# ruffle-rs/h263-rs

Hardware: NVIDIA B200
Metric: decoded_rgba_megapixels_per_s (higher is better)
Workload: dtype f32+u8

## Files before the change

bindings/h263cu-sys/src/lib.rs:

```rust
#![allow(non_camel_case_types)]
use std::os::raw::{c_char, c_int, c_void};

pub const H263CU_OK: c_int = 0;
pub const H263CU_ERR_INTERNAL_DECODER_ERROR: c_int = -1;
pub const H263CU_ERR_MIDDLE_OF_BITSTREAM: c_int = -2;
pub const H263CU_ERR_INVALID_MACROBLOCK_HEADER: c_int = -3;
pub const H263CU_ERR_INVALID_MACROBLOCK_CODED_BITS: c_int = -4;
pub const H263CU_ERR_INVALID_INTRA_DC: c_int = -5;
pub const H263CU_ERR_INVALID_SHORT_COEFFICIENT: c_int = -6;
pub const H263CU_ERR_INVALID_LONG_COEFFICIENT: c_int = -7;
pub const H263CU_ERR_INVALID_MVD: c_int = -8;
pub const H263CU_ERR_INVALID_PTYPE: c_int = -9;
pub const H263CU_ERR_INVALID_PLUSPTYPE: c_int = -10;
pub const H263CU_ERR_INVALID_GOB_HEADER: c_int = -11;
pub const H263CU_ERR_INVALID_BITSTREAM: c_int = -12;
pub const H263CU_ERR_PICTURE_FORMAT_MISSING: c_int = -13;
pub const H263CU_ERR_PICTURE_FORMAT_INVALID: c_int = -14;
pub const H263CU_ERR_UNCODED_IFRAME_BLOCKS: c_int = -15;
pub const H263CU_ERR_UNHANDLED_IO_ERROR: c_int = -16;
pub const H263CU_ERR_UNIMPLEMENTED_DECODING: c_int = -17;
pub const H263CU_ERR_BAD_ARGUMENT: c_int = -100;
pub const H263CU_ERR_CUDA: c_int = -101;
pub const H263CU_ERR_NO_DEVICE: c_int = -102;
pub const H263CU_ERR_CAPACITY: c_int = -103;
pub const H263CU_ERR_REFERENCE_WOULD_ABORT: c_int = -104;
pub const H263CU_ERR_NO_PICTURE: c_int = -105;
pub const H263CU_ERR_OUT_OF_MEMORY: c_int = -106;

pub const H263CU_OPT_SORENSON_SPARK_BITSTREAM: u32 = 1;
pub const H263CU_OPT_USE_SCALABILITY_MODE: u32 = 2;
pub const H263CU_OPT_DECODE_DISPOSABLE: u32 = 0x100;

pub const H263CU_PIC_I: u8 = 0;
pub const H263CU_PIC_P: u8 = 1;
pub const H263CU_PIC_DISPOSABLE_P: u8 = 2;
pub const H263CU_PIC_OTHER: u8 = 3;
pub const H263CU_PICFLAG_DEBLOCK: u8 = 1;
pub const H263CU_PICFLAG_HAS_INTER: u8 = 2;
pub const H263CU_PICFLAG_MV_IN_RANGE: u8 = 4;
pub const H263CU_PICFLAG_DISPOSABLE: u8 = 8;
pub const H263CU_MB_INTER: u8 = 1;
pub const H263CU_MB_WIDE: u8 = 2;
pub const H263CU_MB_FOURMV: u8 = 4;
pub const H263CU_MB_CODED: u8 = 8;
pub const H263CU_OUT_RGBA: u32 = 1;
pub const H263CU_OUT_DEBLOCK: u32 = 2;
pub const H263CU_YUV_I420: u32 = 0;
pub const H263CU_YUV_NV12: u32 = 1;
pub const H263CU_TENSOR_U8: u32 = 0;
pub const H263CU_TENSOR_F32: u32 = 1;
pub const H263CU_TENSOR_F16: u32 = 2;
pub const H263CU_TENSOR_BF16: u32 = 3;
pub const H263CU_FIT_STRETCH: u32 = 0;
pub const H263CU_FIT_LETTERBOX: u32 = 1;
pub const H263CU_FIT_CENTER_CROP: u32 = 2;
pub const H263CU_FILTER_BILINEAR: u32 = 0;
pub const H263CU_FILTER_BILINEAR_AA: u32 = 1;
pub const H263CU_FILTER_BICUBIC_AA: u32 = 2;

#[repr(C)]
#[derive(Clone, Copy, Debug, Default)]
pub struct h263cu_pic {
    pub stream: u32,
    pub width: u16,
    pub height: u16,
    pub mb_w: u8,
    pub mb_h: u8,
    pub pic_type: u8,
    pub pquant: u8,
    pub flags: u8,
    pub version: u8,
    pub temporal_reference: u16,
    pub first_mb: u32,
    pub n_mbs: u32,
    pub first_event: u32,
    pub n_event_units: u32,
}

#[repr(C)]
#[derive(Clone, Copy, Debug, Default)]
pub struct h263cu_mb {
    pub ev_off: u32,
    pub pic: u16,
    pub mbx: u8,
    pub mby: u8,
    pub flags: u8,
    pub quant: u8,
    pub nev: [u8; 6],
    pub u: [u8; 8],
}

#[repr(C)]
#[derive(Clone, Copy, Debug, Default)]
pub struct h263cu_flv_packet {
    pub offset: u64,
    pub size: u32,
    pub timestamp_ms: u32,
    pub frame_type: u8,
    pub codec_id: u8,
    pub reserved: u16,
    pub reserved2: u32,
}

pub type h263cu_event = u16;

#[repr(C)]
#[derive(Clone, Copy, Debug)]
pub struct h263cu_device_rgba {
    pub base: *mut u8,
    pub row_pitch: u64,
    pub pic_stride: u64,
    pub width: u32,
    pub height: u32,
    pub stream: *mut c_void,
}

#[repr(C)]
#[derive(Clone, Copy, Debug)]
pub struct h263cu_device_plane {
    pub base: *mut u8,
    pub row_pitch: u64,
    pub pic_stride: u64,
}

#[repr(C)]
#[derive(Clone, Copy, Debug)]
pub struct h263cu_device_yuv {
    pub plane: [h263cu_device_plane; 3],
    pub width: u32,
    pub height: u32,
    pub format: u32,
    pub reserved: u32,
    pub stream: *mut c_void,
}

#[repr(C)]
#[derive(Clone, Copy, Debug)]
pub struct h263cu_device_tensor {
    pub base: *mut c_void,
    pub stride: [i64; 4],
    pub width: u32,
    pub height: u32,
    pub dtype: u32,
    pub reserved: u32,
    pub mul: [f32; 3],
    pub add: [f32; 3],
    pub stream: *mut c_void,
}

#[repr(C)]
#[derive(Clone, Copy, Debug)]
pub struct h263cu_tensor_crop {
    pub x: u32,
    pub y: u32,
    pub width: u32,
    pub height: u32,
}

#[repr(C)]
#[derive(Clone, Copy, Debug)]
pub struct h263cu_tensor_fit {
    pub mode: u32,
    pub short_side: u32,
    pub fill: [f32; 3],
    pub reserved: u32,
    pub crops: *const h263cu_tensor_crop,
}

#[repr(C)]
pub struct h263cu_parser {
    _private: [u8; 0],
}
#[repr(C)]
pub struct h263cu_ctx {
    _private: [u8; 0],
}
#[repr(C)]
pub struct h263cu_step {
    _private: [u8; 0],
}
#[repr(C)]
pub struct h263cu_graph {
    _private: [u8; 0],
}
#[repr(C)]
pub struct h263cu_group {
    _private: [u8; 0],
}

extern "C" {
    pub fn h263cu_is_eof_error(err: c_int) -> c_int;
    pub fn h263cu_is_macroblock_error(err: c_int) -> c_int;
    pub fn h263cu_is_gob_error(err: c_int) -> c_int;
    pub fn h263cu_strerror(err: c_int) -> *const c_char;
    pub fn h263cu_version() -> c_int;

    pub fn h263cu_parser_create(decoder_options: u32) -> *mut h263cu_parser;
// ... 167 lines not shown
```

h263_rs_b200/_lib.py:

```python
import ctypes as C
import os

HERE = os.path.dirname(os.path.abspath(__file__))
LIB_PATH = os.environ.get("H263CU_LIB", os.path.join(HERE, "libh263cu.so"))

OK = 0
ERR_INVALID_BITSTREAM = -12
ERR_UNHANDLED_IO_ERROR = -16
ERR_BAD_ARGUMENT = -100
ERR_CUDA = -101
ERR_NO_DEVICE = -102
ERR_CAPACITY = -103
ERR_REFERENCE_WOULD_ABORT = -104
ERR_NO_PICTURE = -105

OPT_SORENSON = 1
OUT_RGBA = 1
OUT_DEBLOCK = 2

PIC_I, PIC_P, PIC_DISPOSABLE_P, PIC_OTHER = 0, 1, 2, 3
MB_INTER, MB_WIDE, MB_FOURMV, MB_CODED = 1, 2, 4, 8


class Pic(C.Structure):
    _fields_ = [
        ("stream", C.c_uint32), ("width", C.c_uint16), ("height", C.c_uint16), ("mb_w", C.c_uint8),
        ("mb_h", C.c_uint8), ("pic_type", C.c_uint8), ("pquant", C.c_uint8), ("flags", C.c_uint8),
        ("version", C.c_uint8), ("temporal_reference", C.c_uint16), ("first_mb", C.c_uint32), ("n_mbs", C.c_uint32),
        ("first_event", C.c_uint32), ("n_event_units", C.c_uint32),
    ]


class MbUnion(C.Union):
    _fields_ = [("mv", (C.c_int8 * 2) * 4), ("intradc", C.c_uint8 * 6)]


class Mb(C.Structure):
    _fields_ = [
        ("ev_off", C.c_uint32), ("pic", C.c_uint16), ("mbx", C.c_uint8), ("mby", C.c_uint8), ("flags", C.c_uint8),
        ("quant", C.c_uint8), ("nev", C.c_uint8 * 6), ("u", MbUnion),
    ]


class DeviceRgba(C.Structure):
    _fields_ = [
        ("base", C.c_void_p), ("row_pitch", C.c_uint64), ("pic_stride", C.c_uint64), ("width", C.c_uint32),
        ("height", C.c_uint32), ("stream", C.c_void_p),
    ]


class DevicePlane(C.Structure):
    _fields_ = [("base", C.c_void_p), ("row_pitch", C.c_uint64), ("pic_stride", C.c_uint64)]


class DeviceYuv(C.Structure):
    _fields_ = [
        ("plane", DevicePlane * 3), ("width", C.c_uint32), ("height", C.c_uint32), ("format", C.c_uint32),
        ("reserved", C.c_uint32), ("stream", C.c_void_p),
    ]


YUV_I420, YUV_NV12 = 0, 1


class DeviceTensor(C.Structure):
    _fields_ = [
        ("base", C.c_void_p), ("stride", C.c_int64 * 4), ("width", C.c_uint32), ("height", C.c_uint32),
        ("dtype", C.c_uint32), ("reserved", C.c_uint32), ("mul", C.c_float * 3), ("add", C.c_float * 3),
        ("stream", C.c_void_p),
    ]


TENSOR_U8, TENSOR_F32, TENSOR_F16, TENSOR_BF16 = 0, 1, 2, 3


class TensorCrop(C.Structure):
    _fields_ = [("x", C.c_uint32), ("y", C.c_uint32), ("width", C.c_uint32), ("height", C.c_uint32)]


class TensorFit(C.Structure):
    _fields_ = [
        ("mode", C.c_uint32), ("short_side", C.c_uint32), ("fill", C.c_float * 3), ("reserved", C.c_uint32),
        ("crops", C.POINTER(TensorCrop)),
    ]


FIT_STRETCH, FIT_LETTERBOX, FIT_CENTER_CROP = 0, 1, 2
FILTER_BILINEAR, FILTER_BILINEAR_AA, FILTER_BICUBIC_AA = 0, 1, 2

assert C.sizeof(Pic) == 32 and C.sizeof(Mb) == 24 and C.sizeof(DeviceRgba) == 40
assert C.sizeof(DevicePlane) == 24 and C.sizeof(DeviceYuv) == 96 and C.sizeof(DeviceTensor) == 88
assert C.sizeof(TensorCrop) == 16 and C.sizeof(TensorFit) == 32

SYMBOLS = [
    "h263cu_is_eof_error", "h263cu_is_macroblock_error", "h263cu_is_gob_error", "h263cu_strerror",
    "h263cu_version", "h263cu_parser_create", "h263cu_parser_destroy", "h263cu_parser_options", "h263cu_parser_reset",
    "h263cu_peek_picture", "h263cu_parse_picture", "h263cu_parse_step", "h263cu_device_count",
    "h263cu_create", "h263cu_destroy", "h263cu_device_of", "h263cu_alloc_pinned", "h263cu_free_pinned",
    "h263cu_step_upload", "h263cu_step_free", "h263cu_step_run", "h263cu_submit_step",
    "h263cu_submit_step_readback", "h263cu_decode_step", "h263cu_sync", "h263cu_stream_info", "h263cu_read_yuv", "h263cu_read_rgba",
    "h263cu_checksums", "h263cu_timer_start", "h263cu_timer_stop", "h263cu_launch_count", "h263cu_tiled_launch_count",
    "h263cu_profile_enable", "h263cu_profile_read", "h263cu_host_times",
    "h263cu_yuv420_to_rgba", "h263cu_deblock", "h263cu_quant_to_strength",
    "h263cu_flv_scan", "h263cu_flv_mux",
    "h263cu_test_read_bits", "h263cu_test_start_code", "h263cu_test_read_vlc", "h263cu_test_decode_block",
    "h263cu_readback_wait", "h263cu_stream_dims", "h263cu_graph_build", "h263cu_graph_launch", "h263cu_graph_free", "h263cu_group_create", "h263cu_group_destroy", "h263cu_group_size", "h263cu_group_ctx",
    "h263cu_group_decode_step", "h263cu_group_sync", "h263cu_decode_step_device", "h263cu_group_decode_step_device",
    "h263cu_decode_step_device_yuv", "h263cu_group_decode_step_device_yuv",
    "h263cu_decode_step_device_tensor", "h263cu_group_decode_step_device_tensor",
    "h263cu_decode_step_device_tensor_fit", "h263cu_group_decode_step_device_tensor_fit", "h263cu_test_fit_geometry",
    "h263cu_decode_step_device_tensor_filter", "h263cu_group_decode_step_device_tensor_filter",
]

_lib = None


def lib():
    global _lib
    if _lib is not None:
        return _lib
    if not os.path.exists(LIB_PATH):
        raise RuntimeError(
            "libh263cu.so is missing (%s): run `python -c 'import __graft_entry__ as g; g.build()'`; "
            "this package has no CPU fallback" % LIB_PATH
        )
    L = C.CDLL(LIB_PATH)
    vp, u32, u64, i32 = C.c_void_p, C.c_uint32, C.c_uint64, C.c_int
    L.h263cu_strerror.restype = C.c_char_p
    L.h263cu_strerror.argtypes = [i32]
    L.h263cu_parser_create.restype = vp
    L.h263cu_parser_create.argtypes = [u32]
    L.h263cu_parser_destroy.argtypes = [vp]
    L.h263cu_parser_options.restype = u32
    L.h263cu_parser_options.argtypes = [vp]
    L.h263cu_parser_destroy.restype = None
    L.h263cu_parser_reset.argtypes = [vp]
    L.h263cu_parser_reset.restype = None
    L.h263cu_peek_picture.argtypes = [u32, C.c_char_p, C.c_size_t, C.POINTER(Pic)]
    L.h263cu_parse_picture.argtypes = [vp, C.c_char_p, C.c_size_t, u32, C.c_uint16, u32, u32, C.POINTER(Pic), vp, u32,
                                       vp, u32]
    L.h263cu_parse_step.argtypes = [vp, vp, vp, vp, u32, i32, vp, vp, u32, vp, u32, C.POINTER(u32), C.POINTER(u32),
                                    C.POINTER(u32), vp, vp]
    if hasattr(L, "h263cu_create"):
        L.h263cu_create.restype = vp
        L.h263cu_create.argtypes = [i32, u32, u32, u32, u32, C.POINTER(i32)]
        L.h263cu_destroy.argtypes = [vp]
        L.h263cu_destroy.restype = None
        L.h263cu_device_of.argtypes = [vp]
        L.h263cu_alloc_pinned.restype = vp
        L.h263cu_alloc_pinned.argtypes = [C.c_size_t]
        L.h263cu_free_pinned.argtypes = [vp]
        L.h263cu_free_pinned.restype = None
        L.h263cu_step_upload.restype = vp
        L.h263cu_step_upload.argtypes = [vp, vp, u32, vp, u32, vp, u32, C.POINTER(i32)]
        L.h263cu_step_free.argtypes = [vp, vp]
        L.h263cu_step_free.restype = None
        L.h263cu_step_run.argtypes = [vp, vp, u32]
        L.h263cu_submit_step.argtypes = [vp, vp, u32, vp, u32, vp, u32, u32]
        L.h263cu_submit_step_readback.argtypes = [vp, vp, u32, vp, u32, vp, u32, u32, vp, vp]
        L.h263cu_decode_step.argtypes = [vp, vp, vp, vp, vp, u32, i32, u32, vp, u64, vp, C.POINTER(u32)]
        L.h263cu_decode_step_device.argtypes = [vp, vp, vp, vp, vp, u32, i32, u32, C.POINTER(DeviceRgba), vp, C.POINTER(u32)]
        L.h263cu_decode_step_device_yuv.argtypes = [vp, vp, vp, vp, vp, u32, i32, u32, C.POINTER(DeviceYuv), vp, C.POINTER(u32)]
        L.h263cu_decode_step_device_tensor.argtypes = [vp, vp, vp, vp, vp, u32, i32, u32, C.POINTER(DeviceTensor), vp, C.POINTER(u32)]
        L.h263cu_decode_step_device_tensor_fit.argtypes = [vp, vp, vp, vp, vp, u32, i32, u32, C.POINTER(DeviceTensor),
                                                           C.POINTER(TensorFit), vp, C.POINTER(u32)]
        L.h263cu_decode_step_device_tensor_filter.argtypes = [vp, vp, vp, vp, vp, u32, i32, u32, C.POINTER(DeviceTensor),
                                                              C.POINTER(TensorFit), u32, vp, C.POINTER(u32)]
        L.h263cu_sync.argtypes = [vp]
        L.h263cu_readback_wait.argtypes = [vp, u32]
        L.h263cu_graph_build.restype = vp
        L.h263cu_graph_build.argtypes = [vp, vp, u32, u32, C.POINTER(i32)]
        L.h263cu_graph_launch.argtypes = [vp, vp]
        L.h263cu_graph_free.argtypes = [vp, vp]
        L.h263cu_graph_free.restype = None
# ... 69 lines not shown
```

h263_rs_b200/csrc/context.cu:

```cuda
#include <cuda_runtime.h>

#include <algorithm>
#include <chrono>
#include <cmath>
#include <cstdio>
#include <cstdlib>
#include <cstring>
#include <mutex>
#include <new>
#include <vector>

#include "device_math.cuh"
#include "kernels.cuh"

using namespace h263dev;

namespace h263fe {
int parse_step_deferred(h263cu_parser* const* parsers, const uint8_t* const* packets, const size_t* lens,
                        const uint32_t* stream_ids, uint32_t n, int threads, h263cu_pic* pics, h263cu_mb* mbs, uint32_t mb_cap,
                        h263cu_event* events, uint32_t ev_cap, uint32_t* n_pics_out, uint32_t* n_mbs_out, uint32_t* n_units_out,
                        int* per_pic_err, int32_t* pic_of_input, uint32_t max_w, uint32_t max_h, const uint32_t* min_size);
void parse_step_finish(h263cu_parser* const* parsers, uint32_t n, bool accept);
}

extern "C" const uint8_t h263cu_quant_to_strength[32] = H263_QUANT_TO_STRENGTH;

namespace {

#define CU_TRY(expr)                      \
    do {                                  \
        cudaError_t _e = (expr);          \
        if (_e != cudaSuccess) return map_cuda_error(_e); \
    } while (0)

int map_cuda_error(cudaError_t e) {
    switch (e) {
        case cudaErrorNoDevice:
        case cudaErrorInsufficientDriver:
        case cudaErrorInvalidDevice: return H263CU_ERR_NO_DEVICE;
        case cudaErrorMemoryAllocation: return H263CU_ERR_OUT_OF_MEMORY;
        default: return H263CU_ERR_CUDA;
    }
}

inline size_t round_up(size_t v, size_t a) { return (v + a - 1) / a * a; }

struct StreamState {
    bool has_pic = false;
    uint8_t cur_slot = 0;
    int8_t rgba_slot = -1;
    uint16_t w = 0, h = 0;
    uint8_t pic_type = 0, pquant = 0;
    uint16_t tr = 0;
    uint32_t stamp = 0;
    uint32_t seen = 0;
    bool has_ref = false;
    uint8_t ref_slot = 0;
    uint16_t ref_w = 0, ref_h = 0;
    bool padded = false;
};

inline int next_slot(const StreamState& st) { return st.has_ref ? (st.ref_slot ^ 1) : (st.has_pic ? (st.cur_slot ^ 1) : 0); }

inline void advance_stream(StreamState& st, const h263cu_pic& p, bool want_rgba, int rgba_ring, bool tiled) {
    const int slot = next_slot(st);
    st.cur_slot = (uint8_t)slot;
    st.has_pic = true;
    st.w = p.width, st.h = p.height;
    st.pic_type = p.pic_type, st.pquant = p.pquant, st.tr = p.temporal_reference;
    st.rgba_slot = want_rgba ? (int8_t)rgba_ring : (int8_t)-1;
    if (!(p.flags & H263CU_PICFLAG_DISPOSABLE)) {
        st.has_ref = true;
        st.ref_slot = (uint8_t)slot;
        st.ref_w = p.width, st.ref_h = p.height;
        st.padded = tiled;
    }
}

}

struct h263cu_step {
    std::vector<h263cu_pic> pics;
    h263cu_mb* d_mbs = nullptr;
    h263cu_event* d_events = nullptr;
    uint32_t n_mbs = 0, n_units = 0;
    size_t mb_cap = 0, ev_cap = 0;
    uint32_t max_w = 0, max_h = 0;
};

struct h263cu_ctx {
    int device = 0;
    uint32_t max_streams = 0, max_w = 0, max_h = 0;
    uint32_t mbw = 0, mbh = 0;
    uint32_t pitch_y = 0, pitch_c = 0, rgba_pitch = 0;
    size_t y_slot = 0, c_slot = 0, rgba_slot = 0;
    uint8_t *y_pool = nullptr, *c_pool = nullptr, *rgba_pool = nullptr;
    CUtensorMap rgba_map;
    std::vector<StreamState> streams;
    uint32_t stamp = 0, decode_epoch = 0;
    uint32_t rgba_parity = 0;

    cudaStream_t s_main = nullptr, s_h2d = nullptr, s_d2h = nullptr;
    cudaStream_t s_pics = nullptr;
    static constexpr int PIC_RING = 4;
    PicDev* h_pics[PIC_RING] = {};
    PicDev* d_pics[PIC_RING] = {};
    cudaEvent_t pics_done[PIC_RING] = {};
    cudaEvent_t pics_up[PIC_RING] = {};
    FitGeom* h_geo[PIC_RING] = {};
    FitGeom* d_geo[PIC_RING] = {};
    size_t pics_cap = 0;
    int pic_ring_pos = 0;
    h263cu_step ring[2];
    cudaEvent_t ring_h2d_done[2] = {}, ring_run_done[2] = {};
    int ring_pos = 0;
    struct Staging {
        h263cu_pic* pics = nullptr;
        h263cu_mb* mbs = nullptr;
        h263cu_event* events = nullptr;
        size_t pic_cap = 0, mb_cap = 0, ev_cap = 0;
    } staging[2];
    std::vector<int32_t> pic_of_input;
    std::vector<uint64_t> rgba_offsets;
    std::vector<uint32_t> dev_slots;
    std::vector<uint32_t> fit_min;
    std::vector<FitGeom> fit_geo;
    cudaEvent_t dev_ready = nullptr, dev_done = nullptr;
    uint8_t* tensor_scratch = nullptr;
    size_t tensor_scratch_slots = 0;
    cudaEvent_t rgba_written[2] = {}, rgba_read[2] = {};
    cudaEvent_t t0 = nullptr, t1 = nullptr;
    uint64_t launches = 0, tiled_launches = 0;
    bool profiling = false;
    std::vector<cudaEvent_t> prof_free;
    struct ProfSpan {
        cudaEvent_t a, b;
        int kind;
    };
    std::vector<ProfSpan> prof_spans;
    ChecksumJob* d_jobs = nullptr;
    unsigned long long* d_sums = nullptr;
    size_t jobs_cap = 0;

    int force_kernel = 0;
    double host_parse_s = 0.0, host_other_s = 0.0;
    uint64_t host_calls = 0;
    uint8_t* plane(int p, uint32_t stream, int slot) const {
        const size_t idx = (size_t)stream * 2 + (size_t)slot;
        if (p == 0) return y_pool + idx * y_slot + (size_t)PAD_Y_ROWS * pitch_y + PAD_Y_COLS;
        return c_pool + idx * c_slot + (size_t)PAD_C_ROWS * pitch_c + PAD_C_COLS + (p == 2 ? 1 : 0);
    }
    uint8_t* rgba(uint32_t stream, int slot) const { return rgba_pool + ((size_t)slot * max_streams + stream) * rgba_slot; }
};

namespace {

int ensure_pic_ring(h263cu_ctx* c, size_t n) {
    if (n <= c->pics_cap) return 0;
    CU_TRY(cudaStreamSynchronize(c->s_main));
    size_t cap = std::max<size_t>(n, 256);
    for (int i = 0; i < h263cu_ctx::PIC_RING; i++) {
        if (c->h_pics[i]) cudaFreeHost(c->h_pics[i]);
        if (c->d_pics[i]) cudaFree(c->d_pics[i]);
        if (c->h_geo[i]) cudaFreeHost(c->h_geo[i]);
        if (c->d_geo[i]) cudaFree(c->d_geo[i]);
        c->h_pics[i] = nullptr, c->d_pics[i] = nullptr, c->h_geo[i] = nullptr, c->d_geo[i] = nullptr;
        CU_TRY(cudaHostAlloc((void**)&c->h_pics[i], cap * sizeof(PicDev), cudaHostAllocDefault));
        CU_TRY(cudaMalloc((void**)&c->d_pics[i], cap * sizeof(PicDev)));
        CU_TRY(cudaHostAlloc((void**)&c->h_geo[i], cap * sizeof(FitGeom), cudaHostAllocDefault));
        CU_TRY(cudaMalloc((void**)&c->d_geo[i], cap * sizeof(FitGeom)));
    }
    c->pics_cap = cap;
    return 0;
}

int step_reserve(h263cu_step* s, size_t n_mbs, size_t n_units) {
    if (n_mbs > s->mb_cap) {
        if (s->d_mbs) cudaFree(s->d_mbs);
        s->d_mbs = nullptr;
        size_t cap = n_mbs + n_mbs / 8 + 64;
        CU_TRY(cudaMalloc((void**)&s->d_mbs, cap * sizeof(h263cu_mb)));
        s->mb_cap = cap;
    }
    if (n_units + 8 > s->ev_cap) {
        if (s->d_events) cudaFree(s->d_events);
        s->d_events = nullptr;
        size_t cap = n_units + n_units / 8 + 64;
        CU_TRY(cudaMalloc((void**)&s->d_events, cap * sizeof(h263cu_event)));
        s->ev_cap = cap;
    }
    return 0;
}

int prof_take(h263cu_ctx* c, cudaEvent_t* a, cudaEvent_t* b) {
    for (cudaEvent_t* e : {a, b}) {
        if (!c->prof_free.empty()) {
            *e = c->prof_free.back();
            c->prof_free.pop_back();
        } else {
            CU_TRY(cudaEventCreate(e));
        }
    }
    return 0;
}
void prof_end(h263cu_ctx* c, cudaEvent_t a, cudaEvent_t b, int kind) {
    cudaEventRecord(b, c->s_main);
    c->prof_spans.push_back({a, b, kind});
}

PicDev make_picdev(const h263cu_ctx* c, const h263cu_pic& p, const StreamState& st, bool want_rgba, int rgba_ring) {
    const int ref_slot = st.ref_slot, new_slot = next_slot(st);
    PicDev d;
    std::memset(&d, 0, sizeof(d));
    for (int k = 0; k < 3; k++) {
        d.cur[k] = c->plane(k, p.stream, new_slot);
        d.ref[k] = st.has_ref ? c->plane(k, p.stream, ref_slot) : nullptr;
    }
    d.rgba = want_rgba ? c->rgba(p.stream, rgba_ring) : nullptr;
    d.cur_y4 = (uint32_t)((d.cur[0] - c->y_pool) >> 2);
    d.cur_c4 = (uint32_t)((d.cur[1] - c->c_pool) >> 2);
    d.ref_y4 = st.has_ref ? (uint32_t)((d.ref[0] - c->y_pool) >> 2) : 0u;
    d.ref_c4 = st.has_ref ? (uint32_t)((d.ref[1] - c->c_pool) >> 2) : 0u;
    d.rgba_row0 = want_rgba ? (uint32_t)((size_t)(d.rgba - c->rgba_pool) / c->rgba_pitch) : 0u;
    d.first_event = p.first_event;
    d.rgba_pitch = c->rgba_pitch;
    d.w = p.width, d.h = p.height;
    d.cw = (uint16_t)((p.width + 1) / 2), d.ch = (uint16_t)((p.height + 1) / 2);
    d.pitch_y = (uint16_t)c->pitch_y, d.pitch_c = (uint16_t)c->pitch_c;
    d.strength = h263cu_quant_to_strength[p.pquant & 31];
    d.flags = p.flags;
    return d;
}

struct DeviceTarget {
    int out;
    CUtensorMap map;
    uint8_t* base;
    uint64_t row_pitch, pic_stride;
    YuvDst yuv;
    TensorDst tensor;
// ... 2 lines not shown
    float fill[3];
    uint32_t filter;
    const uint32_t* slots;
    cudaStream_t stream;
};

int ensure_tensor_scratch(h263cu_ctx* c, uint32_t n, YuvDst* d) {
    const size_t pitch = (size_t)c->mbw * 16, y_bytes = pitch * c->mbh * 16, c_bytes = pitch * c->mbh * 8;
    if (n > c->tensor_scratch_slots) {
        CU_TRY(cudaStreamSynchronize(c->s_main));
        if (c->tensor_scratch) cudaFree(c->tensor_scratch);
        c->tensor_scratch = nullptr, c->tensor_scratch_slots = 0;
        const size_t slots = std::max<size_t>(n, 64);
        CU_TRY(cudaMalloc((void**)&c->tensor_scratch, slots * (y_bytes + c_bytes)));
        c->tensor_scratch_slots = slots;
    }
    std::memset(d, 0, sizeof(*d));
    d->base[0] = c->tensor_scratch, d->base[1] = c->tensor_scratch + c->tensor_scratch_slots * y_bytes;
    d->stride[0] = y_bytes, d->stride[1] = c_bytes;
    d->pitch[0] = d->pitch[1] = (uint32_t)pitch;
    d->nv12 = 1;
    return 0;
}

int run_step(h263cu_ctx* c, h263cu_step* s, uint32_t out_flags, bool lean = false, const DeviceTarget* dev = nullptr) {
    const uint32_t n = (uint32_t)s->pics.size();
    if (n == 0) return 0;
    if (n > 65535) return H263CU_ERR_CAPACITY;
    const bool want_rgba = dev || (out_flags & H263CU_OUT_RGBA) != 0;
    const bool pool_rgba = want_rgba && !dev;
    const bool want_deblock = want_rgba && (out_flags & H263CU_OUT_DEBLOCK) != 0;
    const bool tensor = dev && dev->out == OUT_TENSOR;
    const uint32_t stamp = ++c->stamp;
    uint32_t max_w = 0, max_h = 0;
    bool tiled = true, aligned16 = true, wide_mv = false;
    for (uint32_t i = 0; i < n; i++) {
        const h263cu_pic& p = s->pics[i];
        if (p.stream >= c->max_streams) return H263CU_ERR_CAPACITY;
        if (p.width == 0 || p.height == 0 || p.width > c->max_w || p.height > c->max_h) return H263CU_ERR_CAPACITY;
        if ((uint32_t)p.mb_w * 16 < p.width || (uint32_t)p.mb_h * 16 < p.height ||
            (uint32_t)p.mb_w > c->mbw || (uint32_t)p.mb_h > c->mbh)
            return H263CU_ERR_BAD_ARGUMENT;
        if ((uint64_t)p.first_mb + p.n_mbs > s->n_mbs || (uint64_t)p.first_event + p.n_event_units > s->n_units ||
            p.n_mbs != (uint32_t)p.mb_w * p.mb_h)
            return H263CU_ERR_BAD_ARGUMENT;
        StreamState& st = c->streams[p.stream];
        if (st.stamp == stamp) return H263CU_ERR_BAD_ARGUMENT;
        st.stamp = stamp;
        if (p.flags & H263CU_PICFLAG_HAS_INTER) {
            if (!st.has_ref) return H263CU_ERR_UNCODED_IFRAME_BLOCKS;
            if (st.ref_w != p.width || st.ref_h != p.height) return H263CU_ERR_REFERENCE_WOULD_ABORT;
        }
        max_w = std::max<uint32_t>(max_w, p.width);
        max_h = std::max<uint32_t>(max_h, p.height);
        if ((p.width | p.height) & 15) aligned16 = false;
        if ((p.flags & H263CU_PICFLAG_HAS_INTER) && !(p.flags & H263CU_PICFLAG_MV_IN_RANGE)) wide_mv = true;
        if ((p.flags & H263CU_PICFLAG_HAS_INTER) && !st.padded) tiled = false;
    }
    if (c->force_kernel == 1) tiled = false;
    int e = ensure_pic_ring(c, n);
    if (e) return e;
    YuvDst scratch{};
    if (tensor && want_deblock && (e = ensure_tensor_scratch(c, n, &scratch))) return e;
    const int slot = c->pic_ring_pos;
    CU_TRY(cudaEventSynchronize(c->pics_done[slot]));
    const int rgba_ring = (int)(c->rgba_parity & 1u);
    PicDev* hp = c->h_pics[slot];
    const bool fit = tensor && dev->geo;
    if (fit) std::memcpy(c->h_geo[slot], dev->geo, n * sizeof(FitGeom));
    for (uint32_t i = 0; i < n; i++) {
        const h263cu_pic& p = s->pics[i];
        PicDev d = make_picdev(c, p, c->streams[p.stream], pool_rgba, rgba_ring);
        if (tensor) {
            d.rgba = want_deblock ? yuv_row(scratch, 0, i, 0) : nullptr;
            d.rgba_row0 = i << 12;
            d.out_slot = dev->slots[i];
        } else if (dev) {
            if (dev->out == OUT_YUV) {
                d.rgba = yuv_row(dev->yuv, 0, dev->slots[i], 0);
                d.rgba_pitch = dev->yuv.pitch[0];
            } else {
                d.rgba = dev->base + (size_t)dev->slots[i] * dev->pic_stride;
                d.rgba_pitch = (uint32_t)dev->row_pitch;
            }
            d.rgba_row0 = dev->slots[i] << 12;
        }
        hp[i] = d;
    }
    cudaEvent_t pa = nullptr, pb = nullptr, qa = nullptr, qb = nullptr;
    if (c->profiling) {
        if ((e = prof_take(c, &pa, &pb))) return e;
        if (want_deblock && (e = prof_take(c, &qa, &qb))) {
            c->prof_free.push_back(pa), c->prof_free.push_back(pb);
            return e;
        }
    }
    if (lean) {
        CU_TRY(cudaMemcpyAsync(c->d_pics[slot], hp, n * sizeof(PicDev), cudaMemcpyHostToDevice, c->s_main));
        if (fit) CU_TRY(cudaMemcpyAsync(c->d_geo[slot], c->h_geo[slot], n * sizeof(FitGeom), cudaMemcpyHostToDevice, c->s_main));
    } else {
        CU_TRY(cudaMemcpyAsync(c->d_pics[slot], hp, n * sizeof(PicDev), cudaMemcpyHostToDevice, c->s_pics));
        if (fit) CU_TRY(cudaMemcpyAsync(c->d_geo[slot], c->h_geo[slot], n * sizeof(FitGeom), cudaMemcpyHostToDevice, c->s_pics));
        CU_TRY(cudaEventRecord(c->pics_up[slot], c->s_pics));
        CU_TRY(cudaStreamWaitEvent(c->s_main, c->pics_up[slot], 0));
    }
    if (pool_rgba) {
        CU_TRY(cudaStreamWaitEvent(c->s_main, c->rgba_read[rgba_ring], 0));
    }
    if (dev) {
        CU_TRY(cudaEventRecord(c->dev_ready, dev->stream));
        CU_TRY(cudaStreamWaitEvent(c->s_main, c->dev_ready, 0));
    }
    if (pa) cudaEventRecord(pa, c->s_main);
    const Pools pools{c->y_pool, c->c_pool, c->rgba_pool, c->pitch_y, c->pitch_c, c->rgba_pitch};
    const YuvDst* yuv = dev && dev->out == OUT_YUV ? &dev->yuv : tensor && want_deblock ? &scratch : nullptr;
    const bool dev_out = dev && !tensor;
    launch_recon(c->d_pics[slot], s->d_mbs, s->d_events, s->n_mbs, want_rgba && !want_deblock && !tensor, tiled ? (aligned16 ? 1 : 2) : 0,
                 wide_mv, pools, dev_out ? &dev->map : &c->rgba_map, dev_out ? dev->out : OUT_POOL, yuv, c->s_main);
    if (pa) prof_end(c, pa, pb, 0);
    if (want_deblock) {
        if (qa) cudaEventRecord(qa, c->s_main);
        if (aligned16 && c->force_kernel != 1)
            launch_deblock_rgba_tile(c->d_pics[slot], n, max_w, max_h, yuv, c->s_main);
        else
            launch_deblock_rgba(c->d_pics[slot], n, max_w, max_h, yuv, c->s_main);
        if (qa) prof_end(c, qa, qb, 1);
    }
    if (tensor) {
        const FitArgs fa{c->d_geo[slot], {dev->fill[0], dev->fill[1], dev->fill[2]}};
        if (fit && dev->filter != H263CU_FILTER_BILINEAR)
            launch_resample_filter(c->d_pics[slot], n, want_deblock ? &scratch : nullptr, dev->tensor, dev->dtype, dev->filter, fa,
                                   c->s_main);
        else
            launch_resample_rgb(c->d_pics[slot], n, want_deblock ? &scratch : nullptr, dev->tensor, dev->dtype, fit ? &fa : nullptr,
                                c->s_main);
    }
    CU_TRY(cudaGetLastError());
    c->pic_ring_pos = (c->pic_ring_pos + 1) % h263cu_ctx::PIC_RING;
    c->launches += (want_deblock ? 2 : 1) + (tensor ? 1 : 0);
    if (tiled) c->tiled_launches++;
    for (uint32_t i = 0; i < n; i++) advance_stream(c->streams[s->pics[i].stream], s->pics[i], pool_rgba, rgba_ring, tiled);
    CU_TRY(cudaEventRecord(c->pics_done[slot], c->s_main));
    if (dev) {
        CU_TRY(cudaEventRecord(c->dev_done, c->s_main));
        CU_TRY(cudaStreamWaitEvent(dev->stream, c->dev_done, 0));
    }
    if (pool_rgba) {
        if (!lean) CU_TRY(cudaEventRecord(c->rgba_written[rgba_ring], c->s_main));
        c->rgba_parity++;
    }
    return 0;
}

int validate_side_info(std::vector<h263cu_pic>& pics, const h263cu_mb* mbs, uint32_t n_mbs, uint32_t n_units) {
    for (size_t i = 0; i < pics.size(); i++) {
        h263cu_pic& p = pics[i];
        if ((uint64_t)p.first_mb + p.n_mbs > n_mbs || (uint64_t)p.first_event + p.n_event_units > n_units ||
            p.n_mbs != (uint32_t)p.mb_w * p.mb_h || p.mb_w == 0)
            return H263CU_ERR_BAD_ARGUMENT;
        bool any_inter = false, in_range = true;
        const h263cu_mb* m = mbs + p.first_mb;
        for (uint32_t k = 0; k < p.n_mbs; k++, m++) {
            if (m->pic != i || (uint32_t)m->mby * p.mb_w + m->mbx != k || m->mbx >= p.mb_w) return H263CU_ERR_BAD_ARGUMENT;
            const bool intra = !(m->flags & H263CU_MB_INTER);
            uint32_t ev = 0;
            for (int b = 0; b < 6; b++) {
                if (m->nev[b] > (intra ? 63 : 64) || (intra && m->nev[b] && m->u.intradc[b] == 0)) return H263CU_ERR_BAD_ARGUMENT;
                ev += m->nev[b];
            }
            if (m->flags & H263CU_MB_WIDE) ev *= 2;
            if ((uint64_t)m->ev_off + ev > p.n_event_units) return H263CU_ERR_BAD_ARGUMENT;
            if (m->flags & H263CU_MB_INTER) {
                any_inter = true;
                for (int b = 0; b < 4; b++)
                    in_range &= m->u.mv[b][0] >= -32 && m->u.mv[b][0] <= 31 && m->u.mv[b][1] >= -32 && m->u.mv[b][1] <= 31;
            }
        }
        if (any_inter) p.flags |= H263CU_PICFLAG_HAS_INTER;
        if (!in_range) p.flags &= (uint8_t)~H263CU_PICFLAG_MV_IN_RANGE;
    }
    return 0;
}

int upload_into(h263cu_ctx* c, h263cu_step* s, const h263cu_pic* pics, uint32_t n_pics, const h263cu_mb* mbs,
                uint32_t n_mbs, const h263cu_event* events, uint32_t n_units, cudaStream_t stream, bool trusted) {
    int e = step_reserve(s, n_mbs, n_units);
    if (e) return e;
    try {
        s->pics.assign(pics, pics + n_pics);
    } catch (const std::bad_alloc&) {
        return H263CU_ERR_OUT_OF_MEMORY;
    }
    s->n_mbs = n_mbs, s->n_units = n_units;
    if (!trusted && (e = validate_side_info(s->pics, mbs, n_mbs, n_units))) {
        s->pics.clear();
        return e;
    }
    if (n_mbs) CU_TRY(cudaMemcpyAsync(s->d_mbs, mbs, (size_t)n_mbs * sizeof(h263cu_mb), cudaMemcpyHostToDevice, stream));
    if (n_units)
        CU_TRY(cudaMemcpyAsync(s->d_events, events, (size_t)n_units * sizeof(h263cu_event), cudaMemcpyHostToDevice, stream));
    (void)c;
    return 0;
}

template <typename T>
int grow_pinned(T** p, size_t* cap, size_t need) {
    if (need <= *cap) return 0;
    if (*p) cudaFreeHost(*p);
    *p = nullptr, *cap = 0;
    const size_t n = need + need / 4 + 64;
    CU_TRY(cudaHostAlloc((void**)p, n * sizeof(T), cudaHostAllocDefault));
    *cap = n;
    return 0;
}
typedef CUresult (*EncodeTiled)(CUtensorMap*, CUtensorMapDataType, cuuint32_t, void*, const cuuint64_t*, const cuuint64_t*,
                                const cuuint32_t*, const cuuint32_t*, CUtensorMapInterleave, CUtensorMapSwizzle,
                                CUtensorMapL2promotion, CUtensorMapFloatOOBfill);
EncodeTiled encode_tiled() {
    static const EncodeTiled fn = [] {
        EncodeTiled enc = nullptr;
        cudaDriverEntryPointQueryResult q;
        if (cudaGetDriverEntryPoint("cuTensorMapEncodeTiled", (void**)&enc, cudaEnableDefault, &q) != cudaSuccess) {
            cudaGetLastError();
            enc = nullptr;
        }
        return enc;
    }();
    return fn;
}
int encode_rgba_map(CUtensorMap* map, void* base, uint32_t rank, const cuuint64_t* dims, const cuuint64_t* strides) {
    const EncodeTiled enc = encode_tiled();
    if (!enc) return H263CU_ERR_CUDA;
    const cuuint32_t box[3] = {64, 16, 1}, es[3] = {1, 1, 1};
    if (enc(map, CU_TENSOR_MAP_DATA_TYPE_UINT8, rank, base, dims, strides, box, es, CU_TENSOR_MAP_INTERLEAVE_NONE,
            CU_TENSOR_MAP_SWIZZLE_NONE, CU_TENSOR_MAP_L2_PROMOTION_NONE, CU_TENSOR_MAP_FLOAT_OOB_FILL_NONE) != CUDA_SUCCESS)
        return H263CU_ERR_CUDA;
    return 0;
}
int make_rgba_map(CUtensorMap* map, void* base, uint64_t pitch, uint64_t rows) {
    std::memset(map, 0, sizeof(*map));
    if (!recon_tile_uses_tma()) return 0;
    const cuuint64_t dims[2] = {pitch, rows}, strides[1] = {pitch};
    return encode_rgba_map(map, base, 2, dims, strides);
}
int check_device_memory(const h263cu_ctx* c, const void* p) {
    cudaPointerAttributes a;
    if (cudaPointerGetAttributes(&a, p) != cudaSuccess) {
        cudaGetLastError();
        return H263CU_ERR_BAD_ARGUMENT;
    }
    if ((a.type != cudaMemoryTypeDevice && a.type != cudaMemoryTypeManaged) || a.device != c->device) return H263CU_ERR_BAD_ARGUMENT;
    return 0;
}
int check_device_rgba(const h263cu_ctx* c, const h263cu_device_rgba* o) {
    if (!o || !recon_tile_uses_tma()) return H263CU_ERR_BAD_ARGUMENT;
    if (!o->base || ((uintptr_t)o->base & 15u) || o->width == 0 || o->height == 0) return H263CU_ERR_BAD_ARGUMENT;
    if (o->row_pitch % 16 || o->row_pitch < 4ull * o->width || o->row_pitch >= (1ull << 32)) return H263CU_ERR_BAD_ARGUMENT;
    if (o->pic_stride % 16 || o->pic_stride < o->row_pitch * o->height || o->pic_stride >= (1ull << 40)) return H263CU_ERR_BAD_ARGUMENT;
    return check_device_memory(c, o->base);
}
int check_device_yuv(const h263cu_ctx* c, const h263cu_device_yuv* o) {
    if (!o || o->format > H263CU_YUV_NV12 || o->reserved != 0 || o->width == 0 || o->height == 0) return H263CU_ERR_BAD_ARGUMENT;
    const bool nv12 = o->format == H263CU_YUV_NV12;
    const uint64_t cw = (o->width + 1ull) / 2, ch = (o->height + 1ull) / 2;
    const uint64_t row_bytes[3] = {o->width, nv12 ? 2 * cw : cw, cw}, rows[3] = {o->height, ch, ch};
    if (nv12 && (o->plane[2].base || o->plane[2].row_pitch || o->plane[2].pic_stride)) return H263CU_ERR_BAD_ARGUMENT;
    for (int k = 0; k < (nv12 ? 2 : 3); k++) {
        const h263cu_device_plane& p = o->plane[k];
        if (!p.base || ((uintptr_t)p.base & 3u) || p.row_pitch % 4 || p.pic_stride % 4) return H263CU_ERR_BAD_ARGUMENT;
        if (p.row_pitch < row_bytes[k] || p.row_pitch >= (1ull << 32)) return H263CU_ERR_BAD_ARGUMENT;
        if (p.pic_stride < p.row_pitch * rows[k] || p.pic_stride >= (1ull << 40)) return H263CU_ERR_BAD_ARGUMENT;
    }
    for (int k = 0; k < (nv12 ? 2 : 3); k++)
        if (int e = check_device_memory(c, o->plane[k].base)) return e;
    return 0;
}
int check_device_tensor(const h263cu_ctx* c, const h263cu_device_tensor* o) {
    if (!o || o->dtype > H263CU_TENSOR_BF16 || o->reserved != 0) return H263CU_ERR_BAD_ARGUMENT;
    if (o->width == 0 || o->height == 0 || o->width > 16384 || o->height > 16384) return H263CU_ERR_BAD_ARGUMENT;
    static const uint32_t elem_bytes[4] = {1, 4, 2, 2};
    const uint32_t es = elem_bytes[o->dtype];
    if (!o->base || (uintptr_t)o->base % es) return H263CU_ERR_BAD_ARGUMENT;
    for (int k = 0; k < 4; k++)
        if (o->stride[k] <= 0) return H263CU_ERR_BAD_ARGUMENT;
    const unsigned __int128 extent = ((unsigned __int128)(o->width - 1) * (uint64_t)o->stride[3] +
                                      (unsigned __int128)(o->height - 1) * (uint64_t)o->stride[2] +
                                      (unsigned __int128)2 * (uint64_t)o->stride[1] + 1) * es;
    if (extent >= ((unsigned __int128)1 << 40)) return H263CU_ERR_BAD_ARGUMENT;
    for (int k = 0; k < 3; k++) {
        if (!std::isfinite(o->mul[k]) || !std::isfinite(o->add[k])) return H263CU_ERR_BAD_ARGUMENT;
        if (o->dtype == H263CU_TENSOR_U8 && (o->mul[k] != 1.0f || o->add[k] != 0.0f)) return H263CU_ERR_BAD_ARGUMENT;
    }
    return check_device_memory(c, o->base);
}
int check_tensor_fit(const h263cu_tensor_fit* f, uint32_t n) {
    if (!f || f->mode > H263CU_FIT_CENTER_CROP || f->reserved != 0) return H263CU_ERR_BAD_ARGUMENT;
    if (f->mode == H263CU_FIT_CENTER_CROP ? f->short_side < 1 || f->short_side > 16384 : f->short_side != 0)
        return H263CU_ERR_BAD_ARGUMENT;
    for (int k = 0; k < 3; k++)
        if (!(f->fill[k] >= 0.0f && f->fill[k] <= 255.0f)) return H263CU_ERR_BAD_ARGUMENT;
    if (f->crops)
        for (uint32_t i = 0; i < n; i++) {
            const h263cu_tensor_crop& b = f->crops[i];
            if (b.width == 0 || b.height == 0 || (uint64_t)b.x + b.width > 0xFFFFFFFFull || (uint64_t)b.y + b.height > 0xFFFFFFFFull)
                return H263CU_ERR_BAD_ARGUMENT;
        }
    return 0;
}
void fit_geometry(uint32_t mode, uint32_t short_side, uint32_t cw, uint32_t ch, uint32_t W, uint32_t H, int32_t* out4) {
    const int64_t w = cw, h = ch, ow = W, oh = H, S = short_side;
    int64_t rw = ow, rh = oh, px = 0, py = 0;
    if (mode == H263CU_FIT_LETTERBOX) {
        if (w * oh >= h * ow)
            rh = std::max<int64_t>(1, (2 * h * ow + w) / (2 * w));
        else
            rw = std::max<int64_t>(1, (2 * w * oh + h) / (2 * h));
        px = (ow - rw) / 2, py = (oh - rh) / 2;
    } else if (mode == H263CU_FIT_CENTER_CROP) {
        if (w <= h)
            rw = S, rh = S * h / w;
        else
            rh = S, rw = S * w / h;
        const auto place = [](int64_t r, int64_t o) -> int64_t {
            if (r < o) return (o - r) / 2;
            const int64_t d = r - o, k = d / 2;
            return -((d & 1) ? k + (k & 1) : k);
        };
        px = place(rw, ow), py = place(rh, oh);
    }
    out4[0] = (int32_t)rw, out4[1] = (int32_t)rh, out4[2] = (int32_t)px, out4[3] = (int32_t)py;
}
void free_step_buffers(h263cu_step* s) {
    if (s->d_mbs) cudaFree(s->d_mbs);
    if (s->d_events) cudaFree(s->d_events);
    s->d_mbs = nullptr, s->d_events = nullptr;
    s->mb_cap = s->ev_cap = 0;
}

}

extern "C" {

int h263cu_device_count(void) {
    int n = 0;
    if (cudaGetDeviceCount(&n) != cudaSuccess) {
        cudaGetLastError();
        return 0;
    }
    return n;
}

h263cu_ctx* h263cu_create(int device, uint32_t max_streams, uint32_t max_width, uint32_t max_height, uint32_t flags,
                          int* err) {
    (void)flags;
    int dummy;
    if (!err) err = &dummy;
    *err = 0;
    if (max_streams == 0 || max_width == 0 || max_height == 0 || max_width > 4080 || max_height > 4080) {
        *err = H263CU_ERR_BAD_ARGUMENT;
        return nullptr;
    }
    int ndev = 0;
    cudaError_t ce = cudaGetDeviceCount(&ndev);
    if (ce != cudaSuccess || ndev == 0) {
        cudaGetLastError();
        *err = H263CU_ERR_NO_DEVICE;
        return nullptr;
    }
    if (device < 0 || device >= ndev) {
        *err = H263CU_ERR_NO_DEVICE;
        return nullptr;
    }
    if (cudaSetDevice(device) != cudaSuccess) {
        *err = H263CU_ERR_CUDA;
        return nullptr;
    }
    h263cu_ctx* c = new (std::nothrow) h263cu_ctx();
    if (!c) {
        *err = H263CU_ERR_OUT_OF_MEMORY;
        return nullptr;
    }
    c->device = device;
    c->max_streams = max_streams, c->max_w = max_width, c->max_h = max_height;
    c->mbw = (max_width + 15) / 16, c->mbh = (max_height + 15) / 16;
    c->pitch_y = c->mbw * 16 + 2 * PAD_Y_COLS;
    c->pitch_c = c->mbw * 8 * CHROMA_STEP + 2 * PAD_C_COLS;
    c->rgba_pitch = c->mbw * 16 * 4;
    c->y_slot = (size_t)c->pitch_y * (c->mbh * 16 + 2 * PAD_Y_ROWS);
    c->c_slot = (size_t)c->pitch_c * (c->mbh * 8 + 2 * PAD_C_ROWS);
    if (const char* k = getenv("H263CU_KERNEL")) c->force_kernel = !strcmp(k, "mb") ? 1 : (!strcmp(k, "tile") ? 2 : 0);
    c->rgba_slot = (size_t)c->rgba_pitch * c->mbh * 16;
    c->streams.resize(max_streams);
    auto fail = [&](int code) {
        *err = code;
        h263cu_destroy(c);
        return (h263cu_ctx*)nullptr;
    };
    const size_t pad = 256;
    if (c->y_slot * 2 * max_streams + pad >= (16ull << 30) || c->rgba_slot * 2 * max_streams + pad >= (64ull << 30)) return fail(H263CU_ERR_CAPACITY);
    if (cudaMalloc((void**)&c->y_pool, c->y_slot * 2 * max_streams + pad) != cudaSuccess) return fail(H263CU_ERR_OUT_OF_MEMORY);
    if (cudaMalloc((void**)&c->c_pool, c->c_slot * 2 * max_streams + pad) != cudaSuccess) return fail(H263CU_ERR_OUT_OF_MEMORY);
    if (cudaMalloc((void**)&c->rgba_pool, c->rgba_slot * 2 * max_streams + pad) != cudaSuccess) return fail(H263CU_ERR_OUT_OF_MEMORY);
    {
        const int e = make_rgba_map(&c->rgba_map, c->rgba_pool, c->rgba_pitch, (uint64_t)2 * max_streams * c->mbh * 16);
        if (e) return fail(e);
    }
    if (cudaStreamCreateWithFlags(&c->s_main, cudaStreamNonBlocking) != cudaSuccess) return fail(H263CU_ERR_CUDA);
    if (cudaStreamCreateWithFlags(&c->s_h2d, cudaStreamNonBlocking) != cudaSuccess) return fail(H263CU_ERR_CUDA);
    if (cudaStreamCreateWithFlags(&c->s_d2h, cudaStreamNonBlocking) != cudaSuccess) return fail(H263CU_ERR_CUDA);
    if (cudaStreamCreateWithFlags(&c->s_pics, cudaStreamNonBlocking) != cudaSuccess) return fail(H263CU_ERR_CUDA);
    for (int i = 0; i < h263cu_ctx::PIC_RING; i++)
        if (cudaEventCreateWithFlags(&c->pics_done[i], cudaEventDisableTiming) != cudaSuccess ||
            cudaEventCreateWithFlags(&c->pics_up[i], cudaEventDisableTiming) != cudaSuccess)
            return fail(H263CU_ERR_CUDA);
    for (int i = 0; i < 2; i++) {
        if (cudaEventCreateWithFlags(&c->ring_h2d_done[i], cudaEventDisableTiming) != cudaSuccess ||
            cudaEventCreateWithFlags(&c->ring_run_done[i], cudaEventDisableTiming) != cudaSuccess ||
            cudaEventCreateWithFlags(&c->rgba_written[i], cudaEventDisableTiming) != cudaSuccess ||
            cudaEventCreateWithFlags(&c->rgba_read[i], cudaEventDisableTiming) != cudaSuccess)
            return fail(H263CU_ERR_CUDA);
    }
    if (cudaEventCreateWithFlags(&c->dev_ready, cudaEventDisableTiming) != cudaSuccess ||
        cudaEventCreateWithFlags(&c->dev_done, cudaEventDisableTiming) != cudaSuccess)
        return fail(H263CU_ERR_CUDA);
    if (cudaEventCreate(&c->t0) != cudaSuccess || cudaEventCreate(&c->t1) != cudaSuccess) return fail(H263CU_ERR_CUDA);
    cudaMemsetAsync(c->y_pool, 0, c->y_slot * 2 * max_streams + pad, c->s_main);
    cudaMemsetAsync(c->c_pool, 0, c->c_slot * 2 * max_streams + pad, c->s_main);
    if (cudaStreamSynchronize(c->s_main) != cudaSuccess) return fail(H263CU_ERR_CUDA);
    return c;
}

void h263cu_destroy(h263cu_ctx* c) {
    if (!c) return;
    cudaSetDevice(c->device);
    if (c->s_main) cudaStreamSynchronize(c->s_main);
    if (c->s_h2d) cudaStreamSynchronize(c->s_h2d);
    if (c->s_d2h) cudaStreamSynchronize(c->s_d2h);
    if (c->s_pics) cudaStreamSynchronize(c->s_pics);
    for (int i = 0; i < 2; i++) free_step_buffers(&c->ring[i]);
    for (auto& st : c->staging) {
        if (st.pics) cudaFreeHost(st.pics);
        if (st.mbs) cudaFreeHost(st.mbs);
        if (st.events) cudaFreeHost(st.events);
    }
    for (int i = 0; i < h263cu_ctx::PIC_RING; i++) {
        if (c->h_pics[i]) cudaFreeHost(c->h_pics[i]);
        if (c->d_pics[i]) cudaFree(c->d_pics[i]);
        if (c->h_geo[i]) cudaFreeHost(c->h_geo[i]);
        if (c->d_geo[i]) cudaFree(c->d_geo[i]);
        if (c->pics_done[i]) cudaEventDestroy(c->pics_done[i]);
        if (c->pics_up[i]) cudaEventDestroy(c->pics_up[i]);
    }
    for (int i = 0; i < 2; i++) {
        if (c->ring_h2d_done[i]) cudaEventDestroy(c->ring_h2d_done[i]);
        if (c->ring_run_done[i]) cudaEventDestroy(c->ring_run_done[i]);
        if (c->rgba_written[i]) cudaEventDestroy(c->rgba_written[i]);
        if (c->rgba_read[i]) cudaEventDestroy(c->rgba_read[i]);
    }
    if (c->t0) cudaEventDestroy(c->t0);
    if (c->t1) cudaEventDestroy(c->t1);
    if (c->dev_ready) cudaEventDestroy(c->dev_ready);
    if (c->dev_done) cudaEventDestroy(c->dev_done);
    if (c->tensor_scratch) cudaFree(c->tensor_scratch);
    for (auto& sp : c->prof_spans) {
        cudaEventDestroy(sp.a);
        cudaEventDestroy(sp.b);
    }
    for (auto e : c->prof_free) cudaEventDestroy(e);
    if (c->d_jobs) cudaFree(c->d_jobs);
    if (c->d_sums) cudaFree(c->d_sums);
    if (c->y_pool) cudaFree(c->y_pool);
    if (c->c_pool) cudaFree(c->c_pool);
    if (c->rgba_pool) cudaFree(c->rgba_pool);
    if (c->s_main) cudaStreamDestroy(c->s_main);
    if (c->s_h2d) cudaStreamDestroy(c->s_h2d);
    if (c->s_d2h) cudaStreamDestroy(c->s_d2h);
    if (c->s_pics) cudaStreamDestroy(c->s_pics);
    delete c;
}

int h263cu_device_of(h263cu_ctx* c) { return c ? c->device : -1; }

void* h263cu_alloc_pinned(size_t bytes) {
    void* p = nullptr;
    if (cudaHostAlloc(&p, bytes ? bytes : 1, cudaHostAllocDefault) != cudaSuccess) {
        cudaGetLastError();
        return nullptr;
    }
    return p;
// ... 898 lines not shown
```

h263_rs_b200/csrc/frontend.cpp:

```cpp
#include <algorithm>
#include <atomic>
#include <condition_variable>
#include <cstring>
#include <functional>
#include <mutex>
#include <new>
#include <pthread.h>
#include <thread>
#include <vector>

#include "../../include/h263cu.h"
#include "bitio.hpp"

namespace h263fe {

#include "vlc_codes.inc"

void VlcTable::build(const VlcCode* codes, int n) {
    max_len = 0;
    for (int i = 0; i < n; i++) max_len = std::max(max_len, codes[i].len);
    lut.assign((size_t)1 << max_len, VlcEntry{(uint8_t)(2u << 5), 0, 0, 0});
    for (int i = 0; i < n; i++) {
        uint32_t v = 0;
        for (int k = 0; k < codes[i].len; k++) v = (v << 1) | (uint32_t)(codes[i].bits[k] - '0');
        int rest = max_len - codes[i].len;
        VlcEntry e{(uint8_t)((unsigned)codes[i].len | ((unsigned)codes[i].kind << 5)), (int8_t)codes[i].a,
                   (uint8_t)codes[i].b, (uint8_t)codes[i].c};
        for (uint32_t s = 0; s < (1u << rest); s++) lut[((size_t)v << rest) | s] = e;
    }
}

namespace {
struct Tables {
    VlcTable t[5];
    std::vector<uint32_t> tcoef_fast;
    int tcoef_bits = 0;
    Tables() {
        t[T_MCBPC_I].build(MCBPC_I_CODES, MCBPC_I_CODES_COUNT);
        t[T_MCBPC_P].build(MCBPC_P_CODES, MCBPC_P_CODES_COUNT);
        t[T_CBPY].build(CBPY_CODES, CBPY_CODES_COUNT);
        t[T_MVD].build(MVD_CODES, MVD_CODES_COUNT);
        t[T_TCOEF].build(TCOEF_CODES, TCOEF_CODES_COUNT);
        tcoef_bits = t[T_TCOEF].max_len + 1;
        tcoef_fast.resize(t[T_TCOEF].lut.size() * 2);
        for (size_t i = 0; i < tcoef_fast.size(); i++) {
            const VlcEntry& e = t[T_TCOEF].lut[i >> 1];
            uint32_t w = e.len() | (e.kind() << 5);
            if (e.kind() == 0) {
                const uint32_t sign = (uint32_t)(i >> (t[T_TCOEF].max_len - e.len())) & 1u;
                const uint32_t level = sign ? (0u - (uint32_t)e.c) & 0x3FFu : (uint32_t)e.c;
                w = (e.len() + 1u) | ((uint32_t)(e.a != 0) << 7) | ((((uint32_t)e.b << 10) | level) << 16);
            }
            tcoef_fast[i] = w;
        }
    }
};
const Tables& tables() {
    static const Tables T;
    return T;
}
}

const VlcTable& vlc_table(int id) { return tables().t[id]; }
static const uint32_t* tcoef_fast_table(int* bits) {
    *bits = tables().tcoef_bits;
    return tables().tcoef_fast.data();
}
const VlcCode* vlc_codes(int id, int* count) {
    switch (id) {
        case T_MCBPC_I: *count = MCBPC_I_CODES_COUNT; return MCBPC_I_CODES;
        case T_MCBPC_P: *count = MCBPC_P_CODES_COUNT; return MCBPC_P_CODES;
        case T_CBPY: *count = CBPY_CODES_COUNT; return CBPY_CODES;
        case T_MVD: *count = MVD_CODES_COUNT; return MVD_CODES;
        default: *count = TCOEF_CODES_COUNT; return TCOEF_CODES;
    }
}

struct Header {
    int version = -1;
    uint16_t tr = 0;
    int fmt_kind = -1;
    uint16_t w = 0, h = 0;
    bool dims_valid = false;
    uint8_t pic_type = H263CU_PIC_I;
    bool type_supported = true;
    bool deblock = false;
    uint8_t quant = 0;
};

static bool std_dims(int kind, uint16_t* w, uint16_t* h) {
    static const uint16_t W[5] = {128, 176, 352, 704, 1408}, H[5] = {96, 144, 288, 576, 1152};
    if (kind < 0 || kind > 4) return false;
    *w = W[kind], *h = H[kind];
    return true;
}

static int find_start_code(BitReader& r, uint32_t* skipped) {
    const size_t save = r.pos();
    uint32_t max_skip = (uint32_t)((8 - (r.pos() & 7)) & 7);
    uint32_t skip = 0;
    for (;;) {
        if (r.avail() < 17) {
            r.seek(save);
            return H263CU_ERR_UNHANDLED_IO_ERROR;
        }
        if (r.peek_padded(17) == 1) break;
        if (skip > max_skip) {
            r.seek(save);
            return H263CU_ERR_MIDDLE_OF_BITSTREAM;
        }
        r.consume(1);
        skip += 1;
    }
    r.seek(save);
    *skipped = skip;
    return 0;
}

#define RD(n, var)                                         \
    do {                                                   \
        if (!r.read((n), &(var))) return H263CU_ERR_UNHANDLED_IO_ERROR; \
    } while (0)

static int parse_header(BitReader& r, uint32_t options, bool have_prev, int prev_kind, uint16_t prev_w,
                        uint16_t prev_h, Header* out) {
    uint32_t skipped = 0, v = 0;
    int e = find_start_code(r, &skipped);
    if (e) return e;
    if (!r.skip(17 + skipped)) return H263CU_ERR_UNHANDLED_IO_ERROR;
    uint32_t gob_id;
    RD(5, gob_id);
    Header h;
    if (options & H263CU_OPT_SORENSON_SPARK_BITSTREAM) {
        RD(8, v);
        h.tr = (uint16_t)v;
        uint32_t code;
        RD(3, code);
        switch (code) {
            case 0: {
                uint32_t cw, ch;
                RD(8, cw);
                RD(8, ch);
                h.fmt_kind = 6, h.w = (uint16_t)cw, h.h = (uint16_t)ch, h.dims_valid = true;
                break;
            }
            case 1: {
                uint32_t cw, ch;
                RD(16, cw);
                RD(16, ch);
                h.fmt_kind = 6, h.w = (uint16_t)cw, h.h = (uint16_t)ch, h.dims_valid = true;
                break;
            }
            case 2: h.fmt_kind = 2; break;
            case 3: h.fmt_kind = 1; break;
            case 4: h.fmt_kind = 0; break;
            case 5: h.fmt_kind = 6, h.w = 320, h.h = 240, h.dims_valid = true; break;
            case 6: h.fmt_kind = 6, h.w = 160, h.h = 120, h.dims_valid = true; break;
            default: h.fmt_kind = 5; break;
        }
        if (h.fmt_kind <= 4) h.dims_valid = std_dims(h.fmt_kind, &h.w, &h.h);
        RD(2, v);
        h.pic_type = (uint8_t)v;
        if (v == 3) h.type_supported = false;
        RD(1, v);
        h.deblock = v == 1;
        RD(5, v);
        h.quant = (uint8_t)v;
        for (;;) {
            RD(1, v);
            if (v != 1) break;
            RD(8, v);
        }
        h.version = (int)gob_id;
        *out = h;
        return 0;
    }
    if (gob_id != 0) return H263CU_ERR_MIDDLE_OF_BITSTREAM;
    RD(8, v);
    h.tr = (uint16_t)v;
    uint32_t hi;
    RD(8, hi);
    if ((hi & 0xC0) != 0x80) return H263CU_ERR_INVALID_PTYPE;
    switch (hi & 7) {
        case 0: return H263CU_ERR_INVALID_PTYPE;
        case 7: return H263CU_ERR_UNIMPLEMENTED_DECODING;
        case 6: h.fmt_kind = 5; break;
        default: h.fmt_kind = (int)(hi & 7) - 1; break;
    }
    h.dims_valid = std_dims(h.fmt_kind, &h.w, &h.h);
    uint32_t lo;
    RD(5, lo);
    h.pic_type = (lo & 0x10) ? H263CU_PIC_I : H263CU_PIC_P;
    if (lo & 1) h.pic_type = H263CU_PIC_OTHER, h.type_supported = false;
    if (have_prev && !(prev_kind == h.fmt_kind && (h.fmt_kind != 6 || (prev_w == h.w && prev_h == h.h))))
        return H263CU_ERR_UNIMPLEMENTED_DECODING;
    RD(5, v);
    h.quant = (uint8_t)v;
    RD(1, v);
    if (v) RD(2, v);
    if (lo & 1) {
        RD(3, v);
        RD(2, v);
    }
    for (;;) {
        RD(1, v);
        if (v != 1) break;
        RD(8, v);
    }
    h.version = -1;
    *out = h;
    return 0;
}

static inline int median3(int a, int b, int c) {
    int lo = std::min(a, b), hi = std::max(a, b);
    return std::max(lo, std::min(hi, c));
}
static inline int wrap_mv(int pred, int mvd) {
    int out = mvd + pred;
    if (out < -32 || out >= 32) out = (mvd > 0 ? mvd - 64 : (mvd < 0 ? mvd + 64 : 0)) + pred;
    return out;
}

struct Mv {
    int8_t x, y;
};

}

using namespace h263fe;

struct h263cu_parser {
    uint32_t options = 0;
    bool has_last = false;
    bool has_reference = false;
    int last_fmt_kind = -1;
    uint16_t last_w = 0, last_h = 0;
    uint16_t ref_w = 0, ref_h = 0;
    std::vector<Mv> mvs;
    std::vector<h263cu_mb> st_mbs;
    std::vector<h263cu_event> st_events;
    h263cu_pic st_pic;
    int st_err = 0;
    struct Pending {
        bool valid = false;
        bool has_last = false, has_reference = false;
        int fmt_kind = -1;
        uint16_t w = 0, h = 0, ref_w = 0, ref_h = 0;
    } pending;
};

namespace {

struct PendingState {
    bool has_last, has_reference;
    int fmt_kind;
    uint16_t w, h, ref_w, ref_h;
};

static inline int parse_block(BitReader& r_io, const Header& hd, uint32_t options, bool intra, bool coded, int* dc_code,
                              uint8_t* __restrict ev_run, int16_t* __restrict ev_level, int* nev, bool* overflow) {
    const VlcTable& T = vlc_table(T_TCOEF);
    BitReader r = r_io;
    uint32_t v;
    *dc_code = -1;
    *nev = 0;
    *overflow = false;
    if (intra) {
        if (!r.read(8, &v)) return H263CU_ERR_UNHANDLED_IO_ERROR;
        if (v == 0 || v == 128) return H263CU_ERR_INVALID_INTRA_DC;
        *dc_code = (int)v;
    }
    if (!coded) {
        r_io = r;
        return 0;
    }
    const bool sorenson_v1 = (options & H263CU_OPT_SORENSON_SPARK_BITSTREAM) && hd.version == 1;
    int idx = intra ? 1 : 0;
    int n = 0;
    bool ovf = false;
    for (;;) {
        const VlcEntry* e;
        bool eof_sign;
        if (!r.read_vlc_bits(T, 1, &e, &v, &eof_sign)) return H263CU_ERR_UNHANDLED_IO_ERROR;
        int last, run, level;
        if (e->kind() == 0) {
            last = e->a, run = e->b, level = v ? -(int)e->c : (int)e->c;
        } else if (e->kind() == 3) {
            unsigned width = 8;
            if (sorenson_v1) {
                if (!r.read(1, &v)) return H263CU_ERR_UNHANDLED_IO_ERROR;
                width = v ? 11 : 7;
            }
            uint32_t l, rn;
            int32_t lv;
            if (!r.read(1, &l) || !r.read(6, &rn) || !r.read_signed(width, &lv)) return H263CU_ERR_UNHANDLED_IO_ERROR;
            if (lv == 0) return H263CU_ERR_INVALID_LONG_COEFFICIENT;
            last = (int)l, run = (int)rn, level = lv;
        } else {
            return H263CU_ERR_INVALID_SHORT_COEFFICIENT;
        }
        idx += run;
        ovf |= idx >= 64;
        if (!ovf) {
            ev_run[n] = (uint8_t)run;
            ev_level[n] = (int16_t)level;
            n++;
        }
        idx += 1;
        if (last) break;
    }
    *overflow = ovf;
    *nev = ovf ? 0 : n;
    r_io = r;
    return 0;
}

static H263_AI int parse_block_fast(BitReader& r, const uint32_t* __restrict tf, int tf_bits, bool sorenson_v1, bool intra, bool coded,
                                    int* dc_code, h263cu_event* __restrict out, int* nev, bool* overflow, bool* wide) {
    uint32_t v;
    *dc_code = -1;
    *nev = 0;
    *overflow = false;
    if (intra) {
        if (!r.read(8, &v)) return H263CU_ERR_UNHANDLED_IO_ERROR;
        if (v == 0 || v == 128) return H263CU_ERR_INVALID_INTRA_DC;
        *dc_code = (int)v;
    }
    if (!coded) return 0;
    int idx = intra ? 1 : 0;
    int n = 0;
    bool ovf = false;
    for (;;) {
        const uint64_t w = r.window();
        const uint32_t e = tf[(uint32_t)(w >> (64 - tf_bits))];
        const unsigned len = e & 31u, kind = (e >> 5) & 3u;
        int last, run, level;
        uint32_t unit;
        if (__builtin_expect(kind == 0, 1)) {
            if (__builtin_expect(len > r.avail(), 0)) return H263CU_ERR_UNHANDLED_IO_ERROR;
            r.consume(len);
            last = (int)((e >> 7) & 1u);
            unit = e >> 16;
            run = (int)(e >> 26);
        } else if (kind == 3) {
            if (len > r.avail()) return H263CU_ERR_UNHANDLED_IO_ERROR;
            r.consume(len);
            unsigned width = 8;
            if (sorenson_v1) {
                if (!r.read(1, &v)) return H263CU_ERR_UNHANDLED_IO_ERROR;
                width = v ? 11 : 7;
            }
            uint32_t l, rn;
            int32_t lv;
            if (!r.read(1, &l) || !r.read(6, &rn) || !r.read_signed(width, &lv)) return H263CU_ERR_UNHANDLED_IO_ERROR;
            if (lv == 0) return H263CU_ERR_INVALID_LONG_COEFFICIENT;
            last = (int)l, run = (int)rn, level = lv;
            *wide |= level < -512 || level > 511;
            unit = ((uint32_t)run << 10) | ((uint32_t)level & 0x3FFu);
        } else {
            if (len > r.avail()) return H263CU_ERR_UNHANDLED_IO_ERROR;
            return H263CU_ERR_INVALID_SHORT_COEFFICIENT;
        }
        idx += run;
        if (__builtin_expect(idx >= 64, 0))
            ovf = true;
        else if (!ovf)
            out[n++] = (h263cu_event)unit;
        idx += 1;
        if (last) break;
    }
    *overflow = ovf;
    *nev = ovf ? 0 : n;
    return 0;
}

static int parse_picture_impl(h263cu_parser* p, const uint8_t* data, size_t len, uint32_t stream, uint16_t pic_index,
                              uint32_t mb_base, uint32_t ev_base, h263cu_pic* pic, h263cu_mb* mbs, uint32_t mb_cap,
                              h263cu_event* events, uint32_t ev_cap, PendingState* pending) {
    BitReader r0(data, len);
    Header hd;
    int e = parse_header(r0, p->options, p->has_last, p->last_fmt_kind, p->last_w, p->last_h, &hd);
    if (e) return e;
    BitReader r = r0;
    int tf_bits;
    const uint32_t* const tf = tcoef_fast_table(&tf_bits);
    const bool sorenson_v1 = (p->options & H263CU_OPT_SORENSON_SPARK_BITSTREAM) && hd.version == 1;
    if (!hd.dims_valid) return H263CU_ERR_PICTURE_FORMAT_INVALID;
    const uint32_t W = hd.w, H = hd.h;
    const uint32_t mb_w = (W + 15) / 16, mb_h = (H + 15) / 16;
    if (mb_w == 0) return H263CU_ERR_REFERENCE_WOULD_ABORT;
    if (mb_w > 255 || mb_h > 255) return H263CU_ERR_CAPACITY;
    const uint32_t capacity = mb_w * mb_h;
    if (capacity > mb_cap) return H263CU_ERR_CAPACITY;

    const bool is_sorenson = (p->options & H263CU_OPT_SORENSON_SPARK_BITSTREAM) != 0;
    const bool decode_disposable = (p->options & H263CU_OPT_DECODE_DISPOSABLE) != 0;
    const bool is_i = hd.pic_type == H263CU_PIC_I;
    const VlcTable& TMt = vlc_table(is_i ? T_MCBPC_I : T_MCBPC_P);
    const VlcTable& TCt = vlc_table(T_CBPY);
    const VlcTable& TVt = vlc_table(T_MVD);
    const VlcEntry* const TM = TMt.lut.data();
    const VlcEntry* const TC = TCt.lut.data();
    const VlcEntry* const TV = TVt.lut.data();
    const unsigned TM_len = (unsigned)TMt.max_len, TC_len = (unsigned)TCt.max_len, TV_len = (unsigned)TVt.max_len;

    p->mvs.assign((size_t)capacity * 4, Mv{0, 0});
    Mv* mvs = p->mvs.data();

    int quant = hd.quant;
    uint32_t n = 0;
    uint32_t col = 0, row = 0;
    uint32_t ev_used = 0;
    bool any_inter = false;
    bool mv_in_range = true;
    uint8_t ev_run[6][64];
    int16_t ev_level[6][64];

    for (;;) {
        const size_t mb_start = r.pos();
        uint32_t v;
        int err = 0;
        bool uncoded = false, stuffing = false;
        int mb_type = 0;
        bool cbp[6] = {false, false, false, false, false, false};
        int dquant = 0;
        Mv mvd[4] = {{0, 0}, {0, 0}, {0, 0}, {0, 0}};

        do {
            if (!is_i) {
                if (!r.read(1, &v)) {
                    err = H263CU_ERR_UNHANDLED_IO_ERROR;
                    break;
                }
                if (v) {
                    uncoded = true;
                    break;
                }
            }
            if (!is_i && hd.pic_type != H263CU_PIC_P && !(decode_disposable && hd.pic_type == H263CU_PIC_DISPOSABLE_P)) {
                err = H263CU_ERR_UNIMPLEMENTED_DECODING;
                break;
            }
            if (!hd.type_supported) {
                err = H263CU_ERR_UNIMPLEMENTED_DECODING;
                break;
            }
            const VlcEntry* en;
            if (!r.read_vlc(TM, TM_len, &en)) {
                err = H263CU_ERR_UNHANDLED_IO_ERROR;
                break;
            }
            if (en->kind() == 1) {
                stuffing = true;
                break;
            }
            if (en->kind() != 0) {
                err = H263CU_ERR_INVALID_MACROBLOCK_HEADER;
                break;
            }
            mb_type = en->a;
            cbp[4] = en->b != 0, cbp[5] = en->c != 0;
            if (!r.read_vlc(TC, TC_len, &en)) {
                err = H263CU_ERR_UNHANDLED_IO_ERROR;
                break;
            }
            if (en->kind() != 0) {
                err = H263CU_ERR_INVALID_MACROBLOCK_CODED_BITS;
                break;
            }
            const bool intra = mb_type == 3 || mb_type == 4;
            int y = intra ? en->a : (~en->a & 15);
            cbp[0] = (y & 8) != 0, cbp[1] = (y & 4) != 0, cbp[2] = (y & 2) != 0, cbp[3] = (y & 1) != 0;
            if (mb_type == 1 || mb_type == 4 || mb_type == 5) {
                if (!r.read(2, &v)) {
                    err = H263CU_ERR_UNHANDLED_IO_ERROR;
                    break;
                }
                static const int DQ[4] = {-1, -2, 1, 2};
                dquant = DQ[v];
            }
            if (!intra) {
                int nmv = (mb_type == 2 || mb_type == 5) ? 4 : 1;
                for (int k = 0; k < nmv && !err; k++) {
                    for (int c = 0; c < 2; c++) {
                        if (!r.read_vlc(TV, TV_len, &en)) {
                            err = H263CU_ERR_UNHANDLED_IO_ERROR;
                            break;
                        }
                        if (en->kind() != 0) {
                            err = H263CU_ERR_INVALID_MVD;
                            break;
                        }
                        (c ? mvd[k].y : mvd[k].x) = en->a;
                    }
                }
            }
        } while (0);

        if (err) {
            r.seek(mb_start);
            if (err == H263CU_ERR_UNHANDLED_IO_ERROR) break;
            if ((err == H263CU_ERR_INVALID_MACROBLOCK_HEADER || err == H263CU_ERR_INVALID_MACROBLOCK_CODED_BITS) &&
                !is_sorenson) {
                uint32_t skipped = 0;
                BitReader probe = r;
                int ge = find_start_code(probe, &skipped);
                if (ge == H263CU_ERR_MIDDLE_OF_BITSTREAM) break;
                if (ge) break;
                if (r.avail() < 17 + skipped + 5) break;
                const size_t save = r.pos();
                r.seek(save + 17 + skipped);
                uint32_t gn = r.peek_padded(5);
                r.seek(save);
                if (gn == 0 || gn == 15) break;
                return H263CU_ERR_UNIMPLEMENTED_DECODING;
            }
            return err;
        }
        if (stuffing) continue;

        if (uncoded) {
            if (is_i) return H263CU_ERR_UNCODED_IFRAME_BLOCKS;
            if (n < capacity) {
                h263cu_mb& m = mbs[n];
                std::memset(&m, 0, sizeof(m));
                m.ev_off = ev_used;
                m.pic = pic_index;
                m.mbx = (uint8_t)col, m.mby = (uint8_t)row;
                m.flags = H263CU_MB_INTER;
                m.quant = (uint8_t)quant;
                any_inter = true;
            }
            n++;
            if (++col == mb_w) col = 0, row++;
            continue;
        }

        quant = std::min(std::max(quant + dquant, 1), 31);
        const bool intra = mb_type == 3 || mb_type == 4;
        if (n >= capacity) {
            int dc, nev0;
            bool ovf;
            BitReader tmp = r;
            int be = parse_block(tmp, hd, p->options, intra, cbp[0], &dc, ev_run[0], ev_level[0], &nev0, &ovf);
            return be ? be : H263CU_ERR_REFERENCE_WOULD_ABORT;
        }
        Mv* cur = mvs + (size_t)n * 4;
        if (!intra) {
            const bool four = mb_type == 2 || mb_type == 5;
            const Mv zero{0, 0};
            for (int k = 0; k < (four ? 4 : 1); k++) {
                Mv c1, c2, c3;
                if (k == 0 || k == 2)
                    c1 = col == 0 ? zero : mvs[(size_t)(n - 1) * 4 + k + 1];
                else
                    c1 = cur[k - 1];
                if (k < 2) {
                    c2 = row == 0 ? c1 : mvs[(size_t)(n - mb_w) * 4 + k + 2];
                    if (col == mb_w - 1)
                        c3 = zero;
                    else if (row == 0)
                        c3 = c1;
                    else
                        c3 = mvs[(size_t)(n - mb_w + 1) * 4 + 2];
                } else {
                    c2 = cur[0];
                    c3 = cur[1];
                }
                int px = median3(c1.x, c2.x, c3.x), py = median3(c1.y, c2.y, c3.y);
                cur[k].x = (int8_t)wrap_mv(px, mvd[k].x);
                cur[k].y = (int8_t)wrap_mv(py, mvd[k].y);
                mv_in_range &= cur[k].x >= -32 && cur[k].x <= 31 && cur[k].y >= -32 && cur[k].y <= 31;
            }
            if (!four) cur[1] = cur[2] = cur[3] = cur[0];
            any_inter = true;
        }

        h263cu_mb& m = mbs[n];
        std::memset(&m, 0, sizeof(m));
        m.ev_off = ev_used;
        m.pic = pic_index;
        m.mbx = (uint8_t)col, m.mby = (uint8_t)row;
        m.quant = (uint8_t)quant;
        m.flags = (uint8_t)(H263CU_MB_CODED | (intra ? 0 : H263CU_MB_INTER) |
                            ((mb_type == 2 || mb_type == 5) ? H263CU_MB_FOURMV : 0));
        int nev[6];
        bool wide = false;
        uint32_t units = 0;
        if (ev_cap - ev_used >= 6 * 65) {
            const size_t blocks_start = r.pos();
            h263cu_event* ev = events + ev_used;
            int be = 0;
            for (int b = 0; b < 6 && !be; b++) {
                int dc;
                bool ovf;
                be = parse_block_fast(r, tf, tf_bits, sorenson_v1, intra, cbp[b], &dc, ev, &nev[b], &ovf, &wide);
                if (intra) m.u.intradc[b] = ovf ? 0 : (uint8_t)dc;
                m.nev[b] = (uint8_t)nev[b];
                ev += nev[b];
            }
            if (be) return be;
            if (!wide) {
                units = (uint32_t)(ev - (events + ev_used));
            } else {
                r.seek(blocks_start);
            }
        } else {
            wide = true;
        }
        if (wide) {
            wide = false;
            BitReader tmp = r;
            for (int b = 0; b < 6; b++) {
                int dc;
                bool ovf;
                int be = parse_block(tmp, hd, p->options, intra, cbp[b], &dc, ev_run[b], ev_level[b], &nev[b], &ovf);
                if (be) return be;
                if (intra) m.u.intradc[b] = ovf ? 0 : (uint8_t)dc;
                m.nev[b] = (uint8_t)nev[b];
                for (int k = 0; k < nev[b]; k++) wide |= ev_level[b][k] < -512 || ev_level[b][k] > 511;
            }
            r = tmp;
            uint32_t total = 0;
            for (int b = 0; b < 6; b++) total += (uint32_t)nev[b];
            units = wide ? total * 2 : total;
            if (ev_used + units > ev_cap) return H263CU_ERR_CAPACITY;
            h263cu_event* ev = events + ev_used;
            if (wide) {
                m.flags |= H263CU_MB_WIDE;
                for (int b = 0; b < 6; b++)
                    for (int k = 0; k < nev[b]; k++) {
                        *ev++ = ev_run[b][k];
                        *ev++ = (uint16_t)ev_level[b][k];
                    }
            } else {
                for (int b = 0; b < 6; b++)
                    for (int k = 0; k < nev[b]; k++)
                        *ev++ = (uint16_t)(((uint32_t)ev_run[b][k] << 10) | ((uint32_t)ev_level[b][k] & 0x3FF));
            }
        }
        if (!intra)
            for (int k = 0; k < 4; k++) m.u.mv[k][0] = cur[k].x, m.u.mv[k][1] = cur[k].y;
        ev_used += units;
        n++;
        if (++col == mb_w) col = 0, row++;
    }

    for (uint32_t i = n; i < capacity; i++) {
        h263cu_mb& m = mbs[i];
        std::memset(&m, 0, sizeof(m));
        m.ev_off = ev_used;
        m.pic = pic_index;
        m.mbx = (uint8_t)(i % mb_w), m.mby = (uint8_t)(i / mb_w);
        m.flags = H263CU_MB_INTER;
        m.quant = (uint8_t)quant;
        any_inter = true;
    }

    if (any_inter) {
        if (!(p->has_reference && p->has_last)) return H263CU_ERR_UNCODED_IFRAME_BLOCKS;
        const uint16_t rw = decode_disposable ? p->ref_w : p->last_w, rh = decode_disposable ? p->ref_h : p->last_h;
        if (rw != W || rh != H) return H263CU_ERR_REFERENCE_WOULD_ABORT;
    }

    std::memset(pic, 0, sizeof(*pic));
    pic->stream = stream;
    pic->width = (uint16_t)W, pic->height = (uint16_t)H;
    pic->mb_w = (uint8_t)mb_w, pic->mb_h = (uint8_t)mb_h;
    pic->pic_type = hd.pic_type;
    pic->pquant = hd.quant;
    const bool disposable = decode_disposable && hd.pic_type == H263CU_PIC_DISPOSABLE_P;
    pic->flags = (uint8_t)((hd.deblock ? H263CU_PICFLAG_DEBLOCK : 0) | (any_inter ? H263CU_PICFLAG_HAS_INTER : 0) |
                           (mv_in_range ? H263CU_PICFLAG_MV_IN_RANGE : 0) | (disposable ? H263CU_PICFLAG_DISPOSABLE : 0));
    pic->version = hd.version < 0 ? 0xFF : (uint8_t)hd.version;
    pic->first_mb = mb_base;
    pic->n_mbs = capacity;
    pic->first_event = ev_base;
    pic->n_event_units = ev_used;
    pic->temporal_reference = hd.tr;

    pending->has_last = true;
    pending->has_reference = p->has_reference;
    if (is_i) pending->has_reference = false;
    if (hd.pic_type != H263CU_PIC_DISPOSABLE_P) pending->has_reference = true;
    pending->fmt_kind = hd.fmt_kind;
    pending->w = (uint16_t)W, pending->h = (uint16_t)H;
    pending->ref_w = disposable ? p->ref_w : (uint16_t)W, pending->ref_h = disposable ? p->ref_h : (uint16_t)H;
    return 0;
}

static inline void commit(h263cu_parser* p, const PendingState& s) {
    p->has_last = s.has_last;
    p->has_reference = s.has_reference;
    p->last_fmt_kind = s.fmt_kind;
    p->last_w = s.w, p->last_h = s.h;
    p->ref_w = s.ref_w, p->ref_h = s.ref_h;
}

}

namespace {
class WorkerPool {
  public:
    void run(int threads, const std::function<void()>& fn) {
        if (threads <= 1) {
            fn();
            return;
        }
        std::lock_guard<std::mutex> job(job_mutex_);
        {
            std::unique_lock<std::mutex> lk(m_);
            while ((int)n_workers_ < threads - 1) {
                std::thread(&WorkerPool::worker, this, n_workers_).detach();
                n_workers_++;
            }
            fn_ = &fn;
            wanted_ = threads - 1;
            running_ = threads - 1;
            generation_++;
        }
        cv_.notify_all();
        fn();
        std::unique_lock<std::mutex> lk(m_);
        done_.wait(lk, [&] { return running_ == 0; });
        fn_ = nullptr;
    }

  private:
    void worker(size_t index) {
        uint64_t seen = 0;
        for (;;) {
            const std::function<void()>* fn;
            {
                std::unique_lock<std::mutex> lk(m_);
                cv_.wait(lk, [&] { return generation_ != seen; });
                seen = generation_;
                if ((int)index >= wanted_) continue;
                fn = fn_;
            }
            (*fn)();
            std::lock_guard<std::mutex> lk(m_);
            if (--running_ == 0) done_.notify_all();
        }
    }
    std::mutex job_mutex_, m_;
    std::condition_variable cv_, done_;
    const std::function<void()>* fn_ = nullptr;
    size_t n_workers_ = 0;
    int wanted_ = 0, running_ = 0;
    uint64_t generation_ = 0;
};
WorkerPool* g_pool = nullptr;
std::once_flag g_pool_once;
WorkerPool& worker_pool() {
    std::call_once(g_pool_once, [] {
        g_pool = new WorkerPool();
        pthread_atfork(nullptr, nullptr, [] { g_pool = new WorkerPool(); });
    });
    return *g_pool;
}
}

extern "C" {

h263cu_parser* h263cu_parser_create(uint32_t decoder_options) {
    h263cu_parser* p = new (std::nothrow) h263cu_parser();
    if (p) p->options = decoder_options;
    (void)tables();
    return p;
}
void h263cu_parser_destroy(h263cu_parser* p) { delete p; }
uint32_t h263cu_parser_options(const h263cu_parser* p) { return p ? p->options : 0u; }
void h263cu_parser_reset(h263cu_parser* p) {
    if (!p) return;
    p->has_last = p->has_reference = false;
    p->last_fmt_kind = -1;
    p->last_w = p->last_h = 0;
    p->ref_w = p->ref_h = 0;
}

int h263cu_peek_picture(uint32_t decoder_options, const uint8_t* data, size_t len, h263cu_pic* pic) {
    if (!data || !pic) return H263CU_ERR_BAD_ARGUMENT;
    BitReader r(data, len);
    Header hd;
    int e = parse_header(r, decoder_options, false, -1, 0, 0, &hd);
    if (e) return e;
    std::memset(pic, 0, sizeof(*pic));
    if (hd.dims_valid) {
        pic->width = hd.w, pic->height = hd.h;
        uint32_t mw = (hd.w + 15u) / 16u, mh = (hd.h + 15u) / 16u;
        pic->mb_w = (uint8_t)std::min(mw, 255u), pic->mb_h = (uint8_t)std::min(mh, 255u);
        pic->n_mbs = mw * mh;
    }
    pic->pic_type = hd.pic_type;
    pic->pquant = hd.quant;
    pic->flags = hd.deblock ? H263CU_PICFLAG_DEBLOCK : 0;
    pic->version = hd.version < 0 ? 0xFF : (uint8_t)hd.version;
    pic->temporal_reference = hd.tr;
    return 0;
}

int h263cu_parse_picture(h263cu_parser* p, const uint8_t* data, size_t len, uint32_t stream, uint16_t pic_index,
                         uint32_t mb_base, uint32_t ev_base, h263cu_pic* pic, h263cu_mb* mbs, uint32_t mb_cap,
                         h263cu_event* events, uint32_t ev_cap) {
    if (!p || !data || !pic || !mbs || (!events && ev_cap)) return H263CU_ERR_BAD_ARGUMENT;
    PendingState s;
    int e = parse_picture_impl(p, data, len, stream, pic_index, mb_base, ev_base, pic, mbs, mb_cap, events, ev_cap, &s);
    if (e) return e;
    commit(p, s);
    return 0;
}

static int parse_step_impl(h263cu_parser* const* parsers, const uint8_t* const* packets, const size_t* lens,
                           const uint32_t* stream_ids, uint32_t n, int threads, h263cu_pic* pics, h263cu_mb* mbs,
                           uint32_t mb_cap, h263cu_event* events, uint32_t ev_cap, uint32_t* n_pics_out,
                           uint32_t* n_mbs_out, uint32_t* n_units_out, int* per_pic_err, int32_t* pic_of_input,
                           bool commit_now, uint32_t max_w, uint32_t max_h, const uint32_t* min_size) {
    if (!parsers || !packets || !lens || !pics || !mbs || !n_pics_out || !n_mbs_out || !n_units_out)
        return H263CU_ERR_BAD_ARGUMENT;
    for (uint32_t i = 0; i < n; i++)
        if (parsers[i]) parsers[i]->pending.valid = false;
    if (n > 65535) return H263CU_ERR_CAPACITY;
    if (threads <= 0) threads = (int)std::max(1u, std::thread::hardware_concurrency());
    threads = (int)std::min<uint32_t>((uint32_t)threads, std::max(1u, n));
    std::vector<PendingState> pend(n);

    std::atomic<uint32_t> next{0};
    auto work1 = [&]() {
        for (;;) {
            uint32_t i = next.fetch_add(1);
            if (i >= n) break;
            h263cu_parser* p = parsers[i];
            if (!p) continue;
            int e = 0;
            h263cu_pic hdr;
            if (!packets[i]) e = H263CU_ERR_BAD_ARGUMENT;
            if (!e) e = h263cu_peek_picture(p->options, packets[i], lens[i], &hdr);
            if (!e && hdr.n_mbs == 0) e = H263CU_ERR_PICTURE_FORMAT_INVALID;
            if (!e && ((hdr.width + 15u) / 16u > 255u || (hdr.height + 15u) / 16u > 255u)) e = H263CU_ERR_CAPACITY;
            if (!e && max_w && (hdr.width > max_w || hdr.height > max_h)) e = H263CU_ERR_CAPACITY;
            if (!e && min_size && (hdr.width < min_size[2 * i] || hdr.height < min_size[2 * i + 1])) e = H263CU_ERR_BAD_ARGUMENT;
            if (!e) {
                try {
                    p->st_mbs.resize(hdr.n_mbs);
                    p->st_events.resize(lens[i] * 16 / 3 + 16);
                } catch (const std::bad_alloc&) {
                    e = H263CU_ERR_OUT_OF_MEMORY;
                }
            }
            if (!e) {
                e = parse_picture_impl(p, packets[i], lens[i], stream_ids ? stream_ids[i] : i, 0, 0, 0, &p->st_pic,
                                       p->st_mbs.data(), (uint32_t)p->st_mbs.size(), p->st_events.data(),
                                       (uint32_t)p->st_events.size(), &pend[i]);
            }
            p->st_err = e;
        }
    };
    worker_pool().run(threads, work1);

    uint32_t np = 0, nm = 0, nu = 0;
    std::vector<uint32_t> mb_base(n), ev_base(n);
    std::vector<int32_t> packed(n, -1);
    for (uint32_t i = 0; i < n; i++) {
        h263cu_parser* p = parsers[i];
        if (!p) {
            if (per_pic_err) per_pic_err[i] = H263CU_ERR_BAD_ARGUMENT;
            continue;
        }
        if (per_pic_err) per_pic_err[i] = p->st_err;
        if (p->st_err) continue;
        if ((uint64_t)nm + p->st_pic.n_mbs > mb_cap || (uint64_t)nu + p->st_pic.n_event_units > ev_cap)
            return H263CU_ERR_CAPACITY;
        packed[i] = (int32_t)np;
        mb_base[i] = nm, ev_base[i] = nu;
        np++;
        nm += p->st_pic.n_mbs;
        nu += p->st_pic.n_event_units;
    }
    next.store(0);
    auto work2 = [&]() {
        for (;;) {
            uint32_t i = next.fetch_add(1);
            if (i >= n) break;
            if (packed[i] < 0) continue;
            h263cu_parser* p = parsers[i];
            h263cu_pic pc = p->st_pic;
            pc.first_mb = mb_base[i];
            pc.first_event = ev_base[i];
            pics[packed[i]] = pc;
            h263cu_mb* dst = mbs + mb_base[i];
            std::memcpy(dst, p->st_mbs.data(), (size_t)pc.n_mbs * sizeof(h263cu_mb));
            for (uint32_t k = 0; k < pc.n_mbs; k++) dst[k].pic = (uint16_t)packed[i];
            if (pc.n_event_units)
                std::memcpy(events + ev_base[i], p->st_events.data(), (size_t)pc.n_event_units * sizeof(h263cu_event));
            if (commit_now) {
                commit(p, pend[i]);
            } else {
                p->pending.valid = true;
                p->pending.has_last = pend[i].has_last, p->pending.has_reference = pend[i].has_reference;
                p->pending.fmt_kind = pend[i].fmt_kind, p->pending.w = pend[i].w, p->pending.h = pend[i].h;
                p->pending.ref_w = pend[i].ref_w, p->pending.ref_h = pend[i].ref_h;
            }
        }
    };
    worker_pool().run(threads, work2);
    if (pic_of_input) std::memcpy(pic_of_input, packed.data(), n * sizeof(int32_t));
    *n_pics_out = np;
    *n_mbs_out = nm;
    *n_units_out = nu;
    return 0;
}

int h263cu_parse_step(h263cu_parser* const* parsers, const uint8_t* const* packets, const size_t* lens,
                      const uint32_t* stream_ids, uint32_t n, int threads, h263cu_pic* pics, h263cu_mb* mbs,
                      uint32_t mb_cap, h263cu_event* events, uint32_t ev_cap, uint32_t* n_pics_out,
                      uint32_t* n_mbs_out, uint32_t* n_units_out, int* per_pic_err, int32_t* pic_of_input) {
    try {
        return parse_step_impl(parsers, packets, lens, stream_ids, n, threads, pics, mbs, mb_cap, events, ev_cap, n_pics_out,
                               n_mbs_out, n_units_out, per_pic_err, pic_of_input, true, 0, 0, nullptr);
    } catch (const std::bad_alloc&) {
        return H263CU_ERR_OUT_OF_MEMORY;
    }
}

int h263cu_test_read_bits(const uint8_t* data, size_t len, size_t* bitpos, int nbits, int is_signed, int peek, int64_t* value) {
    if (!data || !bitpos || !value || nbits < 0 || nbits > 32) return H263CU_ERR_BAD_ARGUMENT;
    BitReader r(data, len);
    if (*bitpos > len * 8) return H263CU_ERR_BAD_ARGUMENT;
    r.seek(*bitpos);
    if (nbits == 0) {
        *value = 0;
        return 0;
    }
    if (is_signed) {
        int32_t v;
        if (!r.read_signed((unsigned)nbits, &v)) return H263CU_ERR_UNHANDLED_IO_ERROR;
        *value = v;
    } else {
        uint32_t v;
        if (!r.read((unsigned)nbits, &v)) return H263CU_ERR_UNHANDLED_IO_ERROR;
        *value = v;
    }
    if (!peek) *bitpos = r.pos();
    return 0;
}

int h263cu_test_start_code(const uint8_t* data, size_t len, size_t bitpos, int* skipped) {
    if (!data || !skipped || bitpos > len * 8) return H263CU_ERR_BAD_ARGUMENT;
    BitReader r(data, len);
    r.seek(bitpos);
    uint32_t sk = 0;
    const int e = find_start_code(r, &sk);
    *skipped = e ? -1 : (int)sk;
    return e;
}

int h263cu_test_read_vlc(int table, const uint8_t* data, size_t len, size_t* bitpos, int* out4) {
    if (table < 0 || table > 4 || !data || !bitpos || !out4 || *bitpos > len * 8) return H263CU_ERR_BAD_ARGUMENT;
    BitReader r(data, len);
    r.seek(*bitpos);
    const VlcEntry* e;
    if (!r.read_vlc(vlc_table(table), &e)) return H263CU_ERR_UNHANDLED_IO_ERROR;
    *bitpos = r.pos();
    out4[0] = (int)e->kind(), out4[1] = e->a, out4[2] = e->b, out4[3] = e->c;
    return 0;
}

int h263cu_test_decode_block(const uint8_t* data, size_t len, size_t* bitpos, uint32_t decoder_options, int version, int is_intra,
                             int tcoef_present, int* intradc_code, int* n_events, uint8_t* run, int16_t* level, int* overflow) {
    if (!data || !bitpos || !intradc_code || !n_events || !run || !level || *bitpos > len * 8) return H263CU_ERR_BAD_ARGUMENT;
    BitReader r(data, len);
    r.seek(*bitpos);
    Header hd;
    hd.version = version;
    uint8_t ev_run[64];
    int16_t ev_level[64];
    bool ovf = false;
    const int e = parse_block(r, hd, decoder_options, is_intra != 0, tcoef_present != 0, intradc_code, ev_run, ev_level, n_events, &ovf);
    if (e) return e;
    for (int k = 0; k < *n_events; k++) run[k] = ev_run[k], level[k] = ev_level[k];
    if (overflow) *overflow = ovf;
    *bitpos = r.pos();
    return 0;
}

int h263cu_is_eof_error(int err) { return err == H263CU_ERR_UNHANDLED_IO_ERROR; }
int h263cu_is_macroblock_error(int err) {
    return err == H263CU_ERR_INVALID_MACROBLOCK_HEADER || err == H263CU_ERR_INVALID_MACROBLOCK_CODED_BITS;
}
int h263cu_is_gob_error(int err) { return err == H263CU_ERR_INVALID_GOB_HEADER; }

const char* h263cu_strerror(int err) {
    switch (err) {
        case H263CU_OK: return "ok";
        case H263CU_ERR_INTERNAL_DECODER_ERROR: return "the H.263 decoder failed internally, this is a bug";
        case H263CU_ERR_MIDDLE_OF_BITSTREAM: return "the H.263 bitstream doesn't start with a picture";
        case H263CU_ERR_INVALID_MACROBLOCK_HEADER: return "the H.263 bitstream contains an invalid macroblock header";
        case H263CU_ERR_INVALID_MACROBLOCK_CODED_BITS: return "the H.263 bitstream contains invalid macroblock coded bits";
        case H263CU_ERR_INVALID_INTRA_DC: return "the H.263 bitstream contains an invalid intra-dc coefficient";
        case H263CU_ERR_INVALID_SHORT_COEFFICIENT: return "the H.263 bitstream contains an invalid short ac coefficient";
        case H263CU_ERR_INVALID_LONG_COEFFICIENT: return "the H.263 bitstream contains an invalid long ac coefficient";
        case H263CU_ERR_INVALID_MVD: return "the H.263 bitstream contains an invalid motion vector";
        case H263CU_ERR_INVALID_PTYPE: return "the H.263 bitstream has an invalid picture type";
        case H263CU_ERR_INVALID_PLUSPTYPE: return "the H.263 bitstream has an invalid extension picture type";
        case H263CU_ERR_INVALID_GOB_HEADER: return "the H.263 bitstream has an invalid group-of-blocks header";
        case H263CU_ERR_INVALID_BITSTREAM: return "the H.263 bitstream could not be decoded";
// ... 49 lines not shown
```

h263_rs_b200/csrc/kernels.cu:

```cuda
#include "recon_common.cuh"

namespace h263dev {

template <bool YUV>
__global__ void __launch_bounds__(WARPS_PER_CTA * 32)
    recon_mb_kernel(const PicDev* __restrict__ pics, const h263cu_mb* __restrict__ mbs,
                    const h263cu_event* __restrict__ events, uint32_t n_mbs, int emit_rgba, const YuvDst yuv) {
    __shared__ WarpScratch scratch[WARPS_PER_CTA];
    __shared__ uint8_t s_dezigzag[64];
    if (threadIdx.x < 64) s_dezigzag[threadIdx.x] = c_dezigzag[threadIdx.x];
    __syncthreads();

    const int warp = threadIdx.x >> 5, lane = threadIdx.x & 31;
    const uint32_t mb_idx = blockIdx.x * WARPS_PER_CTA + warp;
    if (mb_idx >= n_mbs) return;
    WarpScratch& S = scratch[warp];

    const uint32_t* mw = reinterpret_cast<const uint32_t*>(mbs + mb_idx);
    const uint32_t mword = lane < 6 ? __ldg(mw + lane) : 0u;
    const uint32_t w0 = __shfl_sync(FULL, mword, 0), w1 = __shfl_sync(FULL, mword, 1);
    const uint32_t w2 = __shfl_sync(FULL, mword, 2), w3 = __shfl_sync(FULL, mword, 3);
    const uint32_t w4 = __shfl_sync(FULL, mword, 4), w5 = __shfl_sync(FULL, mword, 5);
    const PicDev& P = pics[w1 & 0xFFFFu];
    const int mbx = (w1 >> 16) & 0xFF, mby = w1 >> 24;
    const bool inter = (w2 & H263CU_MB_INTER) != 0;
    const bool wide = (w2 & H263CU_MB_WIDE) != 0;
    const int quant = (w2 >> 8) & 0xFF;
    const uint32_t c1 = (w2 >> 16) & 0xFF, c2 = c1 + (w2 >> 24), c3 = c2 + (w3 & 0xFF), c4 = c3 + ((w3 >> 8) & 0xFF),
                   c5 = c4 + ((w3 >> 16) & 0xFF), total = c5 + (w3 >> 24);
    const h263cu_event* ev = events + P.first_event + w0;

    uint32_t info[6] = {0, 0, 0, 0, 0, 0};
    const bool has_coefs = total > 0 || !inter;
    if (has_coefs) {
        float4* cz = reinterpret_cast<float4*>(S.coef);
        for (int i = lane; i < 6 * COEF_STRIDE / 4; i += 32) cz[i] = make_float4(0.f, 0.f, 0.f, 0.f);
        __syncwarp();
        const int first_idx = inter ? 0 : 1;
        if (total <= 32) {
            const bool active = (uint32_t)lane < total;
            const uint32_t e = (uint32_t)lane;
            const int b = (e >= c1) + (e >= c2) + (e >= c3) + (e >= c4) + (e >= c5);
            const int seg_start = b == 0 ? 0 : (b == 1 ? c1 : (b == 2 ? c2 : (b == 3 ? c3 : (b == 4 ? c4 : c5))));
            int run = 0, level = 1;
            if (active) load_event(ev, e, wide, run, level);
            int v = active ? run + 1 : 0;
#pragma unroll
            for (int d = 1; d < 32; d <<= 1) {
                int t = __shfl_up_sync(FULL, v, d);
                if (lane - d >= seg_start) v += t;
            }
            const int pos = first_idx + v - 1;
            const bool ok = active && pos < 64;
            const uint32_t ovf_ballot = __ballot_sync(FULL, active && pos >= 64);
            uint32_t bits = 0;
            if (ok) {
                const int lin = s_dezigzag[pos];
                S.coef[b * COEF_STRIDE + lin] = (float)dequant(level, quant);
                bits = (1u << (lin >> 3)) | ((lin & 7) ? INFO_COL : 0u);
            }
            const uint32_t cs[7] = {0, c1, c2, c3, c4, c5, total};
#pragma unroll
            for (int bb = 0; bb < 6; bb++) {
                uint32_t m = __reduce_or_sync(FULL, (ok && b == bb) ? bits : 0u);
                const uint64_t seg = ((1ull << cs[bb + 1]) - 1ull) ^ ((1ull << cs[bb]) - 1ull);
                if (ovf_ballot & (uint32_t)seg) m |= INFO_OVF;
                info[bb] = m;
            }
        } else {
            uint32_t mine = 0;
            if (lane < 6) {
                const uint32_t cs[7] = {0, c1, c2, c3, c4, c5, total};
                int idx = first_idx;
                for (uint32_t k = cs[lane]; k < cs[lane + 1]; k++) {
                    int run, level;
                    load_event(ev, k, wide, run, level);
                    idx += run;
                    if (idx >= 64) {
                        mine |= INFO_OVF;
                        break;
                    }
                    const int lin = s_dezigzag[idx];
                    S.coef[lane * COEF_STRIDE + lin] = (float)dequant(level, quant);
                    mine |= (1u << (lin >> 3)) | ((lin & 7) ? INFO_COL : 0u);
                    idx += 1;
                }
            }
#pragma unroll
            for (int bb = 0; bb < 6; bb++) info[bb] = __shfl_sync(FULL, mine, bb);
        }
        if (!inter) {
            uint32_t code = 0;
            if (lane < 6) code = lane < 4 ? byte_of(w4, lane) : byte_of(w5, lane - 4);
            uint32_t my_info = __shfl_sync(FULL, 0u, 0);
#pragma unroll
            for (int bb = 0; bb < 6; bb++)
                if (lane == bb) my_info = info[bb];
            const bool dc_ok = lane < 6 && code != 0 && !(my_info & INFO_OVF);
            if (dc_ok) S.coef[lane * COEF_STRIDE] = (float)intradc_level((int)code);
            const uint32_t dc_ballot = __ballot_sync(FULL, dc_ok);
#pragma unroll
            for (int bb = 0; bb < 6; bb++)
                if ((dc_ballot >> bb) & 1u) info[bb] |= INFO_DC;
        }
        __syncwarp();
    }

    int cls[6];
    int dcres[6];
#pragma unroll
    for (int bb = 0; bb < 6; bb++) {
        const uint32_t m = info[bb];
        const uint32_t rows_ev = m & INFO_ROWS;
        int c;
        if ((m & INFO_OVF) || !(m & (INFO_ROWS | INFO_DC)))
            c = CLS_ZERO;
        else if (!(rows_ev & 0xFEu) && !(m & INFO_COL))
            c = CLS_DC;
        else if (!(m & INFO_COL))
            c = CLS_VERT;
        else
            c = CLS_FULL;
        cls[bb] = c;
        dcres[bb] = 0;
        if (c == CLS_DC) dcres[bb] = round_residual_dc(S.coef[bb * COEF_STRIDE]);
    }

    {
        const int i = lane & 7, jg = lane >> 3;
        float bi[8], bj0[8], bj1[8];
#pragma unroll
        for (int k = 0; k < 8; k++) {
            bi[k] = c_basis[k][i];
            bj0[k] = c_basis[k][jg];
            bj1[k] = c_basis[k][jg + 4];
        }
#pragma unroll
        for (int bb = 0; bb < 6; bb++) {
            if (cls[bb] != CLS_FULL && cls[bb] != CLS_VERT) continue;
            const bool vert = cls[bb] == CLS_VERT;
            const uint32_t rows = (info[bb] & INFO_ROWS) | ((info[bb] & INFO_DC) ? 1u : 0u);
            const int n = __popc(rows);
            const float* cb = S.coef + bb * COEF_STRIDE;
            for (int base = 0; base < n; base += 4) {
                const int ridx = base + jg;
                if (ridx < n) {
                    const int y = __fns(rows, 0, ridx + 1);
                    float t;
                    if (vert) {
                        t = cb[y * 8];
                    } else {
                        const float4 ca = *reinterpret_cast<const float4*>(cb + y * 8);
                        const float4 cc = *reinterpret_cast<const float4*>(cb + y * 8 + 4);
                        t = 0.0f;
                        t = fadd(t, fmul(ca.x, bi[0]));
                        t = fadd(t, fmul(ca.y, bi[1]));
                        t = fadd(t, fmul(ca.z, bi[2]));
                        t = fadd(t, fmul(ca.w, bi[3]));
                        t = fadd(t, fmul(cc.x, bi[4]));
                        t = fadd(t, fmul(cc.y, bi[5]));
                        t = fadd(t, fmul(cc.z, bi[6]));
                        t = fadd(t, fmul(cc.w, bi[7]));
                    }
                    S.tbuf[y * 8 + i] = t;
                }
            }
            __syncwarp();
            float a0 = 0.0f, a1 = 0.0f;
#pragma unroll
            for (int y = 0; y < 8; y++) {
                if ((rows >> y) & 1u) {
                    const float tv = S.tbuf[y * 8 + i];
                    a0 = fadd(a0, fmul(tv, bj0[y]));
                    a1 = fadd(a1, fmul(tv, bj1[y]));
                }
            }
            const int r0 = vert ? round_residual_scaled(a0) : round_residual(a0);
            const int r1 = vert ? round_residual_scaled(a1) : round_residual(a1);
            S.res[bb][jg * 8 + i] = (int16_t)r0;
            S.res[bb][(jg + 4) * 8 + i] = (int16_t)r1;
            __syncwarp();
        }
    }

    const int mv0x = (int8_t)byte_of(w4, 0), mv0y = (int8_t)byte_of(w4, 1);
    const int mv1x = (int8_t)byte_of(w4, 2), mv1y = (int8_t)byte_of(w4, 3);
    const int mv2x = (int8_t)byte_of(w5, 0), mv2y = (int8_t)byte_of(w5, 1);
    const int mv3x = (int8_t)byte_of(w5, 2), mv3y = (int8_t)byte_of(w5, 3);
    {
        const int rowpix = lane >> 1, half = lane & 1;
        const int b = ((rowpix >> 3) << 1) | half, j = rowpix & 7;
        const int c = half ? (rowpix >= 8 ? cls[3] : cls[1]) : (rowpix >= 8 ? cls[2] : cls[0]);
        const int dcv = half ? (rowpix >= 8 ? dcres[3] : dcres[1]) : (rowpix >= 8 ? dcres[2] : dcres[0]);
        uint32_t p0 = 0, p1 = 0;
        if (inter && P.ref[0]) {
            const int mvx = half ? (rowpix >= 8 ? mv3x : mv1x) : (rowpix >= 8 ? mv2x : mv0x);
            const int mvy = half ? (rowpix >= 8 ? mv3y : mv1y) : (rowpix >= 8 ? mv2y : mv0y);
            mc_fetch8(P.ref[0], P.pitch_y, P.w, P.h, mbx * 16 + half * 8, mby * 16 + rowpix, mvx, mvy, p0, p1);
        }
        if (c == CLS_DC) {
            p0 = add_clamp4(p0, dcv, dcv, dcv, dcv);
            p1 = add_clamp4(p1, dcv, dcv, dcv, dcv);
        } else if (c != CLS_ZERO) {
            const int4 rv = *reinterpret_cast<const int4*>(&S.res[b][j * 8]);
            p0 = add_clamp4(p0, (int16_t)(rv.x & 0xFFFF), rv.x >> 16, (int16_t)(rv.y & 0xFFFF), rv.y >> 16);
            p1 = add_clamp4(p1, (int16_t)(rv.z & 0xFFFF), rv.z >> 16, (int16_t)(rv.w & 0xFFFF), rv.w >> 16);
        }
        *reinterpret_cast<uint2*>(P.cur[0] + (size_t)(mby * 16 + rowpix) * P.pitch_y + mbx * 16 + half * 8) =
            make_uint2(p0, p1);
        *reinterpret_cast<uint2*>(&S.rec[rowpix * 16 + half * 8]) = make_uint2(p0, p1);
    }
    if (lane < 16) {
        const int plane = lane >> 3, j = lane & 7, b = 4 + plane;
        const int c = plane ? cls[5] : cls[4];
        const int dcv = plane ? dcres[5] : dcres[4];
        uint32_t px[8] = {0, 0, 0, 0, 0, 0, 0, 0};
        if (inter && P.ref[1 + plane]) {
            const int cx = average_sum_of_mvs(mv0x + mv1x + mv2x + mv3x);
            const int cy = average_sum_of_mvs(mv0y + mv1y + mv2y + mv3y);
#pragma unroll
            for (int k = 0; k < 8; k++) px[k] = mc_fetch1(P.ref[1 + plane], P.pitch_c, CHROMA_STEP, P.cw, P.ch, mbx * 8 + k, mby * 8 + j, cx, cy);
        }
        uint32_t p0 = px[0] | (px[1] << 8) | (px[2] << 16) | (px[3] << 24), p1 = px[4] | (px[5] << 8) | (px[6] << 16) | (px[7] << 24);
        if (c == CLS_DC) {
            p0 = add_clamp4(p0, dcv, dcv, dcv, dcv);
            p1 = add_clamp4(p1, dcv, dcv, dcv, dcv);
        } else if (c != CLS_ZERO) {
            const int4 rv = *reinterpret_cast<const int4*>(&S.res[b][j * 8]);
            p0 = add_clamp4(p0, (int16_t)(rv.x & 0xFFFF), rv.x >> 16, (int16_t)(rv.y & 0xFFFF), rv.y >> 16);
            p1 = add_clamp4(p1, (int16_t)(rv.z & 0xFFFF), rv.z >> 16, (int16_t)(rv.w & 0xFFFF), rv.w >> 16);
        }
        uint8_t* dst = P.cur[1 + plane] + (size_t)(mby * 8 + j) * P.pitch_c + (size_t)(mbx * 8) * CHROMA_STEP;
#pragma unroll
        for (int k = 0; k < 4; k++) dst[k * CHROMA_STEP] = (uint8_t)byte_of(p0, k), dst[(k + 4) * CHROMA_STEP] = (uint8_t)byte_of(p1, k);
        *reinterpret_cast<uint2*>(&S.rec[256 + plane * 64 + j * 8]) = make_uint2(p0, p1);
    }

    if (YUV && emit_rgba && P.rgba) {
        __syncwarp();
        const uint32_t slot = P.rgba_row0 >> 12;
#pragma unroll
        for (int g = lane; g < 64; g += 32) {
            const int row = g >> 2, xq = g & 3;
            const int px = mbx * 16 + xq * 4, py = mby * 16 + row;
            if (py >= P.h) continue;
            store_word_cut(yuv_row(yuv, 0, slot, (uint32_t)py) + px, *reinterpret_cast<const uint32_t*>(&S.rec[row * 16 + xq * 4]),
                           P.w - px);
        }
        if (lane < 16) {
            const int row = lane >> 1, half = lane & 1;
            const int cx = mbx * 8 + half * 4, cy = mby * 8 + row, valid = P.cw - cx;
            if (cy < P.ch)
                store_chroma4_cut(yuv, slot, cy, cx, *reinterpret_cast<const uint32_t*>(&S.rec[256 + row * 8 + half * 4]),
                                  *reinterpret_cast<const uint32_t*>(&S.rec[320 + row * 8 + half * 4]), valid);
        }
    }

    if (!YUV && emit_rgba && P.rgba) {
        __syncwarp();
#pragma unroll
        for (int g = lane; g < 64; g += 32) {
            const int row = g >> 2, xq = g & 3;
            const int px = mbx * 16 + xq * 4, py = mby * 16 + row;
            if (px >= P.w || py >= P.h) continue;
            const uint32_t yw = *reinterpret_cast<const uint32_t*>(&S.rec[row * 16 + xq * 4]);
            const uint32_t cbp = *reinterpret_cast<const uint16_t*>(&S.rec[256 + (row >> 1) * 8 + xq * 2]);
            const uint32_t crp = *reinterpret_cast<const uint16_t*>(&S.rec[320 + (row >> 1) * 8 + xq * 2]);
            const ChromaTerms t0 = chroma_terms((int)(cbp & 0xFF), (int)(crp & 0xFF));
// ... 188 lines not shown
```

h263_rs_b200/csrc/recon_common.cuh:

```cuda
#pragma once
#include "device_math.cuh"
#include "kernels.cuh"

namespace h263dev {

static __constant__ float c_basis[8][8] = H263_BASIS_TABLE;
static __constant__ uint8_t c_dezigzag[64] = H263_DEZIGZAG_LINEAR;

constexpr int WARPS_PER_CTA = 8;
constexpr int COEF_STRIDE = 68;
constexpr unsigned FULL = 0xFFFFFFFFu;

enum { CLS_ZERO = 0, CLS_DC = 1, CLS_VERT = 3, CLS_FULL = 4 };

constexpr uint32_t INFO_ROWS = 0xFFu;
constexpr uint32_t INFO_COL = 0x100u;
constexpr uint32_t INFO_DC = 0x200u;
constexpr uint32_t INFO_OVF = 0x400u;

struct __align__(16) WarpScratch {
    float coef[6 * COEF_STRIDE];
    float tbuf[64];
    int16_t res[6][64];
    uint8_t rec[384];
};

__device__ __forceinline__ uint32_t byte_of(uint32_t w, int k) { return (w >> (8 * k)) & 0xFFu; }

__device__ __forceinline__ uint32_t add_clamp4(uint32_t pred, int r0, int r1, int r2, int r3) {
    uint32_t o0 = (uint32_t)clamp_u8((int)byte_of(pred, 0) + r0);
    uint32_t o1 = (uint32_t)clamp_u8((int)byte_of(pred, 1) + r1);
    uint32_t o2 = (uint32_t)clamp_u8((int)byte_of(pred, 2) + r2);
    uint32_t o3 = (uint32_t)clamp_u8((int)byte_of(pred, 3) + r3);
    return o0 | (o1 << 8) | (o2 << 16) | (o3 << 24);
}

__device__ __forceinline__ void mc_fetch8(const uint8_t* __restrict__ ref, int pitch, int W, int H, int x0, int y0,
                                          int mvx, int mvy, uint32_t& o0, uint32_t& o1) {
    const int dx = mvx >> 1, ix = mvx & 1, dy = mvy >> 1, iy = mvy & 1;
    const int sx = x0 + dx, sy = y0 + dy;
    uint32_t a0, a1, b0 = 0, b1 = 0, c0 = 0, c1 = 0, d0 = 0, d1 = 0;
    const bool inside = sx >= 0 && sy >= 0 && sx + 8 + ix <= W && sy + 1 + iy <= H;
    if (inside) {
        const int a = sx & 3;
        const uint32_t* wp = reinterpret_cast<const uint32_t*>(ref + (size_t)sy * pitch + (sx - a));
        const int sh = a * 8;
        uint32_t w0 = __ldg(wp), w1 = __ldg(wp + 1), w2 = __ldg(wp + 2);
        a0 = __funnelshift_r(w0, w1, sh);
        a1 = __funnelshift_r(w1, w2, sh);
        if (ix) {
            b0 = __funnelshift_rc(w0, w1, sh + 8);
            b1 = __funnelshift_rc(w1, w2, sh + 8);
        }
        if (iy) {
            const uint32_t* wq = wp + (pitch >> 2);
            uint32_t v0 = __ldg(wq), v1 = __ldg(wq + 1), v2 = __ldg(wq + 2);
            c0 = __funnelshift_r(v0, v1, sh);
            c1 = __funnelshift_r(v1, v2, sh);
            if (ix) {
                d0 = __funnelshift_rc(v0, v1, sh + 8);
                d1 = __funnelshift_rc(v1, v2, sh + 8);
            }
        }
    } else {
        uint32_t px[2][9];
#pragma unroll
        for (int r = 0; r < 2; r++) {
            const int cy = min(max(sy + r, 0), H - 1);
            const uint8_t* row = ref + (size_t)cy * pitch;
#pragma unroll
            for (int k = 0; k < 9; k++) px[r][k] = row[min(max(sx + k, 0), W - 1)];
        }
        a0 = px[0][0] | (px[0][1] << 8) | (px[0][2] << 16) | (px[0][3] << 24);
        a1 = px[0][4] | (px[0][5] << 8) | (px[0][6] << 16) | (px[0][7] << 24);
        b0 = px[0][1] | (px[0][2] << 8) | (px[0][3] << 16) | (px[0][4] << 24);
        b1 = px[0][5] | (px[0][6] << 8) | (px[0][7] << 16) | (px[0][8] << 24);
        c0 = px[1][0] | (px[1][1] << 8) | (px[1][2] << 16) | (px[1][3] << 24);
        c1 = px[1][4] | (px[1][5] << 8) | (px[1][6] << 16) | (px[1][7] << 24);
        d0 = px[1][1] | (px[1][2] << 8) | (px[1][3] << 16) | (px[1][4] << 24);
        d1 = px[1][5] | (px[1][6] << 8) | (px[1][7] << 16) | (px[1][8] << 24);
    }
    if (ix && iy) {
        o0 = avg4_u8x4(a0, b0, c0, d0);
        o1 = avg4_u8x4(a1, b1, c1, d1);
    } else if (ix) {
        o0 = avg2_u8x4(a0, b0);
        o1 = avg2_u8x4(a1, b1);
    } else if (iy) {
        o0 = avg2_u8x4(a0, c0);
        o1 = avg2_u8x4(a1, c1);
    } else {
        o0 = a0;
        o1 = a1;
    }
}

__device__ __forceinline__ uint32_t mc_fetch1(const uint8_t* __restrict__ ref, int pitch, int step, int W, int H, int x, int y,
                                              int mvx, int mvy) {
    const int sx = x + (mvx >> 1), sy = y + (mvy >> 1), ix = mvx & 1, iy = mvy & 1;
    const int x0 = min(max(sx, 0), W - 1), x1 = min(max(sx + 1, 0), W - 1);
    const int y0 = min(max(sy, 0), H - 1), y1 = min(max(sy + 1, 0), H - 1);
    const uint32_t a = ref[(size_t)y0 * pitch + x0 * step];
    if (ix && iy) {
        const uint32_t b = ref[(size_t)y0 * pitch + x1 * step], c = ref[(size_t)y1 * pitch + x0 * step],
                       d = ref[(size_t)y1 * pitch + x1 * step];
        return (a + b + c + d + 2u) >> 2;
    }
    if (ix) return (a + ref[(size_t)y0 * pitch + x1 * step] + 1u) >> 1;
    if (iy) return (a + ref[(size_t)y1 * pitch + x0 * step] + 1u) >> 1;
    return a;
}

__device__ __forceinline__ void load_event(const h263cu_event* __restrict__ ev, uint32_t idx, bool wide, int& run,
                                           int& level) {
    if (wide) {
        run = __ldg(ev + 2 * idx) & 63;
        level = (int16_t)__ldg(ev + 2 * idx + 1);
    } else {
        uint32_t u = __ldg(ev + idx);
        run = (int)(u >> 10);
        level = ((int)(u << 22)) >> 22;
    }
}


__device__ __forceinline__ void store_rgba_quad(uint8_t* dst, const uint4& o, int valid) {
    if (valid >= 4) {
        *reinterpret_cast<uint4*>(dst) = o;
    } else {
        uint32_t* d = reinterpret_cast<uint32_t*>(dst);
        d[0] = o.x;
        if (valid > 1) d[1] = o.y;
        if (valid > 2) d[2] = o.z;
    }
}

__device__ __forceinline__ void store_word_cut(uint8_t* dst, uint32_t v, int valid) {
    if (valid >= 4) {
        *reinterpret_cast<uint32_t*>(dst) = v;
    } else if (valid >= 2) {
        *reinterpret_cast<uint16_t*>(dst) = (uint16_t)v;
        if (valid > 2) dst[2] = (uint8_t)(v >> 16);
    } else if (valid == 1) {
        dst[0] = (uint8_t)v;
    }
}
__device__ __forceinline__ void store_pair_cut(uint8_t* dst, uint32_t v, int valid) {
    if (valid >= 2)
        *reinterpret_cast<uint16_t*>(dst) = (uint16_t)v;
    else if (valid == 1)
        dst[0] = (uint8_t)v;
}
__device__ __forceinline__ void store_chroma4_cut(const YuvDst& d, uint32_t slot, int cy, int cx, uint32_t cb, uint32_t cr, int valid) {
    if (d.nv12) {
        uint8_t* o = yuv_row(d, 1, slot, (uint32_t)cy) + 2 * cx;
        store_word_cut(o, __byte_perm(cb, cr, 0x5140), 2 * valid);
        store_word_cut(o + 4, __byte_perm(cb, cr, 0x7362), 2 * valid - 4);
    } else {
        store_word_cut(yuv_row(d, 1, slot, (uint32_t)cy) + cx, cb, valid);
        store_word_cut(yuv_row(d, 2, slot, (uint32_t)cy) + cx, cr, valid);
    }
}

}
```

h263_rs_b200/csrc/recon_tile.cu:

```cuda
#include "recon_common.cuh"

namespace h263dev {

namespace {

constexpr int WARP_MBS = 4;
#ifndef H263_STD_WARPS
#define H263_STD_WARPS 5
#endif
#ifndef H263_STD_CTAS
#define H263_STD_CTAS 7
#endif
constexpr int GEN_WARPS = 4, GEN_CTAS = 8;
#ifndef H263_ABLATE
#define H263_ABLATE 0
#endif
#ifndef H263_RGBA_TMA
#define H263_RGBA_TMA 1
#endif
#ifndef H263_RGBA_MODE
#define H263_RGBA_MODE 4
#endif
constexpr int WARP_BLOCKS = WARP_MBS * 6;
constexpr int RES_WORDS = 36;
constexpr int EV_CAP = 64;
constexpr int SLOT_FLOATS = 68;
constexpr int STAGE_BYTES = 4096;

constexpr uint32_t MBF_INTER = 1u << 0;
constexpr uint32_t MBF_LEFT = 1u << 2, MBF_RIGHT = 1u << 3, MBF_TOP = 1u << 4, MBF_BOTTOM = 1u << 5;
constexpr uint32_t MBF_RGBA = 1u << 6;
constexpr uint32_t BF_SLOW = 1u << 4;

struct __align__(16) WarpStage {
    uint32_t res[WARP_BLOCKS][RES_WORDS];
    uint32_t evbuf[EV_CAP];
    uint2 slotdesc[WARP_BLOCKS];
    uint32_t sstart[WARP_BLOCKS];
    uint32_t slotinfo[WARP_BLOCKS];
};
static_assert(sizeof(WarpStage) == STAGE_BYTES, "the RGBA tile aliases exactly this");

template <bool COMPACT>
struct WarpTailT;
template <>
struct __align__(16) WarpTailT<true> {
    float coef[4][SLOT_FLOATS];
    uint4 mba[WARP_MBS];
    uint32_t bd[WARP_BLOCKS];
    uint32_t meta[WARP_BLOCKS];
    uint8_t bf[WARP_BLOCKS];
    __device__ __forceinline__ uint32_t* mbrec() { return reinterpret_cast<uint32_t*>(&coef[0][0]); }
};
template <>
struct __align__(16) WarpTailT<false> {
    float coef[4][SLOT_FLOATS];
    uint4 mba[WARP_MBS];
    uint4 mbb[WARP_MBS];
    uint32_t bd[WARP_BLOCKS];
    uint32_t meta[WARP_BLOCKS];
    uint32_t mbrec_[WARP_BLOCKS];
    uint8_t bf[WARP_BLOCKS];
    __device__ __forceinline__ uint32_t* mbrec() { return mbrec_; }
};

template <bool COMPACT, int NW>
struct TileSmemT {
    WarpStage stage[NW];
    WarpTailT<COMPACT> tail[NW];
};
static_assert(sizeof(TileSmemT<true, H263_STD_WARPS>) <= 200704 / H263_STD_CTAS - 1024, "shared memory budget of the standard instantiations");
static_assert(sizeof(TileSmemT<false, GEN_WARPS>) <= 200704 / GEN_CTAS - 1024, "shared memory budget of the generic instantiations");

__device__ const float g_basis[8][8] = H263_BASIS_TABLE;
__device__ const uint8_t g_dezigzag[64] = H263_DEZIGZAG_LINEAR;

__device__ __forceinline__ constexpr float k_basis(int y, int j) {
    constexpr float T[8][8] = H263_BASIS_TABLE;
    return T[y][j];
}

__device__ __forceinline__ int dequant_narrow(int level, int q2, int qc) {
    const int mag = q2 * abs(level) + qc;
    const int v = level < 0 ? -mag : mag;
    return max(min(v, 2047), -2048);
}

__device__ __forceinline__ int round_q(float q, float m) { return __float2int_rz(fadd(fmul(q, m), copysign_half(q))); }

struct RowSum {
    uint32_t lo, hi;
};
__device__ __forceinline__ RowSum row_sum4(uint32_t w0, uint32_t w1, int sh, int shb) {
    const uint32_t a = __funnelshift_r(w0, w1, sh), b = __funnelshift_rc(w0, w1, shb);
    RowSum h;
    h.hi = __byte_perm(a, 0, 0x4341) + __byte_perm(b, 0, 0x4341);
    h.lo = (a + b) - 256u * h.hi;
    return h;
}
__device__ __forceinline__ uint32_t vmix(uint32_t top, uint32_t bottom, uint32_t wt, uint32_t wb) {
    return __byte_perm(top * wt + (bottom * wb + 0x00800080u), 0, 0x4341);
}

#if H263_RGBA_MODE == 0 || H263_RGBA_MODE == 3
__device__ __forceinline__ uint32_t pack_sat(int a, int b, uint32_t c) {
    uint32_t d;
    asm("cvt.pack.sat.u8.s32.b32 %0, %1, %2, %3;" : "=r"(d) : "r"(a), "r"(b), "r"(c));
    return d;
}
#endif
struct CT {
    int r, g, b;
};
__device__ __forceinline__ int opaque(int v) {
    asm("" : "+r"(v));
    return v;
}
#if H263_RGBA_MODE == 0 || H263_RGBA_MODE == 3
__device__ __forceinline__ CT chroma_terms_folded(int cb, int cr, int kr, int kg, int kb) {
    CT t;
    t.r = cr * kr + (32768 - 128 * 104597 - 16 * 76309);
    t.g = cr * kg + (cb * -25675 + (32768 + 128 * 53279 + 128 * 25675 - 16 * 76309));
    t.b = cb * kb + (32768 - 128 * 132201 - 16 * 76309);
    return t;
}
#else
__device__ __forceinline__ CT chroma_terms_folded(int cb, int cr, int kr, int kg, int kb) {
    CT t;
    t.r = cr * kr + (0xFFFFFF - (32768 - 128 * 104597 - 16 * 76309));
    t.g = cr * kg + (cb * 25675 + (0xFFFFFF - (32768 + 128 * 53279 + 128 * 25675 - 16 * 76309)));
    t.b = cb * kb + (0xFFFFFF - (32768 - 128 * 132201 - 16 * 76309));
#if H263_RGBA_MODE == 4
    t.g = cr * (kg - kr) + (cb * 25675 + ((32768 - 128 * 104597) - (32768 + 128 * 53279 + 128 * 25675)));
    t.b = cb * kb + (cr * -kr + ((32768 - 128 * 104597) - (32768 - 128 * 132201)));
#endif
    return t;
}
#endif
#if H263_RGBA_MODE == 0
__device__ __forceinline__ uint32_t rgba_px(uint32_t yw, int k, int ky, const CT& t) {
    const int y = (int)(__byte_perm(yw, 0, 0x4440 + k));
    const int r = (y * ky + t.r) >> 16, g = (y * ky + t.g) >> 16, b = (y * ky + t.b) >> 16;
    return pack_sat(g, r, pack_sat(255, b, 0));
}
#elif H263_RGBA_MODE == 3
__device__ __forceinline__ uint32_t rgba_px(uint32_t yw, int k, int ky, const CT& t) {
    const int y = (int)__dp4a(yw, 1u << (8 * k), 0u);
    const int r = __dp2a_hi(y * ky + t.r, 0x01000000, 0), g = __dp2a_hi(y * ky + t.g, 0x01000000, 0), b = __dp2a_hi(y * ky + t.b, 0x01000000, 0);
    return pack_sat(g, r, pack_sat(255, b, 0));
}
#else
__device__ __forceinline__ uint32_t rgba_px(uint32_t yw, int k, int ky, const CT& t) {
#if H263_RGBA_MODE == 1
    const int y = (int)(__byte_perm(yw, 0, 0x4440 + k));
#else
    const int y = (int)__dp4a(yw, 1u << (8 * k), 0u);
#endif
#if H263_RGBA_MODE == 4
    const int xr = y * ky + t.r;
    const uint32_t wr = (uint32_t)__vimin_s32_relu(xr, 0xFFFFFF), wg = (uint32_t)__viaddmin_s32_relu(xr, t.g, 0xFFFFFF),
                   wb = (uint32_t)__viaddmin_s32_relu(xr, t.b, 0xFFFFFF);
#else
    const int nyk = opaque(y * ky);
    const uint32_t wr = (uint32_t)__viaddmin_s32_relu(nyk, t.r, 0xFFFFFF), wg = (uint32_t)__viaddmin_s32_relu(nyk, t.g, 0xFFFFFF),
                   wb = (uint32_t)__viaddmin_s32_relu(nyk, t.b, 0xFFFFFF);
#endif
    const uint32_t rg = __byte_perm(wr, wg, 0x3362);
    uint32_t px;
    asm("lop3.b32 %0, %1, %2, 0xFFFF0000, 0x07;" : "=r"(px) : "r"(rg), "r"(wb));
    return px;
}
#endif

__device__ __forceinline__ uint32_t scan_up_step(uint32_t v, int d) {
    asm volatile("{ .reg .pred p; .reg .b32 t; shfl.sync.up.b32 t|p, %0, %1, 0, 0xffffffff; @p add.u32 %0, %0, t; }" : "+r"(v) : "r"(d));
    return v;
}
__device__ __forceinline__ int seg_scan_up_step(int v, int d, int dist) {
    asm volatile("{ .reg .pred p; .reg .b32 t; shfl.sync.up.b32 t, %0, %1, 0, 0xffffffff; setp.ge.s32 p, %2, %1; @p add.s32 %0, %0, t; }"
                 : "+r"(v)
                 : "r"(d), "r"(dist));
    return v;
}

__device__ __forceinline__ uint32_t mad_pack(uint32_t o, uint32_t e) { return o * 256u + e; }

__device__ __forceinline__ uint32_t merge_bytes(uint32_t a, uint32_t b, int keep) {
    const uint32_t m = keep >= 4 ? 0xFFFFFFFFu : ((1u << (8 * keep)) - 1u);
    return (a & m) | (b & ~m);
}

__device__ __forceinline__ uint32_t stage_offset(int q, int row, int c) { return (uint32_t)(q * 1024 + row * 64 + c * 16); }

}


template <int PY, int PC, int PR, bool EDGE, bool WIDE_MV, int NW, int NCTAS, int OUT>
__global__ void __launch_bounds__(NW * 32, NCTAS)
    recon_tile_kernel(const PicDev* __restrict__ pics, const h263cu_mb* __restrict__ mbs,
                      const h263cu_event* __restrict__ events, uint32_t n_mbs, int emit_rgba, const Pools pools,
                      const __grid_constant__ CUtensorMap rgba_map, const YuvDst yuv) {
    constexpr bool COMPACT = PY != 0 && !EDGE && !WIDE_MV;
    constexpr int CTA_WARPS = NW;
    __shared__ __align__(1024) TileSmemT<COMPACT, NW> S;
    const int tid = threadIdx.x, lane = tid & 31, warp = tid >> 5;
    WarpStage& G = S.stage[warp];
    WarpTailT<COMPACT>& W = S.tail[warp];
    uint32_t* const mbrec = W.mbrec();
    const int g = lane >> 3, t = lane & 7;
    const uint32_t lt_mask = (1u << lane) - 1u;

    const uint32_t n_tiles = (n_mbs + WARP_MBS - 1) / WARP_MBS;
    const uint32_t tile = blockIdx.x * CTA_WARPS + warp;
    if (tile >= n_tiles) return;
    const uint32_t mb0 = tile * WARP_MBS;
    const int n_w = (int)min((uint32_t)WARP_MBS, n_mbs - mb0);

    if (lane < n_w * 6) mbrec[lane] = __ldg(reinterpret_cast<const uint32_t*>(mbs) + (size_t)tile * WARP_BLOCKS + lane);
    __syncwarp();
    int n_slots;
    {
        const bool bvalid = lane < n_w * 6;
        const int bm = bvalid ? (lane * 43) >> 8 : 0, bb = bvalid ? lane - bm * 6 : 0;
        const uint32_t* r = &mbrec[bm * 6];
        const uint32_t w0 = r[0], w1 = r[1], w2 = r[2], w3 = r[3], w4 = r[4], w5 = r[5];
        const uint32_t pic = w1 & 0xFFFFu;
        const PicDev& P = pics[pic];
        const int mbx = (w1 >> 16) & 0xFF, mby = w1 >> 24;
        const bool inter = (w2 & H263CU_MB_INTER) != 0, wide = (w2 & H263CU_MB_WIDE) != 0;
        const uint32_t nev = bvalid ? __byte_perm(w2, w3, 0x4440u + (uint32_t)bb + 2u) & 0xFFu : 0u;
        const uint32_t code = inter ? 0u : __byte_perm(w4, w5, 0x4440u + (uint32_t)bb) & 0xFFu;

        uint32_t boff = 0, bflags = 0;
        if (inter) {
            int mvx, mvy, bx, sy, pitch;
            uint32_t base;
            bool in_range;
            if (bb < 4) {
                const int m = (int)((bb < 2 ? w4 : w5) >> (16 * (bb & 1)));
                mvx = __dp4a(m, 0x00000001, 0), mvy = __dp4a(m, 0x00000100, 0);
                in_range = mvx >= -32 && mvx <= 31 && mvy >= -32 && mvy <= 31;
                bx = mbx * 16 + (bb & 1) * 8 + (mvx >> 1), sy = mby * 16 + (bb >> 1) * 8 + (mvy >> 1);
                pitch = PY ? PY : P.pitch_y, base = P.ref_y4;
            } else {
                const int sx = __dp4a((int)w5, 0x00010001, __dp4a((int)w4, 0x00010001, 13));
                const int sy13 = __dp4a((int)w5, 0x01000100, __dp4a((int)w4, 0x01000100, 13));
                mvx = (sx >> 4) + ((sx - 11) >> 4), mvy = (sy13 >> 4) + ((sy13 - 11) >> 4);
                in_range = mvx >= -16 && mvx <= 15 && mvy >= -16 && mvy <= 15;
                bx = 2 * (mbx * 8 + (mvx >> 1)), sy = mby * 8 + (mvy >> 1);
                pitch = PC ? PC : P.pitch_c, base = P.ref_c4;
            }
            const int a = bx & 3;
            boff = base + (uint32_t)((sy * pitch + (bx - a)) >> 2);
            bflags = (uint32_t)(a | ((mvx & 1) << 2) | ((mvy & 1) << 3)) | (!WIDE_MV || in_range ? 0u : BF_SLOW);
        }
        if (bvalid) {
            W.bd[lane] = boff;
            W.bf[lane] = (uint8_t)bflags;
            if (bb == 0) {
                const int pitch_y = PY ? PY : P.pitch_y, pitch_c = PC ? PC : P.pitch_c;
                const int mbw = (P.w + 15) >> 4, mbh = (P.h + 15) >> 4;
                const uint32_t ed = EDGE ? ((uint32_t)(P.w & 15) | ((uint32_t)(P.h & 15) << 4) | ((uint32_t)(P.cw & 7) << 8) |
                                            ((uint32_t)(P.ch & 7) << 12))
                                         : 0u;
                uint32_t flags = inter ? MBF_INTER : 0u;
                if (mbx == 0) flags |= MBF_LEFT;
                if (mbx == mbw - 1) flags |= MBF_RIGHT;
                if (mby == 0) flags |= MBF_TOP;
                if (mby == mbh - 1) flags |= MBF_BOTTOM;
                if (emit_rgba && P.rgba) flags |= MBF_RGBA;
                W.mba[bm] = make_uint4(P.cur_y4 + (uint32_t)((mby * 16 * pitch_y + mbx * 16) >> 2),
                                       P.cur_c4 + (uint32_t)((mby * 8 * pitch_c + mbx * 16) >> 2), P.rgba_row0 + (uint32_t)(mby * 16),
                                       flags | ((uint32_t)mbx << 8));
                if constexpr (!COMPACT) W.mbb[bm] = make_uint4((uint32_t)pitch_y | ((uint32_t)pitch_c << 16), 0u, pic, ed);
            }
        }

        const bool coded = nev > 0;
        const uint32_t coded_mask = __ballot_sync(FULL, coded);
        const int pos = __popc(coded_mask & lt_mask);
        n_slots = __popc(coded_mask);
        uint32_t ev_incl = nev;
#pragma unroll
        for (int d = 1; d < 32; d <<= 1) ev_incl = scan_up_step(ev_incl, d);
        const uint32_t before = (ev_incl - nev) - __shfl_sync(FULL, ev_incl - nev, bm * 6);
        if (coded) {
            G.sstart[pos] = ev_incl - nev;
            const uint32_t first = P.first_event + w0 + (wide ? 2 * before : before);
            const uint32_t quant = (w2 >> 8) & 31u;
            G.slotdesc[pos] = make_uint2(first, nev | (quant << 8) | (wide ? 1u << 13 : 0u) | (inter ? 1u << 14 : 0u) |
                                                    (bb >= 4 ? 1u << 15 : 0u) | ((uint32_t)lane << 16) | (code << 24));
            asm volatile("prefetch.global.L1 [%0];" ::"l"(events + first));
        } else if (bvalid) {
            const bool has_dc = code != 0;
            const int dcres = has_dc ? round_residual_dc((float)intradc_level((int)code)) : 0;
            W.meta[lane] = (uint32_t)(has_dc ? CLS_DC : CLS_ZERO) | ((uint32_t)dcres << 16);
        }
    }
    __syncwarp();


    {
        const float* const basis = &g_basis[0][0];
        const float bt0 = basis[0 * 8 + t], bt1 = basis[1 * 8 + t], bt2 = basis[2 * 8 + t], bt3 = basis[3 * 8 + t],
                    bt4 = basis[4 * 8 + t], bt5 = basis[5 * 8 + t], bt6 = basis[6 * 8 + t], bt7 = basis[7 * 8 + t];
        float* c = W.coef[g];
        const int tperm = (t & 4) | ((t & 1) << 1) | ((t >> 1) & 1);
        if (H263_ABLATE & 1) n_slots = 0;
        const bool is_slot = lane < n_slots;
        const uint2 my_sd = is_slot ? G.slotdesc[lane] : make_uint2(0u, 0u);
        const uint32_t my_start = is_slot ? G.sstart[lane] : 0xFFFFFFFFu;
        const uint32_t my_end = my_start + (my_sd.y & 0xFFu);
        int s_lo = 0;
        uint32_t e_lo = 0;
        while (s_lo < n_slots) {
            const int s_hi = max(s_lo + 1, s_lo + __popc(__ballot_sync(FULL, is_slot && lane >= s_lo && my_end - e_lo <= (uint32_t)EV_CAP)));
            const bool in_chunk = lane >= s_lo && lane < s_hi;
            const uint32_t e_end = __shfl_sync(FULL, my_end, s_hi - 1);
            const uint32_t e_hi = min(e_end, e_lo + (uint32_t)EV_CAP);
            if (in_chunk) G.slotinfo[lane] = 0u;
            __syncwarp();

            uint32_t carry = 0;
            for (uint32_t eb = e_lo; eb < e_hi; eb += 32) {
                const uint32_t e = eb + lane;
                const bool act = e < e_hi;
                const bool head = in_chunk && my_start >= eb && my_start < eb + 32;
                const uint32_t heads = __reduce_or_sync(FULL, head ? 1u << (my_start - eb) : 0u);
                const int n_before = __popc(__ballot_sync(FULL, in_chunk && my_start < eb));
                const uint32_t below = heads & (0xFFFFFFFFu >> (31 - lane));
                const int slot = s_lo + n_before - 1 + __popc(below);
                const int seg = below ? 31 - __clz(below) : -1;
                int v = 0, val = 0;
                bool inter = false;
                if (act) {
                    const uint2 sd = G.slotdesc[slot];
                    const uint32_t k = e - G.sstart[slot];
                    const int quant = (int)((sd.y >> 8) & 31u);
                    inter = (sd.y >> 14) & 1u;
                    int run;
                    if (!((sd.y >> 13) & 1u)) {
                        const uint32_t u = __ldg(events + sd.x + k);
                        run = (int)(u >> 10);
                        val = dequant_narrow(((int)(u << 22)) >> 22, 2 * quant, quant - 1 + (quant & 1));
                    } else {
                        run = __ldg(events + sd.x + 2 * k) & 63;
                        val = dequant((int16_t)__ldg(events + sd.x + 2 * k + 1), quant);
                    }
                    v = run + 1;
                }
                const int dist = lane - max(seg, 0);
#pragma unroll
                for (int d = 1; d < 32; d <<= 1) v = seg_scan_up_step(v, d, dist);
                if (seg < 0) v += (int)carry;
                carry = (uint32_t)__shfl_sync(FULL, v, 31);
                if (act) {
                    const int idx = (inter ? 0 : 1) + v - 1;
                    uint32_t bits, ent;
                    if (idx < 64) {
                        const int lin = g_dezigzag[idx];
                        ent = (uint32_t)lin | ((uint32_t)val << 16);
                        bits = (1u << (lin >> 3)) | ((lin & 7) ? 0x100u : 0u);
                    } else {
                        ent = 0x8000u;
                        bits = 0x200u;
                    }
                    G.evbuf[e - e_lo] = ent;
                    atomicOr(&G.slotinfo[slot], bits);
                }
            }
            __syncwarp();

            int key = 4;
            uint32_t pd = 0u;
            if (in_chunk) {
                const uint32_t info = G.slotinfo[lane];
                const bool inter = (my_sd.y >> 14) & 1u;
                const uint32_t blk = (my_sd.y >> 16) & 0xFFu, code = my_sd.y >> 24;
                const bool ovf = (info & 0x200u) != 0, col = (info & 0x100u) != 0;
                const uint32_t rows = info & 0xFFu;
                const bool has_dc = !inter && code != 0 && !ovf;
                int cls, dcres = 0;
                uint32_t R = 0;
                if (ovf || (!rows && !has_dc)) {
                    cls = CLS_ZERO;
                } else if (!(rows & 0xFEu) && !col) {
                    cls = CLS_DC;
                    const int dc = has_dc ? intradc_level((int)code) : (int)G.evbuf[my_start - e_lo] >> 16;
                    dcres = round_residual_dc((float)dc);
                } else {
                    cls = col ? CLS_FULL : CLS_VERT;
                    R = rows | (has_dc ? 1u : 0u);
                }
                W.meta[blk] = (uint32_t)cls | ((uint32_t)lane << 3) | ((uint32_t)dcres << 16);
                pd = (uint32_t)lane | (R << 5) | (cls == CLS_VERT ? 1u << 13 : 0u) | (has_dc ? 1u << 14 : 0u) | ((my_start - e_lo) << 15) |
                     ((my_sd.y & 0xFFu) << 22) | ((my_sd.y & 0x8000u) << 15);
                const int n = __popc(R);
                key = n >= 4 ? 0 : (n >= 2 ? 1 : (n == 1 ? 2 : 3));
            }
            int pos = s_lo, n_need = 0;
#pragma unroll
            for (int j = 0; j < 3; j++) {
                const uint32_t b = __ballot_sync(FULL, key == j);
                if (j < key) pos += __popc(b);
                if (j == key) pos += __popc(b & lt_mask);
                n_need += __popc(b);
            }
            __syncwarp();
            if (key < 3) G.slotinfo[pos] = pd;
            __syncwarp();

            for (int si0 = s_lo; si0 < s_lo + n_need; si0 += 4) {
                const int si = si0 + g;
                const bool valid = si < s_lo + n_need;
                const uint32_t pd = valid ? G.slotinfo[si] : 0u;
                const int sl = (int)(pd & 31u);
                const uint32_t R = (pd >> 5) & 0xFFu;
                const bool vert = (pd >> 13) & 1u;
                const int nev = (int)((pd >> 22) & 0xFFu);
                const uint32_t first = (pd >> 15) & 127u;
                *reinterpret_cast<float4*>(c + t * 8) = make_float4(0.f, 0.f, 0.f, 0.f);
                *reinterpret_cast<float4*>(c + t * 8 + 4) = make_float4(0.f, 0.f, 0.f, 0.f);
                const int nevmax = __reduce_max_sync(FULL, nev);
                __syncwarp();
                if (t < nev) {
                    const uint32_t ent = G.evbuf[first + t];
                    c[ent & 63u] = (float)((int)ent >> 16);
                }
                if (nevmax > 8) {
                    for (int k = t + 8; k < nev; k += 8) {
                        const uint32_t ent = G.evbuf[first + k];
                        c[ent & 63u] = (float)((int)ent >> 16);
                    }
                }
                if (pd & 0x4000u) {
                    if (t == 0) c[0] = (float)intradc_level((int)(G.slotdesc[sl].y >> 24));
                }
                const uint32_t U = __reduce_or_sync(FULL, R);
                __syncwarp();
                float acc[8] = {0.f, 0.f, 0.f, 0.f, 0.f, 0.f, 0.f, 0.f};
#pragma unroll
                for (int y = 0; y < 8; y++) {
                    if (!((U >> y) & 1u)) continue;
                    const float4 ca = *reinterpret_cast<const float4*>(c + y * 8);
                    const float4 cc = *reinterpret_cast<const float4*>(c + y * 8 + 4);
                    float a = fmul(ca.x, bt0);
                    a = fadd(a, fmul(ca.y, bt1));
                    a = fadd(a, fmul(ca.z, bt2));
                    a = fadd(a, fmul(ca.w, bt3));
                    a = fadd(a, fmul(cc.x, bt4));
                    a = fadd(a, fmul(cc.y, bt5));
                    a = fadd(a, fmul(cc.z, bt6));
                    a = fadd(a, fmul(cc.w, bt7));
                    if (vert) a = ca.x;
                    a = fmul(a, 0.25f);
#pragma unroll
                    for (int j = 0; j < 8; j++) acc[j] = fadd(acc[j], fmul(a, k_basis(y, j)));
                }
                const bool any_vert = __any_sync(FULL, vert);
                if (R) {
                    uint16_t* rrow = reinterpret_cast<uint16_t*>(&G.res[sl][0]) + ((pd & 0x40000000u) ? t : tperm);
                    if (any_vert) {
                        const float m = vert ? H263_B00 : 1.0f;
#pragma unroll
                        for (int j = 0; j < 8; j++) rrow[j * 8] = (uint16_t)(int16_t)round_q(acc[j], m);
                    } else {
#pragma unroll
                        for (int j = 0; j < 8; j++) rrow[j * 8] = (uint16_t)(int16_t)__float2int_rz(fadd(acc[j], copysign_half(acc[j])));
                    }
                }
                __syncwarp();
            }
            s_lo = s_hi;
            e_lo = e_end;
        }
    }

    {
        const int mbq = lane >> 3, rgrp = (lane >> 2) & 1, cg = lane & 3;
        const bool unit_ok = mbq < n_w;
        const int mbi = unit_ok ? mbq : 0;
        const uint4 ma = W.mba[mbi];
        uint4 mv = make_uint4(0u, (ma.w >> 8) & 0xFFu, 0u, 0u);
        if constexpr (!COMPACT) {
            const uint4 b = W.mbb[mbi];
            mv.x = b.x, mv.z = b.z, mv.w = b.w;
        }
        const uint32_t flags = (unit_ok ? ma.w : 0u) & ~((H263_ABLATE & 2) ? MBF_INTER : 0u) & ~((H263_ABLATE & 4) ? MBF_RGBA : 0u);
        const uint32_t pitch_y4 = PY ? PY / 4 : (mv.x & 0xFFFFu) >> 2, pitch_c4 = PC ? PC / 4 : mv.x >> 18;
        const int lb = rgrp * 2 + (cg >> 1);
        const int bl = mbi * 6 + lb, bc = mbi * 6 + 4;

        uint32_t ylo[8], yhi[8];
        uint32_t cbp[4], crp[4];
        if (flags & MBF_INTER) {
            const uint32_t fl = W.bf[bl], fc = W.bf[bc];
            if (!WIDE_MV || !(fl & BF_SLOW)) {
                const int sh = (fl & 3u) * 8, shb = sh + ((fl & 4u) << 1);
                const uint32_t wb = ((fl >> 3) & 1u) * 64u, wt = 128u - wb;
                const bool second = (fl & 7u) != 0;
                const uint32_t* src = reinterpret_cast<const uint32_t*>(pools.y) + W.bd[bl] + (uint32_t)(cg & 1);
                RowSum hs[9];
#pragma unroll
                for (int r = 0; r < 9; r++) {
                    const uint32_t* p = src + (uint32_t)r * pitch_y4;
                    uint32_t w0 = 0u, w1 = 0u;
                    if (r < 8 || wb != 0) {
                        w0 = __ldg(p);
                        if (second) w1 = __ldg(p + 1);
                    }
                    hs[r] = row_sum4(w0, w1, sh, shb);
                }
#pragma unroll
                for (int r = 0; r < 8; r++) {
                    ylo[r] = vmix(hs[r].lo, hs[r + 1].lo, wt, wb);
                    yhi[r] = vmix(hs[r].hi, hs[r + 1].hi, wt, wb);
                }
            } else {
                const PicDev& P = pics[mv.z];
                const uint32_t* rr = &mbrec[mbi * 6];
                const uint32_t w1 = rr[1];
                const uint32_t mvw = lb < 2 ? (rr[4] >> (16 * lb)) : (rr[5] >> (16 * (lb - 2)));
                const int mvx = (int8_t)(mvw & 0xFF), mvy = (int8_t)((mvw >> 8) & 0xFF);
                const int x0 = (int)((w1 >> 16) & 0xFF) * 16 + cg * 4, y0 = (int)(w1 >> 24) * 16 + rgrp * 8;
#pragma unroll
                for (int r = 0; r < 8; r++) {
                    uint32_t s[4];
#pragma unroll
                    for (int k = 0; k < 4; k++) s[k] = mc_fetch1(P.ref[0], P.pitch_y, 1, P.w, P.h, x0 + k, y0 + r, mvx, mvy);
                    ylo[r] = s[0] | (s[2] << 16), yhi[r] = s[1] | (s[3] << 16);
                }
            }
            if (!WIDE_MV || !(fc & BF_SLOW)) {
                const int sh = (fc & 3u) * 8, shb = sh + ((fc & 4u) << 2);
                const uint32_t wb = ((fc >> 3) & 1u) * 64u, wt = 128u - wb;
                const bool second = (fc & 7u) != 0;
                const uint32_t* src = reinterpret_cast<const uint32_t*>(pools.c) + W.bd[bc] + (uint32_t)cg + (uint32_t)(rgrp * 4) * pitch_c4;
                RowSum hs[5];
#pragma unroll
// ... 344 lines not shown
```

h263_rs_b200/frontend.py:

```python
import ctypes as C

import numpy as np

from . import _lib
from ._lib import Mb, Pic, check

MB_DTYPE = np.dtype(
    {
        "names": ["ev_off", "pic", "mbx", "mby", "flags", "quant", "nev", "u"],
        "formats": ["<u4", "<u2", "u1", "u1", "u1", "u1", ("u1", 6), ("u1", 8)],
        "offsets": [0, 4, 6, 7, 8, 9, 10, 16],
        "itemsize": 24,
    }
)
PIC_DTYPE = np.dtype(
    {
        "names": ["stream", "width", "height", "mb_w", "mb_h", "pic_type", "pquant", "flags", "version",
                  "temporal_reference", "first_mb", "n_mbs", "first_event", "n_event_units"],
        "formats": ["<u4", "<u2", "<u2", "u1", "u1", "u1", "u1", "u1", "u1", "<u2", "<u4", "<u4", "<u4", "<u4"],
        "offsets": [0, 4, 6, 8, 9, 10, 11, 12, 13, 14, 16, 20, 24, 28],
        "itemsize": 32,
    }
)


class Parser:

    def __init__(self, options=_lib.OPT_SORENSON):
        self.L = _lib.lib()
        self.options = options
        self.h = self.L.h263cu_parser_create(options)
        if not self.h:
            raise MemoryError

    def __del__(self):
        if getattr(self, "h", None):
            self.L.h263cu_parser_destroy(self.h)
            self.h = None

    def reset(self):
        self.L.h263cu_parser_reset(self.h)

    def parse_picture(self, packet: bytes, stream=0, pic_index=0, mb_base=0, ev_base=0):
        hdr = Pic()
        check(self.L.h263cu_peek_picture(self.options, packet, len(packet), C.byref(hdr)))
        n_mbs = max(int(hdr.n_mbs), 1)
        mbs = np.zeros(n_mbs, MB_DTYPE)
        ev_cap = len(packet) * 16 // 3 + 16
        events = np.zeros(ev_cap, np.uint16)
        pic = np.zeros(1, PIC_DTYPE)
        check(
            self.L.h263cu_parse_picture(
                self.h, packet, len(packet), stream, pic_index, mb_base, ev_base,
                C.cast(pic.ctypes.data, C.POINTER(Pic)), mbs.ctypes.data, n_mbs, events.ctypes.data, ev_cap,
            )
        )
        return pic, mbs[: int(pic["n_mbs"][0])], events[: int(pic["n_event_units"][0])]


def peek_picture(packet: bytes, options=_lib.OPT_SORENSON):
    pic = np.zeros(1, PIC_DTYPE)
    check(_lib.lib().h263cu_peek_picture(options, packet, len(packet), C.cast(pic.ctypes.data, C.POINTER(Pic))))
    return pic[0]


def decode_events(mb, events, ev_base=0):
    out = []
    off = ev_base + int(mb["ev_off"])
    wide = bool(mb["flags"] & _lib.MB_WIDE)
    for b in range(6):
        blk = []
        for _ in range(int(mb["nev"][b])):
            if wide:
                run = int(events[off]) & 63
                level = int(np.int16(events[off + 1]))
                off += 2
            else:
                u = int(events[off])
                run = u >> 10
                level = u & 0x3FF
                if level >= 512:
                    level -= 1024
                off += 1
            blk.append((run, level))
        out.append(blk)
    return out


def parse_step(parsers, packets, stream_ids=None, threads=0, mb_cap=None, ev_cap=None, pinned=None):
    L = _lib.lib()
    n = len(parsers)
    assert len(packets) == n
    hp = (C.c_void_p * n)(*[p.h for p in parsers])
    bufs = [np.frombuffer(pk, np.uint8) for pk in packets]
    pp = (C.c_void_p * n)(*[b.ctypes.data for b in bufs])
    lens = (C.c_size_t * n)(*[len(pk) for pk in packets])
    sid = None
    if stream_ids is not None:
        sid = np.ascontiguousarray(stream_ids, np.uint32)
    if mb_cap is None:
        mb_cap = 0
        for pk, p in zip(packets, parsers):
            try:
                mb_cap += int(peek_picture(pk, p.options)["n_mbs"])
            except _lib.H263Error:
                pass
        mb_cap = max(mb_cap, 1)
    if ev_cap is None:
        ev_cap = sum(len(pk) for pk in packets) * 16 // 3 + 16 * n
    pics = np.zeros(n, PIC_DTYPE)
    mbs = np.zeros(mb_cap, MB_DTYPE)
    events = np.zeros(ev_cap, np.uint16)
    errs = np.zeros(n, np.int32)
    pic_of = np.zeros(n, np.int32)
    npics, nm, nu = C.c_uint32(), C.c_uint32(), C.c_uint32()
    check(
        L.h263cu_parse_step(
            hp, pp, lens, sid.ctypes.data if sid is not None else None, n, threads, pics.ctypes.data,
            mbs.ctypes.data, mb_cap, events.ctypes.data, ev_cap, C.byref(npics), C.byref(nm), C.byref(nu),
            errs.ctypes.data, pic_of.ctypes.data,
        )
    )
    return pics[: npics.value], mbs[: nm.value], events[: nu.value], errs, pic_of
```

include/h263cu.h:

```cpp
#ifndef H263CU_H
#define H263CU_H

#include <stddef.h>
#include <stdint.h>

#ifdef __cplusplus
extern "C" {
#endif

#define H263CU_OK 0
#define H263CU_ERR_INTERNAL_DECODER_ERROR (-1)
#define H263CU_ERR_MIDDLE_OF_BITSTREAM (-2)
#define H263CU_ERR_INVALID_MACROBLOCK_HEADER (-3)
#define H263CU_ERR_INVALID_MACROBLOCK_CODED_BITS (-4)
#define H263CU_ERR_INVALID_INTRA_DC (-5)
#define H263CU_ERR_INVALID_SHORT_COEFFICIENT (-6)
#define H263CU_ERR_INVALID_LONG_COEFFICIENT (-7)
#define H263CU_ERR_INVALID_MVD (-8)
#define H263CU_ERR_INVALID_PTYPE (-9)
#define H263CU_ERR_INVALID_PLUSPTYPE (-10)
#define H263CU_ERR_INVALID_GOB_HEADER (-11)
#define H263CU_ERR_INVALID_BITSTREAM (-12)
#define H263CU_ERR_PICTURE_FORMAT_MISSING (-13)
#define H263CU_ERR_PICTURE_FORMAT_INVALID (-14)
#define H263CU_ERR_UNCODED_IFRAME_BLOCKS (-15)
#define H263CU_ERR_UNHANDLED_IO_ERROR (-16)
#define H263CU_ERR_UNIMPLEMENTED_DECODING (-17)
#define H263CU_ERR_BAD_ARGUMENT (-100)
#define H263CU_ERR_CUDA (-101)
#define H263CU_ERR_NO_DEVICE (-102)
#define H263CU_ERR_CAPACITY (-103)
#define H263CU_ERR_REFERENCE_WOULD_ABORT (-104)
#define H263CU_ERR_NO_PICTURE (-105)
#define H263CU_ERR_OUT_OF_MEMORY (-106)

int h263cu_is_eof_error(int err);
int h263cu_is_macroblock_error(int err);
int h263cu_is_gob_error(int err);
const char* h263cu_strerror(int err);
int h263cu_version(void);

#define H263CU_OPT_SORENSON_SPARK_BITSTREAM 1u
#define H263CU_OPT_USE_SCALABILITY_MODE 2u
#define H263CU_OPT_DECODE_DISPOSABLE 0x100u


#define H263CU_PIC_I 0
#define H263CU_PIC_P 1
#define H263CU_PIC_DISPOSABLE_P 2
#define H263CU_PIC_OTHER 3

#define H263CU_PICFLAG_DEBLOCK 1u
#define H263CU_PICFLAG_HAS_INTER 2u
#define H263CU_PICFLAG_MV_IN_RANGE 4u
#define H263CU_PICFLAG_DISPOSABLE 8u

typedef struct h263cu_pic {
    uint32_t stream;
    uint16_t width, height;
    uint8_t mb_w, mb_h;
    uint8_t pic_type;
    uint8_t pquant;
    uint8_t flags;
    uint8_t version;
    uint16_t temporal_reference;
    uint32_t first_mb;
    uint32_t n_mbs;
    uint32_t first_event;
    uint32_t n_event_units;
} h263cu_pic;

#define H263CU_MB_INTER 1u
#define H263CU_MB_WIDE 2u
#define H263CU_MB_FOURMV 4u
#define H263CU_MB_CODED 8u

typedef struct h263cu_mb {
    uint32_t ev_off;
    uint16_t pic;
    uint8_t mbx, mby;
    uint8_t flags;
    uint8_t quant;
    uint8_t nev[6];
    union {
        int8_t mv[4][2];
        uint8_t intradc[6];
    } u;
} h263cu_mb;

typedef uint16_t h263cu_event;

typedef struct h263cu_parser h263cu_parser;

h263cu_parser* h263cu_parser_create(uint32_t decoder_options);
void h263cu_parser_destroy(h263cu_parser*);
uint32_t h263cu_parser_options(const h263cu_parser*);
void h263cu_parser_reset(h263cu_parser*);

int h263cu_peek_picture(uint32_t decoder_options, const uint8_t* data, size_t len, h263cu_pic* pic);

int h263cu_parse_picture(h263cu_parser*, const uint8_t* data, size_t len, uint32_t stream,
                         uint16_t pic_index, uint32_t mb_base, uint32_t ev_base, h263cu_pic* pic,
                         h263cu_mb* mbs, uint32_t mb_cap, h263cu_event* events, uint32_t ev_cap);

int h263cu_parse_step(h263cu_parser* const* parsers, const uint8_t* const* packets, const size_t* lens,
                      const uint32_t* stream_ids, uint32_t n, int threads, h263cu_pic* pics,
                      h263cu_mb* mbs, uint32_t mb_cap, h263cu_event* events, uint32_t ev_cap,
                      uint32_t* n_pics_out, uint32_t* n_mbs_out, uint32_t* n_units_out,
                      int* per_pic_err, int32_t* pic_of_input);

int h263cu_test_read_bits(const uint8_t* data, size_t len, size_t* bitpos, int nbits, int is_signed, int peek,
                          int64_t* value);
int h263cu_test_start_code(const uint8_t* data, size_t len, size_t bitpos, int* skipped);
int h263cu_test_read_vlc(int table, const uint8_t* data, size_t len, size_t* bitpos, int* out4);
int h263cu_test_decode_block(const uint8_t* data, size_t len, size_t* bitpos, uint32_t decoder_options, int version,
                             int is_intra, int tcoef_present, int* intradc_code, int* n_events, uint8_t* run,
                             int16_t* level, int* overflow);

typedef struct h263cu_ctx h263cu_ctx;
typedef struct h263cu_step h263cu_step;

#define H263CU_OUT_RGBA 1u
#define H263CU_OUT_DEBLOCK 2u

int h263cu_device_count(void);
h263cu_ctx* h263cu_create(int device, uint32_t max_streams, uint32_t max_width, uint32_t max_height,
                          uint32_t flags, int* err);
void h263cu_destroy(h263cu_ctx*);
int h263cu_device_of(h263cu_ctx*);

void* h263cu_alloc_pinned(size_t bytes);
void h263cu_free_pinned(void* p);

h263cu_step* h263cu_step_upload(h263cu_ctx*, const h263cu_pic* pics, uint32_t n_pics, const h263cu_mb* mbs,
                                uint32_t n_mbs, const h263cu_event* events, uint32_t n_units, int* err);
void h263cu_step_free(h263cu_ctx*, h263cu_step*);
int h263cu_step_run(h263cu_ctx*, h263cu_step*, uint32_t out_flags);
typedef struct h263cu_graph h263cu_graph;
h263cu_graph* h263cu_graph_build(h263cu_ctx*, h263cu_step* const* steps, uint32_t n_steps, uint32_t out_flags, int* err);
int h263cu_graph_launch(h263cu_ctx*, h263cu_graph*);
void h263cu_graph_free(h263cu_ctx*, h263cu_graph*);
int h263cu_submit_step(h263cu_ctx*, const h263cu_pic* pics, uint32_t n_pics, const h263cu_mb* mbs,
                       uint32_t n_mbs, const h263cu_event* events, uint32_t n_units, uint32_t out_flags);
int h263cu_submit_step_readback(h263cu_ctx*, const h263cu_pic* pics, uint32_t n_pics, const h263cu_mb* mbs,
                                uint32_t n_mbs, const h263cu_event* events, uint32_t n_units,
                                uint32_t out_flags, uint8_t* host_rgba, const uint64_t* rgba_offsets);
int h263cu_decode_step(h263cu_ctx*, h263cu_parser* const* parsers, const uint8_t* const* packets, const size_t* lens,
                       const uint32_t* stream_ids, uint32_t n, int threads, uint32_t out_flags, uint8_t* host_rgba,
                       uint64_t rgba_stride, int* per_pic_err, uint32_t* n_decoded);

typedef struct h263cu_device_rgba {
    uint8_t* base;
    uint64_t row_pitch;
    uint64_t pic_stride;
    uint32_t width, height;
    void* stream;
} h263cu_device_rgba;
int h263cu_decode_step_device(h263cu_ctx*, h263cu_parser* const* parsers, const uint8_t* const* packets, const size_t* lens,
                              const uint32_t* stream_ids, uint32_t n, int threads, uint32_t out_flags, const h263cu_device_rgba* out,
                              int* per_pic_err, uint32_t* n_decoded);

#define H263CU_YUV_I420 0u
#define H263CU_YUV_NV12 1u
typedef struct h263cu_device_plane {
    uint8_t* base;
    uint64_t row_pitch;
    uint64_t pic_stride;
} h263cu_device_plane;
typedef struct h263cu_device_yuv {
    h263cu_device_plane plane[3];
    uint32_t width, height;
    uint32_t format;
    uint32_t reserved;
    void* stream;
} h263cu_device_yuv;
int h263cu_decode_step_device_yuv(h263cu_ctx*, h263cu_parser* const* parsers, const uint8_t* const* packets, const size_t* lens,
                                  const uint32_t* stream_ids, uint32_t n, int threads, uint32_t out_flags, const h263cu_device_yuv* out,
                                  int* per_pic_err, uint32_t* n_decoded);

#define H263CU_TENSOR_U8 0u
#define H263CU_TENSOR_F32 1u
#define H263CU_TENSOR_F16 2u
#define H263CU_TENSOR_BF16 3u
typedef struct h263cu_device_tensor {
    void* base;
    int64_t stride[4];
    uint32_t width, height;
    uint32_t dtype;
    uint32_t reserved;
    float mul[3], add[3];
    void* stream;
} h263cu_device_tensor;
int h263cu_decode_step_device_tensor(h263cu_ctx*, h263cu_parser* const* parsers, const uint8_t* const* packets, const size_t* lens,
                                     const uint32_t* stream_ids, uint32_t n, int threads, uint32_t out_flags,
                                     const h263cu_device_tensor* out, int* per_pic_err, uint32_t* n_decoded);

#define H263CU_FIT_STRETCH 0u
#define H263CU_FIT_LETTERBOX 1u
#define H263CU_FIT_CENTER_CROP 2u
typedef struct h263cu_tensor_crop {
    uint32_t x, y, width, height;
} h263cu_tensor_crop;
typedef struct h263cu_tensor_fit {
    uint32_t mode;
    uint32_t short_side;
    float fill[3];
    uint32_t reserved;
    const h263cu_tensor_crop* crops;
} h263cu_tensor_fit;
int h263cu_decode_step_device_tensor_fit(h263cu_ctx*, h263cu_parser* const* parsers, const uint8_t* const* packets,
                                         const size_t* lens, const uint32_t* stream_ids, uint32_t n, int threads, uint32_t out_flags,
                                         const h263cu_device_tensor* out, const h263cu_tensor_fit* fit, int* per_pic_err,
                                         uint32_t* n_decoded);
int h263cu_test_fit_geometry(uint32_t mode, uint32_t short_side, uint32_t cw, uint32_t ch, uint32_t width, uint32_t height,
                             int32_t* out4);

#define H263CU_FILTER_BILINEAR 0u
#define H263CU_FILTER_BILINEAR_AA 1u
#define H263CU_FILTER_BICUBIC_AA 2u
int h263cu_decode_step_device_tensor_filter(h263cu_ctx*, h263cu_parser* const* parsers, const uint8_t* const* packets,
                                            const size_t* lens, const uint32_t* stream_ids, uint32_t n, int threads, uint32_t out_flags,
                                            const h263cu_device_tensor* out, const h263cu_tensor_fit* fit, uint32_t filter,
                                            int* per_pic_err, uint32_t* n_decoded);
int h263cu_sync(h263cu_ctx*);
int h263cu_readback_wait(h263cu_ctx*, uint32_t age);

typedef struct h263cu_group h263cu_group;
h263cu_group* h263cu_group_create(const int* devices, uint32_t n_devices, uint32_t streams_per_device, uint32_t max_width,
// ... 66 lines not shown
```

Before: 468,000.

## Emit dezigzagged coefficient positions from parser instead of run lengths

The CPU parser now writes each coefficient event's linear (dezigzagged) position rather than its zigzag run. The GPU recon kernels drop the warp segmented prefix scan, the dezigzag table lookup and overflow handling. Externally supplied run-form side info is validated and converted to position form on the host with a small thread pool into pinned buffers. This moves per-event index computation off the GPU critical path, at the cost of extra host work and a new flag that every consumer of the format must handle.

```diff
diff --git a/bindings/h263cu-sys/src/lib.rs b/bindings/h263cu-sys/src/lib.rs
--- a/bindings/h263cu-sys/src/lib.rs
+++ b/bindings/h263cu-sys/src/lib.rs
@@ -43,6 +43,7 @@
 pub const H263CU_MB_WIDE: u8 = 2;
 pub const H263CU_MB_FOURMV: u8 = 4;
 pub const H263CU_MB_CODED: u8 = 8;
+pub const H263CU_MB_POS: u8 = 16;
 pub const H263CU_OUT_RGBA: u32 = 1;
 pub const H263CU_OUT_DEBLOCK: u32 = 2;
 pub const H263CU_YUV_I420: u32 = 0;
diff --git a/h263_rs_b200/_lib.py b/h263_rs_b200/_lib.py
--- a/h263_rs_b200/_lib.py
+++ b/h263_rs_b200/_lib.py
@@ -19,7 +19,7 @@
 OUT_DEBLOCK = 2
 
 PIC_I, PIC_P, PIC_DISPOSABLE_P, PIC_OTHER = 0, 1, 2, 3
-MB_INTER, MB_WIDE, MB_FOURMV, MB_CODED = 1, 2, 4, 8
+MB_INTER, MB_WIDE, MB_FOURMV, MB_CODED, MB_POS = 1, 2, 4, 8, 16
 
 
 class Pic(C.Structure):
diff --git a/h263_rs_b200/csrc/context.cu b/h263_rs_b200/csrc/context.cu
--- a/h263_rs_b200/csrc/context.cu
+++ b/h263_rs_b200/csrc/context.cu
@@ -7,7 +7,9 @@
 #include <cstdlib>
 #include <cstring>
 #include <mutex>
+#include <atomic>
 #include <new>
+#include <thread>
 #include <vector>
 
 #include "device_math.cuh"
@@ -86,6 +88,10 @@
     uint32_t n_mbs = 0, n_units = 0;
     size_t mb_cap = 0, ev_cap = 0;
     uint32_t max_w = 0, max_h = 0;
+    h263cu_mb* h_mbs = nullptr;
+    h263cu_event* h_events = nullptr;
+    size_t h_mb_cap = 0, h_ev_cap = 0;
+    cudaEvent_t h_copied = nullptr;
 };
 
 struct h263cu_ctx {
@@ -394,7 +400,21 @@
     return 0;
 }
 
-int validate_side_info(std::vector<h263cu_pic>& pics, const h263cu_mb* mbs, uint32_t n_mbs, uint32_t n_units) {
+const uint8_t* zigzag_index() {
+    static const struct Table {
+        uint8_t z[64];
+        Table() {
+            const uint8_t dz[64] = H263_DEZIGZAG_LINEAR;
+            for (int i = 0; i < 64; i++) z[dz[i]] = (uint8_t)i;
+        }
+    } t;
+    return t.z;
+}
+
+int validate_side_info(std::vector<h263cu_pic>& pics, const h263cu_mb* mbs, uint32_t n_mbs, const h263cu_event* events,
+                       uint32_t n_units, bool* run_form) {
+    const uint8_t* zz = zigzag_index();
+    *run_form = false;
     for (size_t i = 0; i < pics.size(); i++) {
         h263cu_pic& p = pics[i];
         if ((uint64_t)p.first_mb + p.n_mbs > n_mbs || (uint64_t)p.first_event + p.n_event_units > n_units ||
@@ -404,14 +424,28 @@
         const h263cu_mb* m = mbs + p.first_mb;
         for (uint32_t k = 0; k < p.n_mbs; k++, m++) {
             if (m->pic != i || (uint32_t)m->mby * p.mb_w + m->mbx != k || m->mbx >= p.mb_w) return H263CU_ERR_BAD_ARGUMENT;
-            const bool intra = !(m->flags & H263CU_MB_INTER);
+            const bool intra = !(m->flags & H263CU_MB_INTER), wide = (m->flags & H263CU_MB_WIDE) != 0;
             uint32_t ev = 0;
             for (int b = 0; b < 6; b++) {
                 if (m->nev[b] > (intra ? 63 : 64) || (intra && m->nev[b] && m->u.intradc[b] == 0)) return H263CU_ERR_BAD_ARGUMENT;
                 ev += m->nev[b];
             }
-            if (m->flags & H263CU_MB_WIDE) ev *= 2;
+            if (wide) ev *= 2;
             if ((uint64_t)m->ev_off + ev > p.n_event_units) return H263CU_ERR_BAD_ARGUMENT;
+            if (m->flags & H263CU_MB_POS) {
+                const h263cu_event* u = events + p.first_event + m->ev_off;
+                for (int b = 0; b < 6; b++) {
+                    int last = intra ? 0 : -1;
+                    for (uint32_t n = m->nev[b]; n; n--) {
+                        const uint32_t pos = wide ? u[0] : (uint32_t)u[0] >> 10;
+                        u += wide ? 2 : 1;
+                        if (pos >= 64 || (int)zz[pos] <= last) return H263CU_ERR_BAD_ARGUMENT;
+                        last = zz[pos];
+                    }
+                }
+            } else {
+                *run_form = true;
+            }
             if (m->flags & H263CU_MB_INTER) {
                 any_inter = true;
                 for (int b = 0; b < 4; b++)
@@ -421,6 +455,105 @@
         if (any_inter) p.flags |= H263CU_PICFLAG_HAS_INTER;
         if (!in_range) p.flags &= (uint8_t)~H263CU_PICFLAG_MV_IN_RANGE;
     }
+    return 0;
+}
+
+template <typename T>
+int grow_pinned(T** p, size_t* cap, size_t need) {
+    if (need <= *cap) return 0;
+    if (*p) cudaFreeHost(*p);
+    *p = nullptr, *cap = 0;
+    const size_t n = need + need / 4 + 64;
+    CU_TRY(cudaHostAlloc((void**)p, n * sizeof(T), cudaHostAllocDefault));
+    *cap = n;
+    return 0;
+}
+
+int rewrite_run_form(h263cu_step* s, const h263cu_mb* mbs, uint32_t n_mbs, const h263cu_event* events, uint32_t* n_units) {
+    std::vector<h263cu_pic>& pics = s->pics;
+    std::vector<uint64_t> start;
+    try {
+        start.resize(pics.size() + 1);
+    } catch (const std::bad_alloc&) {
+        return H263CU_ERR_OUT_OF_MEMORY;
+    }
+    uint64_t need = 0;
+    for (size_t i = 0; i < pics.size(); i++) {
+        start[i] = need;
+        const h263cu_pic& p = pics[i];
+        for (uint32_t k = 0; k < p.n_mbs; k++) {
+            const h263cu_mb& m = mbs[p.first_mb + k];
+            const uint32_t ev = (uint32_t)m.nev[0] + m.nev[1] + m.nev[2] + m.nev[3] + m.nev[4] + m.nev[5];
+            need += (m.flags & H263CU_MB_WIDE) ? 2 * ev : ev;
+        }
+    }
+    start[pics.size()] = need;
+    if (need + 8 >= 0xFFFFFFFFu) return H263CU_ERR_CAPACITY;
+    if (s->h_copied) CU_TRY(cudaEventSynchronize(s->h_copied));
+    int e;
+    if ((e = grow_pinned(&s->h_mbs, &s->h_mb_cap, n_mbs)) || (e = grow_pinned(&s->h_events, &s->h_ev_cap, (size_t)need + 8))) return e;
+    std::memcpy(s->h_mbs, mbs, (size_t)n_mbs * sizeof(h263cu_mb));
+    auto one = [&](size_t i) {
+        static const uint8_t dz[64] = H263_DEZIGZAG_LINEAR;
+        h263cu_pic& p = pics[i];
+        h263cu_event* const first = s->h_events + start[i];
+        h263cu_event* o = first;
+        for (uint32_t k = 0; k < p.n_mbs; k++) {
+            h263cu_mb& m = s->h_mbs[p.first_mb + k];
+            const bool intra = !(m.flags & H263CU_MB_INTER), wide = (m.flags & H263CU_MB_WIDE) != 0;
+            const bool run = !(m.flags & H263CU_MB_POS);
+            const h263cu_event* u = events + p.first_event + m.ev_off;
+            m.ev_off = (uint32_t)(o - first);
+            m.flags |= H263CU_MB_POS;
+            for (int b = 0; b < 6; b++) {
+                const int n = m.nev[b];
+                if (!run) {
+                    const int w = wide ? 2 * n : n;
+                    std::memcpy(o, u, (size_t)w * sizeof(h263cu_event));
+                    o += w, u += w;
+                    continue;
+                }
+                h263cu_event* const bstart = o;
+                int idx = intra ? 1 : 0;
+                bool dropped = false;
+                for (int j = 0; j < n; j++) {
+                    idx += wide ? (u[0] & 63) : (u[0] >> 10);
+                    if (idx >= 64) {
+                        dropped = true;
+                        break;
+                    }
+                    if (wide) {
+                        *o++ = dz[idx], *o++ = u[1], u += 2;
+                    } else {
+                        *o++ = (h263cu_event)(((uint32_t)dz[idx] << 10) | (u[0] & 0x3FFu)), u += 1;
+                    }
+                    idx++;
+                }
+                if (dropped) {
+                    u += (size_t)(wide ? 2 : 1) * (size_t)n - (size_t)(o - bstart);
+                    o = bstart;
+                    m.nev[b] = 0;
+                    if (intra) m.u.intradc[b] = 0;
+                }
+            }
+        }
+        p.first_event = (uint32_t)start[i];
+        p.n_event_units = (uint32_t)(o - first);
+    };
+    std::atomic<size_t> next{0};
+    auto work = [&] {
+        for (size_t i; (i = next.fetch_add(1)) < pics.size();) one(i);
+    };
+    const size_t n_threads = std::min<size_t>(std::min<size_t>(std::max(1u, std::thread::hardware_concurrency()), 16),
+                                              (pics.size() + 63) / 64);
+    std::vector<std::thread> pool;
+    try {
+        for (size_t t = 1; t < n_threads; t++) pool.emplace_back(work);
+    } catch (...) {
+    }
+    work();
+    for (std::thread& th : pool) th.join();
+    *n_units = (uint32_t)need;
     return 0;
 }
 
@@ -433,28 +566,28 @@
     } catch (const std::bad_alloc&) {
         return H263CU_ERR_OUT_OF_MEMORY;
     }
-    s->n_mbs = n_mbs, s->n_units = n_units;
-    if (!trusted && (e = validate_side_info(s->pics, mbs, n_mbs, n_units))) {
+    bool run_form = false;
+    if (!trusted && (e = validate_side_info(s->pics, mbs, n_mbs, events, n_units, &run_form)) == 0 && run_form &&
+        (e = rewrite_run_form(s, mbs, n_mbs, events, &n_units)) == 0) {
+        mbs = s->h_mbs, events = s->h_events;
+        e = step_reserve(s, n_mbs, n_units);
+    }
+    if (e) {
         s->pics.clear();
         return e;
     }
+    s->n_mbs = n_mbs, s->n_units = n_units;
     if (n_mbs) CU_TRY(cudaMemcpyAsync(s->d_mbs, mbs, (size_t)n_mbs * sizeof(h263cu_mb), cudaMemcpyHostToDevice, stream));
     if (n_units)
         CU_TRY(cudaMemcpyAsync(s->d_events, events, (size_t)n_units * sizeof(h263cu_event), cudaMemcpyHostToDevice, stream));
+    if (run_form) {
+        if (!s->h_copied) CU_TRY(cudaEventCreateWithFlags(&s->h_copied, cudaEventDisableTiming));
+        CU_TRY(cudaEventRecord(s->h_copied, stream));
+    }
     (void)c;
     return 0;
 }
 
-template <typename T>
-int grow_pinned(T** p, size_t* cap, size_t need) {
-    if (need <= *cap) return 0;
-    if (*p) cudaFreeHost(*p);
-    *p = nullptr, *cap = 0;
-    const size_t n = need + need / 4 + 64;
-    CU_TRY(cudaHostAlloc((void**)p, n * sizeof(T), cudaHostAllocDefault));
-    *cap = n;
-    return 0;
-}
 typedef CUresult (*EncodeTiled)(CUtensorMap*, CUtensorMapDataType, cuuint32_t, void*, const cuuint64_t*, const cuuint64_t*,
                                 const cuuint32_t*, const cuuint32_t*, CUtensorMapInterleave, CUtensorMapSwizzle,
                                 CUtensorMapL2promotion, CUtensorMapFloatOOBfill);
@@ -577,6 +710,11 @@
     if (s->d_events) cudaFree(s->d_events);
     s->d_mbs = nullptr, s->d_events = nullptr;
     s->mb_cap = s->ev_cap = 0;
+    if (s->h_copied) cudaEventSynchronize(s->h_copied), cudaEventDestroy(s->h_copied);
+    if (s->h_mbs) cudaFreeHost(s->h_mbs);
+    if (s->h_events) cudaFreeHost(s->h_events);
+    s->h_copied = nullptr, s->h_mbs = nullptr, s->h_events = nullptr;
+    s->h_mb_cap = s->h_ev_cap = 0;
 }
 
 }
diff --git a/h263_rs_b200/csrc/frontend.cpp b/h263_rs_b200/csrc/frontend.cpp
--- a/h263_rs_b200/csrc/frontend.cpp
+++ b/h263_rs_b200/csrc/frontend.cpp
@@ -11,6 +11,7 @@
 
 #include "../../include/h263cu.h"
 #include "bitio.hpp"
+#include "device_math.cuh"
 
 namespace h263fe {
 
@@ -316,8 +317,11 @@
     return 0;
 }
 
+static const uint8_t kDezigzag[64] = H263_DEZIGZAG_LINEAR;
+
 static H263_AI int parse_block_fast(BitReader& r, const uint32_t* __restrict tf, int tf_bits, bool sorenson_v1, bool intra, bool coded,
-                                    int* dc_code, h263cu_event* __restrict out, int* nev, bool* overflow, bool* wide) {
+                                    int* dc_code, h263cu_event* __restrict out, int* nev, bool* overflow, bool* wide,
+                                    bool positions) {
     uint32_t v;
     *dc_code = -1;
     *nev = 0;
@@ -366,7 +370,7 @@
         if (__builtin_expect(idx >= 64, 0))
             ovf = true;
         else if (!ovf)
-            out[n++] = (h263cu_event)unit;
+            out[n++] = (h263cu_event)(positions ? ((uint32_t)kDezigzag[idx] << 10) | (unit & 0x3FFu) : unit);
         idx += 1;
         if (last) break;
     }
@@ -377,7 +381,8 @@
 
 static int parse_picture_impl(h263cu_parser* p, const uint8_t* data, size_t len, uint32_t stream, uint16_t pic_index,
                               uint32_t mb_base, uint32_t ev_base, h263cu_pic* pic, h263cu_mb* mbs, uint32_t mb_cap,
-                              h263cu_event* events, uint32_t ev_cap, PendingState* pending) {
+                              h263cu_event* events, uint32_t ev_cap, PendingState* pending, bool positions) {
+    const uint8_t pos_flag = positions ? H263CU_MB_POS : 0;
     BitReader r0(data, len);
     Header hd;
     int e = parse_header(r0, p->options, p->has_last, p->last_fmt_kind, p->last_w, p->last_h, &hd);
@@ -528,7 +533,7 @@
                 m.ev_off = ev_used;
                 m.pic = pic_index;
                 m.mbx = (uint8_t)col, m.mby = (uint8_t)row;
-                m.flags = H263CU_MB_INTER;
+                m.flags = H263CU_MB_INTER | pos_flag;
                 m.quant = (uint8_t)quant;
                 any_inter = true;
             }
@@ -583,7 +588,7 @@
         m.pic = pic_index;
         m.mbx = (uint8_t)col, m.mby = (uint8_t)row;
         m.quant = (uint8_t)quant;
-        m.flags = (uint8_t)(H263CU_MB_CODED | (intra ? 0 : H263CU_MB_INTER) |
+        m.flags = (uint8_t)(H263CU_MB_CODED | pos_flag | (intra ? 0 : H263CU_MB_INTER) |
                             ((mb_type == 2 || mb_type == 5) ? H263CU_MB_FOURMV : 0));
         int nev[6];
         bool wide = false;
@@ -595,7 +600,7 @@
             for (int b = 0; b < 6 && !be; b++) {
                 int dc;
                 bool ovf;
-                be = parse_block_fast(r, tf, tf_bits, sorenson_v1, intra, cbp[b], &dc, ev, &nev[b], &ovf, &wide);
+                be = parse_block_fast(r, tf, tf_bits, sorenson_v1, intra, cbp[b], &dc, ev, &nev[b], &ovf, &wide, positions);
                 if (intra) m.u.intradc[b] = ovf ? 0 : (uint8_t)dc;
                 m.nev[b] = (uint8_t)nev[b];
                 ev += nev[b];
@@ -622,6 +627,13 @@
                 for (int k = 0; k < nev[b]; k++) wide |= ev_level[b][k] < -512 || ev_level[b][k] > 511;
             }
             r = tmp;
+            for (int b = 0; b < 6 && positions; b++) {
+                int idx = intra ? 1 : 0;
+                for (int k = 0; k < nev[b]; k++) {
+                    idx += ev_run[b][k];
+                    ev_run[b][k] = kDezigzag[idx++];
+                }
+            }
             uint32_t total = 0;
             for (int b = 0; b < 6; b++) total += (uint32_t)nev[b];
             units = wide ? total * 2 : total;
@@ -653,7 +665,7 @@
         m.ev_off = ev_used;
         m.pic = pic_index;
         m.mbx = (uint8_t)(i % mb_w), m.mby = (uint8_t)(i / mb_w);
-        m.flags = H263CU_MB_INTER;
+        m.flags = H263CU_MB_INTER | pos_flag;
         m.quant = (uint8_t)quant;
         any_inter = true;
     }
@@ -806,7 +818,7 @@
                          h263cu_event* events, uint32_t ev_cap) {
     if (!p || !data || !pic || !mbs || (!events && ev_cap)) return H263CU_ERR_BAD_ARGUMENT;
     PendingState s;
-    int e = parse_picture_impl(p, data, len, stream, pic_index, mb_base, ev_base, pic, mbs, mb_cap, events, ev_cap, &s);
+    int e = parse_picture_impl(p, data, len, stream, pic_index, mb_base, ev_base, pic, mbs, mb_cap, events, ev_cap, &s, false);
     if (e) return e;
     commit(p, s);
     return 0;
@@ -852,7 +864,7 @@
             if (!e) {
                 e = parse_picture_impl(p, packets[i], lens[i], stream_ids ? stream_ids[i] : i, 0, 0, 0, &p->st_pic,
                                        p->st_mbs.data(), (uint32_t)p->st_mbs.size(), p->st_events.data(),
-                                       (uint32_t)p->st_events.size(), &pend[i]);
+                                       (uint32_t)p->st_events.size(), &pend[i], !commit_now);
             }
             p->st_err = e;
         }
diff --git a/h263_rs_b200/csrc/kernels.cu b/h263_rs_b200/csrc/kernels.cu
--- a/h263_rs_b200/csrc/kernels.cu
+++ b/h263_rs_b200/csrc/kernels.cu
@@ -7,9 +7,6 @@
     recon_mb_kernel(const PicDev* __restrict__ pics, const h263cu_mb* __restrict__ mbs,
                     const h263cu_event* __restrict__ events, uint32_t n_mbs, int emit_rgba, const YuvDst yuv) {
     __shared__ WarpScratch scratch[WARPS_PER_CTA];
-    __shared__ uint8_t s_dezigzag[64];
-    if (threadIdx.x < 64) s_dezigzag[threadIdx.x] = c_dezigzag[threadIdx.x];
-    __syncthreads();
 
     const int warp = threadIdx.x >> 5, lane = threadIdx.x & 31;
     const uint32_t mb_idx = blockIdx.x * WARPS_PER_CTA + warp;
@@ -36,67 +33,23 @@
         float4* cz = reinterpret_cast<float4*>(S.coef);
         for (int i = lane; i < 6 * COEF_STRIDE / 4; i += 32) cz[i] = make_float4(0.f, 0.f, 0.f, 0.f);
         __syncwarp();
-        const int first_idx = inter ? 0 : 1;
-        if (total <= 32) {
-            const bool active = (uint32_t)lane < total;
-            const uint32_t e = (uint32_t)lane;
+        uint32_t acc[6] = {0, 0, 0, 0, 0, 0};
+        for (uint32_t e = (uint32_t)lane; e < total; e += 32) {
             const int b = (e >= c1) + (e >= c2) + (e >= c3) + (e >= c4) + (e >= c5);
-            const int seg_start = b == 0 ? 0 : (b == 1 ? c1 : (b == 2 ? c2 : (b == 3 ? c3 : (b == 4 ? c4 : c5))));
-            int run = 0, level = 1;
-            if (active) load_event(ev, e, wide, run, level);
-            int v = active ? run + 1 : 0;
-#pragma unroll
-            for (int d = 1; d < 32; d <<= 1) {
-                int t = __shfl_up_sync(FULL, v, d);
-                if (lane - d >= seg_start) v += t;
-            }
-            const int pos = first_idx + v - 1;
-            const bool ok = active && pos < 64;
-            const uint32_t ovf_ballot = __ballot_sync(FULL, active && pos >= 64);
-            uint32_t bits = 0;
-            if (ok) {
-                const int lin = s_dezigzag[pos];
-                S.coef[b * COEF_STRIDE + lin] = (float)dequant(level, quant);
-                bits = (1u << (lin >> 3)) | ((lin & 7) ? INFO_COL : 0u);
-            }
-            const uint32_t cs[7] = {0, c1, c2, c3, c4, c5, total};
-#pragma unroll
-            for (int bb = 0; bb < 6; bb++) {
-                uint32_t m = __reduce_or_sync(FULL, (ok && b == bb) ? bits : 0u);
-                const uint64_t seg = ((1ull << cs[bb + 1]) - 1ull) ^ ((1ull << cs[bb]) - 1ull);
-                if (ovf_ballot & (uint32_t)seg) m |= INFO_OVF;
-                info[bb] = m;
-            }
-        } else {
-            uint32_t mine = 0;
-            if (lane < 6) {
-                const uint32_t cs[7] = {0, c1, c2, c3, c4, c5, total};
-                int idx = first_idx;
-                for (uint32_t k = cs[lane]; k < cs[lane + 1]; k++) {
-                    int run, level;
-                    load_event(ev, k, wide, run, level);
-                    idx += run;
-                    if (idx >= 64) {
-                        mine |= INFO_OVF;
-                        break;
-                    }
-                    const int lin = s_dezigzag[idx];
-                    S.coef[lane * COEF_STRIDE + lin] = (float)dequant(level, quant);
-                    mine |= (1u << (lin >> 3)) | ((lin & 7) ? INFO_COL : 0u);
-                    idx += 1;
-                }
-            }
-#pragma unroll
-            for (int bb = 0; bb < 6; bb++) info[bb] = __shfl_sync(FULL, mine, bb);
-        }
+            int lin, level;
+            load_event(ev, e, wide, lin, level);
+            S.coef[b * COEF_STRIDE + lin] = (float)dequant(level, quant);
+            const uint32_t bits = (1u << (lin >> 3)) | ((lin & 7) ? INFO_COL : 0u);
+#pragma unroll
+            for (int bb = 0; bb < 6; bb++)
+                if (b == bb) acc[bb] |= bits;
+        }
+#pragma unroll
+        for (int bb = 0; bb < 6; bb++) info[bb] = __reduce_or_sync(FULL, acc[bb]);
         if (!inter) {
             uint32_t code = 0;
             if (lane < 6) code = lane < 4 ? byte_of(w4, lane) : byte_of(w5, lane - 4);
-            uint32_t my_info = __shfl_sync(FULL, 0u, 0);
-#pragma unroll
-            for (int bb = 0; bb < 6; bb++)
-                if (lane == bb) my_info = info[bb];
-            const bool dc_ok = lane < 6 && code != 0 && !(my_info & INFO_OVF);
+            const bool dc_ok = lane < 6 && code != 0;
             if (dc_ok) S.coef[lane * COEF_STRIDE] = (float)intradc_level((int)code);
             const uint32_t dc_ballot = __ballot_sync(FULL, dc_ok);
 #pragma unroll
@@ -113,7 +66,7 @@
         const uint32_t m = info[bb];
         const uint32_t rows_ev = m & INFO_ROWS;
         int c;
-        if ((m & INFO_OVF) || !(m & (INFO_ROWS | INFO_DC)))
+        if (!(m & (INFO_ROWS | INFO_DC)))
             c = CLS_ZERO;
         else if (!(rows_ev & 0xFEu) && !(m & INFO_COL))
             c = CLS_DC;
diff --git a/h263_rs_b200/csrc/recon_common.cuh b/h263_rs_b200/csrc/recon_common.cuh
--- a/h263_rs_b200/csrc/recon_common.cuh
+++ b/h263_rs_b200/csrc/recon_common.cuh
@@ -5,7 +5,6 @@
 namespace h263dev {
 
 static __constant__ float c_basis[8][8] = H263_BASIS_TABLE;
-static __constant__ uint8_t c_dezigzag[64] = H263_DEZIGZAG_LINEAR;
 
 constexpr int WARPS_PER_CTA = 8;
 constexpr int COEF_STRIDE = 68;
@@ -16,7 +15,6 @@
 constexpr uint32_t INFO_ROWS = 0xFFu;
 constexpr uint32_t INFO_COL = 0x100u;
 constexpr uint32_t INFO_DC = 0x200u;
-constexpr uint32_t INFO_OVF = 0x400u;
 
 struct __align__(16) WarpScratch {
     float coef[6 * COEF_STRIDE];
@@ -111,14 +109,14 @@
     return a;
 }
 
-__device__ __forceinline__ void load_event(const h263cu_event* __restrict__ ev, uint32_t idx, bool wide, int& run,
+__device__ __forceinline__ void load_event(const h263cu_event* __restrict__ ev, uint32_t idx, bool wide, int& pos,
                                            int& level) {
     if (wide) {
-        run = __ldg(ev + 2 * idx) & 63;
+        pos = __ldg(ev + 2 * idx) & 63;
         level = (int16_t)__ldg(ev + 2 * idx + 1);
     } else {
         uint32_t u = __ldg(ev + idx);
-        run = (int)(u >> 10);
+        pos = (int)(u >> 10);
         level = ((int)(u << 22)) >> 22;
     }
 }
diff --git a/h263_rs_b200/csrc/recon_tile.cu b/h263_rs_b200/csrc/recon_tile.cu
--- a/h263_rs_b200/csrc/recon_tile.cu
+++ b/h263_rs_b200/csrc/recon_tile.cu
@@ -73,7 +73,6 @@
 static_assert(sizeof(TileSmemT<false, GEN_WARPS>) <= 200704 / GEN_CTAS - 1024, "shared memory budget of the generic instantiations");
 
 __device__ const float g_basis[8][8] = H263_BASIS_TABLE;
-__device__ const uint8_t g_dezigzag[64] = H263_DEZIGZAG_LINEAR;
 
 __device__ __forceinline__ constexpr float k_basis(int y, int j) {
     constexpr float T[8][8] = H263_BASIS_TABLE;
@@ -176,13 +175,6 @@
     asm volatile("{ .reg .pred p; .reg .b32 t; shfl.sync.up.b32 t|p, %0, %1, 0, 0xffffffff; @p add.u32 %0, %0, t; }" : "+r"(v) : "r"(d));
     return v;
 }
-__device__ __forceinline__ int seg_scan_up_step(int v, int d, int dist) {
-    asm volatile("{ .reg .pred p; .reg .b32 t; shfl.sync.up.b32 t, %0, %1, 0, 0xffffffff; setp.ge.s32 p, %2, %1; @p add.s32 %0, %0, t; }"
-                 : "+r"(v)
-                 : "r"(d), "r"(dist));
-    return v;
-}
-
 __device__ __forceinline__ uint32_t mad_pack(uint32_t o, uint32_t e) { return o * 256u + e; }
 
 __device__ __forceinline__ uint32_t merge_bytes(uint32_t a, uint32_t b, int keep) {
@@ -321,52 +313,28 @@
             if (in_chunk) G.slotinfo[lane] = 0u;
             __syncwarp();
 
-            uint32_t carry = 0;
             for (uint32_t eb = e_lo; eb < e_hi; eb += 32) {
                 const uint32_t e = eb + lane;
-                const bool act = e < e_hi;
                 const bool head = in_chunk && my_start >= eb && my_start < eb + 32;
                 const uint32_t heads = __reduce_or_sync(FULL, head ? 1u << (my_start - eb) : 0u);
                 const int n_before = __popc(__ballot_sync(FULL, in_chunk && my_start < eb));
-                const uint32_t below = heads & (0xFFFFFFFFu >> (31 - lane));
-                const int slot = s_lo + n_before - 1 + __popc(below);
-                const int seg = below ? 31 - __clz(below) : -1;
-                int v = 0, val = 0;
-                bool inter = false;
-                if (act) {
+                const int slot = s_lo + n_before - 1 + __popc(heads & (0xFFFFFFFFu >> (31 - lane)));
+                if (e < e_hi) {
                     const uint2 sd = G.slotdesc[slot];
                     const uint32_t k = e - G.sstart[slot];
                     const int quant = (int)((sd.y >> 8) & 31u);
-                    inter = (sd.y >> 14) & 1u;
-                    int run;
+                    uint32_t lin;
+                    int val;
                     if (!((sd.y >> 13) & 1u)) {
                         const uint32_t u = __ldg(events + sd.x + k);
-                        run = (int)(u >> 10);
+                        lin = u >> 10;
                         val = dequant_narrow(((int)(u << 22)) >> 22, 2 * quant, quant - 1 + (quant & 1));
                     } else {
-                        run = __ldg(events + sd.x + 2 * k) & 63;
+                        lin = __ldg(events + sd.x + 2 * k) & 63u;
                         val = dequant((int16_t)__ldg(events + sd.x + 2 * k + 1), quant);
                     }
-                    v = run + 1;
-                }
-                const int dist = lane - max(seg, 0);
-#pragma unroll
-                for (int d = 1; d < 32; d <<= 1) v = seg_scan_up_step(v, d, dist);
-                if (seg < 0) v += (int)carry;
-                carry = (uint32_t)__shfl_sync(FULL, v, 31);
-                if (act) {
-                    const int idx = (inter ? 0 : 1) + v - 1;
-                    uint32_t bits, ent;
-                    if (idx < 64) {
-                        const int lin = g_dezigzag[idx];
-                        ent = (uint32_t)lin | ((uint32_t)val << 16);
-                        bits = (1u << (lin >> 3)) | ((lin & 7) ? 0x100u : 0u);
-                    } else {
-                        ent = 0x8000u;
-                        bits = 0x200u;
-                    }
-                    G.evbuf[e - e_lo] = ent;
-                    atomicOr(&G.slotinfo[slot], bits);
+                    G.evbuf[e - e_lo] = lin | ((uint32_t)val << 16);
+                    atomicOr(&G.slotinfo[slot], (1u << (lin >> 3)) | ((lin & 7u) ? 0x100u : 0u));
                 }
             }
             __syncwarp();
@@ -377,14 +345,12 @@
                 const uint32_t info = G.slotinfo[lane];
                 const bool inter = (my_sd.y >> 14) & 1u;
                 const uint32_t blk = (my_sd.y >> 16) & 0xFFu, code = my_sd.y >> 24;
-                const bool ovf = (info & 0x200u) != 0, col = (info & 0x100u) != 0;
+                const bool col = (info & 0x100u) != 0;
                 const uint32_t rows = info & 0xFFu;
-                const bool has_dc = !inter && code != 0 && !ovf;
+                const bool has_dc = !inter && code != 0;
                 int cls, dcres = 0;
                 uint32_t R = 0;
-                if (ovf || (!rows && !has_dc)) {
-                    cls = CLS_ZERO;
-                } else if (!(rows & 0xFEu) && !col) {
+                if (!(rows & 0xFEu) && !col) {
                     cls = CLS_DC;
                     const int dc = has_dc ? intradc_level((int)code) : (int)G.evbuf[my_start - e_lo] >> 16;
                     dcres = round_residual_dc((float)dc);
diff --git a/h263_rs_b200/frontend.py b/h263_rs_b200/frontend.py
--- a/h263_rs_b200/frontend.py
+++ b/h263_rs_b200/frontend.py
@@ -64,12 +64,18 @@
     return pic[0]
 
 
+DEZIGZAG = sorted(range(64), key=lambda p: (p % 8 + p // 8, p // 8 if (p % 8 + p // 8) % 2 else p % 8))
+ZIGZAG_INDEX = [DEZIGZAG.index(p) for p in range(64)]
+
+
 def decode_events(mb, events, ev_base=0):
     out = []
     off = ev_base + int(mb["ev_off"])
     wide = bool(mb["flags"] & _lib.MB_WIDE)
+    pos_form = bool(mb["flags"] & _lib.MB_POS)
     for b in range(6):
         blk = []
+        idx = 0 if mb["flags"] & _lib.MB_INTER else 1
         for _ in range(int(mb["nev"][b])):
             if wide:
                 run = int(events[off]) & 63
@@ -82,6 +88,9 @@
                 if level >= 512:
                     level -= 1024
                 off += 1
+            if pos_form:
+                z = ZIGZAG_INDEX[run]
+                run, idx = z - idx, z + 1
             blk.append((run, level))
         out.append(blk)
     return out
diff --git a/include/h263cu.h b/include/h263cu.h
--- a/include/h263cu.h
+++ b/include/h263cu.h
@@ -74,6 +74,7 @@
 #define H263CU_MB_WIDE 2u
 #define H263CU_MB_FOURMV 4u
 #define H263CU_MB_CODED 8u
+#define H263CU_MB_POS 16u
 
 typedef struct h263cu_mb {
     uint32_t ev_off;
```

Measured after the change: 478,300 (median of 6 runs). 1.02x the previous value.
